# yerfor/Real3DPortrait

Hardware: AMD Instinct MI355X
Metric: rendered frames/sec @ 512x512, 48 depth samples (higher is better)
Workload: dtype f32 operands as fp16 hi + lo, fp32 accumulate (SR precision 'f16mx' = the library default, superresolution.DEFAULT_SR_PRECISION; the fp32-class f16x3 is `alt_f16x3`): in block0.conv1, block1.conv0 and block1.conv1 hi*hi runs on the f16 MFMA and the two cross products on the block-scaled 8-bit MFMA

## Files before the change

real3dportrait_amd/_lib.py:

```python
import contextlib
import ctypes
import os
import subprocess

_HERE = os.path.dirname(os.path.abspath(__file__))
LIB_PATH = os.environ.get("R3D_LIB") or os.path.join(_HERE, "lib", "libr3d_hip.so")
CSRC = os.path.join(_HERE, "csrc")

c_void_p, c_int, c_float, c_size_t, c_uint64 = (ctypes.c_void_p, ctypes.c_int, ctypes.c_float,
                                                ctypes.c_size_t, ctypes.c_uint64)
H = c_void_p


class DevPtr:
    DTYPES = {"float": ("float32",), "double": ("float64",), "int32_t": ("int32",), "int64_t": ("int64",), "uint8_t": ("uint8", "bool"),
              "uint16_t": ("bfloat16", "int16", "uint16"), "void": None}
    ctype = c_void_p

    def __init__(self, elem):
        self.elem = elem

    def __repr__(self):
        return "DevPtr(%r)" % self.elem


class Stream:
    ctype = c_void_p


F, F64, I32, I64, U8, U16, V = (DevPtr(e) for e in ("float", "double", "int32_t", "int64_t", "uint8_t", "uint16_t", "void"))
S = Stream()

SIGNATURES = {
    "r3d_version": (c_int, []),
    "r3d_last_error": (ctypes.c_char_p, []),
    "r3d_planes_to_nhwc": (c_int, [F, F, F, c_int, c_int, c_int, c_int, c_int, c_int, F, ctypes.POINTER(c_int), S]),
    "r3d_planes_absmax_partials": (c_size_t, [c_int, c_int, c_int, c_int, c_int]),
    "r3d_raygen": (c_int, [F, F, c_int, c_int, F, F, S]),
    "r3d_render_workspace_bytes": (c_size_t, [c_int, c_int, c_int, c_int]),
    "r3d_render_forward": (c_int, [F, c_int, c_int, c_int, c_int, F, F, F, F, F, F, c_int, c_int, c_int, c_float, c_int, F, F, c_uint64, F, c_int, F,
                                   F, U8, F, c_int, F, F, V, F, c_size_t, V, c_size_t, S]),
    "r3d_run_model": (c_int, [F, c_int, c_int, c_int, c_int, F, F, F, F, F, c_int, c_float, F, F, F, c_int, V, c_size_t, S]),
    "r3d_run_model_workspace_bytes": (c_size_t, []),
    "r3d_sr_block_prepacked_bytes": (c_size_t, [c_int, c_int]),
    "r3d_sr_block_styles_bytes": (c_size_t, [c_int, c_int, c_int]),
    "r3d_sr_block_workspace_bytes": (c_size_t, [c_int, c_int, c_int, c_int, c_int]),
    "r3d_sr_block_prepack": (c_int, [c_int, c_int, F, F, V, c_int, S]),
    "r3d_sr_block_styles": (c_int, [F, c_int, c_int, c_int, c_int, F, F, F, F, F, F, F, F, F, F, F, F, V, S]),
    "r3d_sr_block_forward": (c_int, [V, V, c_int, c_int, c_int, c_int, c_int, c_int, V, c_int, F, c_float, V, c_int, F, c_size_t, F, U8, F, c_int, V,
                                     c_size_t, S]),
    "r3d_chain_fold": (c_int, [H, c_int, c_int, H, c_int, H, c_int, S]),
    "r3d_sr_block_bound_offset": (c_size_t, [c_int, c_int]),
    "r3d_conv_scales_bound_offset": (c_size_t, [c_int, c_int]),
    "r3d_absmax": (c_int, [F, c_size_t, c_int, F, F, S]),
    "r3d_conv_prepacked_bytes": (c_size_t, [c_int, c_int, c_int]),
    "r3d_conv_workspace_bytes": (c_size_t, [c_int, c_int, c_int, c_int]),
    "r3d_conv_scales_bytes": (c_size_t, [c_int, c_int, c_int]),
    "r3d_conv_prepack": (c_int, [F, c_int, c_int, c_int, V, S]),
    "r3d_conv_forward": (c_int, [V, V, F, c_int, c_int, c_int, c_int, c_int, c_int, V, c_int, c_int, c_float, c_float, c_float, V, c_int, F,
                                 c_size_t, F, V, c_size_t, S]),
    "r3d_blend_cat_to_split": (c_int, [F, c_int, c_int, F, c_int, c_int, F, c_int, c_int, c_int, V, c_int, F, c_size_t, S]),
    "r3d_conv_forward_cat": (c_int, [V, V, F, c_int, c_int, c_int, c_int, c_int, c_int, V, c_int, c_int, c_float, c_float, c_float, V, c_int, c_int,
                                     c_int, F, c_int, F, c_size_t, V, c_size_t, S]),
    "r3d_conv_forward_blend": (c_int, [V, V, F, c_int, c_int, c_int, c_int, c_int, c_int, F, F, F, c_int, c_float, c_float, c_float, V, c_int, F,
                                       c_size_t, F, S]),
    "r3d_debug_conv_variant": (c_int, [c_int, c_int, c_int, c_int, c_int, c_int, c_int, c_int, ctypes.POINTER(c_int)]),
    "r3d_debug_sr_block_variants": (c_int, [c_int, c_int, c_int, c_int, c_int, c_int, c_int, c_int, c_float, ctypes.POINTER(c_int)]),
    "r3d_upsample2x_bilinear": (c_int, [F, c_int, c_int, c_int, c_int, V, c_int, F, c_size_t, S]),
    "r3d_resize_bilinear": (c_int, [F, c_int, c_int, c_int, F, c_int, c_int, c_int, S]),
    "r3d_blend": (c_int, [F, F, F, c_int, c_int, c_int, c_int, F, S]),
    "r3d_person_occlusion": (c_int, [F, F, c_float, c_size_t, F, S]),
    "r3d_frames_to_u8": (c_int, [F, c_int, c_int, c_int, U8, S]),
    "r3d_comm_unique_id": (c_int, [H]),
    "r3d_comm_init": (c_int, [H, c_int, c_int, ctypes.POINTER(c_void_p)]),
    "r3d_comm_destroy": (c_int, [H]),
    "r3d_gather_frames": (c_int, [H, U8, c_size_t, U8, c_int, S]),
    "r3d_event_create": (c_int, [ctypes.POINTER(c_void_p)]),
    "r3d_event_record": (c_int, [H, S]),
    "r3d_event_elapsed_ms": (c_int, [H, H, ctypes.POINTER(c_float)]),
    "r3d_event_destroy": (c_int, [H]),
    "r3d_profile_configure": (c_int, [ctypes.c_uint32]),
    "r3d_profile_reset": (c_int, []),
    "r3d_profile_read": (c_int, [c_int, ctypes.POINTER(ctypes.c_double), ctypes.POINTER(c_int)]),
    "r3d_profile_clock": (c_int, [c_int, ctypes.POINTER(ctypes.c_double), ctypes.POINTER(ctypes.c_ulonglong)]),
    "r3d_secc_embed1": (c_int, [F, c_int, c_int, c_int, c_int, F, F, F, F, F, F, F, S]),
    "r3d_secc_conv": (c_int, [F, c_int, c_int, c_int, c_int, F, F, c_int, c_int, c_int, c_int, F, F, c_float, F, S]),
    "r3d_secc_linear": (c_int, [F, c_int, c_int, F, F, c_float, F, F, c_int, c_int, F, F, S]),
    "r3d_secc_layernorm": (c_int, [F, c_int, c_int, F, F, c_float, F, S]),
    "r3d_secc_attention": (c_int, [F, F, c_int, c_int, c_int, c_int, c_int, c_float, F, S]),
    "r3d_secc_dwconv_gelu": (c_int, [F, c_int, c_int, c_int, c_int, F, F, F, S]),
    "r3d_secc_head": (c_int, [F, c_int, c_int, c_int, F, F, F, F, F, F, F, F, S]),
    "r3d_torso_volume_to_cl": (c_int, [F, c_int, c_int, c_int, c_int, c_int, F, S]),
    "r3d_torso_warp": (c_int, [F, c_int, c_int, c_int, c_int, c_int, F, c_int, c_int, c_int, F, c_int, S]),
    "r3d_torso_conv": (c_int, [F, c_int, c_int, c_int, c_int, c_int, c_int, F, F, c_float, F, F, c_int, c_int, c_int, c_float, F, F, F, S]),
    "r3d_torso_conv3d": (c_int, [F, c_int, c_int, c_int, c_int, c_int, c_int, F, F, c_int, c_int, c_int, c_int, c_float, c_int, F, c_int, c_int, F,
                                 S]),
    "r3d_torso_motion_input": (c_int, [F, c_int, c_int, c_int, c_int, c_int, F, F, F, F, F, c_int, F, c_int, F, c_int, S]),
    "r3d_torso_motion_deform": (c_int, [F, c_int, c_int, c_int, c_int, c_int, F, F, F, F, S]),
    "r3d_torso_motion_broadcast": (c_int, [F, c_int, c_int, c_int, c_int, c_int, F, c_int, c_int, S]),
    "r3d_torso_conv_prec": (c_int, [F, c_int, c_int, c_int, c_int, c_int, c_int, F, F, c_float, F, F, c_int, c_int, c_int, c_float, F, F, F, c_int,
                                    S]),
    "r3d_torso_conv3d_prec": (c_int, [F, c_int, c_int, c_int, c_int, c_int, c_int, F, F, c_int, c_int, c_int, c_int, c_float, c_int, F, c_int, c_int,
                                      F, c_int, S]),
    "r3d_torso_split_bf16x3": (c_int, [F, c_size_t, U16, U16, U16, S]),
    "r3d_torso_conv_pool": (c_int, [F, c_int, c_int, c_int, c_int, c_int, F, F, c_int, c_int, c_int, c_float, c_int, F, c_int, S]),
    "r3d_torso_conv_split": (c_int, [F, c_int, c_int, c_int, c_int, c_int, F, F, c_int, c_int, c_int, c_float, c_int, F, c_int, S]),
    "r3d_torso_conv3d_res": (c_int, [F, c_int, c_int, c_int, c_int, c_int, F, F, c_float, F, F, c_int, c_int, c_int, c_float, F, F, F, c_int, S]),
    "r3d_torso_seg_input": (c_int, [F, c_int, c_int, F, c_int, c_int, c_int, c_int, c_int, F, c_int, c_int, S]),
    "r3d_torso_mask_volume": (c_int, [F, c_int, c_int, c_int, c_int, c_int, F, c_int, c_int, c_int, c_int, c_int, c_int, c_int, F, F, S]),
    "r3d_raster_workspace_bytes": (c_size_t, [c_int, c_int, c_int]),
    "r3d_raster_forward": (c_int, [F, F, I32, c_int, c_int, c_int, c_int, c_int, c_int, c_float, c_float, c_int, c_int, c_float, c_float, I64, F, F,
                                   F, V, c_size_t, S]),
    "r3d_secc_blink_workspace_bytes": (c_size_t, [c_int, c_int, c_int]),
    "r3d_secc_blink": (c_int, [F, c_int, c_int, c_int, I32, F64, c_int, F, I32, V, c_size_t, S]),
    "r3d_face_vertex": (c_int, [F, F, F, c_int, c_int, c_int, F, F, F, F, c_int, c_float, c_int, F, S]),
    "r3d_face_landmarks": (c_int, [F, F, F, c_int, c_int, c_int, F, F, F, F, c_int, c_float, c_int, c_float, c_float, c_float, F, S]),
    "r3d_clip_camera": (c_int, [F, F, c_int, c_int, ctypes.c_double, F, S]),
    "r3d_camera_smooth": (c_int, [F, c_int, c_int, c_int, F, S]),
    "r3d_smooth_features": (c_int, [F, c_int, c_int, c_int, c_int, F, S]),
    "r3d_video_depth_range": (c_int, [F, c_size_t, c_int, I32, S]),
    "r3d_video_compose_debug": (c_int, [F, F, c_int, c_int, F, c_int, c_int, F, c_int, c_int, F, c_int, c_int, c_int, c_int, I32, U8, S]),
    "r3d_source_workspace_bytes": (c_size_t, [c_int, c_int, c_int]),
    "r3d_source_nearest": (c_int, [U8, c_int, c_int, c_int, I32, I32, I32, V, c_size_t, S]),
    "r3d_source_background": (c_int, [U8, U8, c_int, c_int, c_int, U8, I32, V, c_size_t, S]),
    "r3d_source_torso": (c_int, [U8, U8, c_int, c_int, ctypes.POINTER(ctypes.c_double), ctypes.POINTER(c_int), U8, U8, U8, U8, V, c_size_t, S]),
    "r3d_source_select": (c_int, [U8, U8, c_int, c_int, c_int, U8, U8, S]),
    "r3d_source_to_planes": (c_int, [U8, U8, c_int, c_int, c_int, F, S]),
}
AUDIO_SIGNATURES = {
    "r3d_a2m_conv1d": (c_int, [F, c_int, c_int, c_int, c_int, c_int, c_int, F, F, c_int, c_int, c_int, c_int, c_int, F, F, I64, c_int, c_int, F, F, F, F, F, F,
                               c_int, c_int, c_int, S]),
    "r3d_a2m_wn_layer": (c_int, [F, F, c_int, c_int, c_int, c_int, c_int, F, F, F, F, F, c_int, c_int, F, F, S]),
    "r3d_a2m_pitch_embed": (c_int, [F, c_int, c_int, F, c_int, c_int, I32, F, S]),
}
_FIT_COMMON = [F, F, F, c_int, c_int, c_int, F, F, c_int, c_int, c_float, c_float, c_float, ctypes.POINTER(c_float)]
FIT_SIGNATURES = {
    "r3d_fit_workspace_bytes": (c_size_t, [c_int, c_int, c_int, c_int]),
    "r3d_fit_state_bytes": (c_size_t, [c_int, c_int, c_int, c_int]),
    "r3d_fit_landmark_grad": (c_int, _FIT_COMMON + [F, F, F, F, F, F, F, F, F, V, c_size_t, S]),
    "r3d_fit_landmark_run": (c_int, _FIT_COMMON + [c_float, c_float, c_int, c_int, c_int, c_int, F, V, c_size_t, S]),
}
FIT_LOSS_WORDS, FIT_LAUNCHES = 8, 2
A2M_WN_ROWS = 16
VIDEO_STATE_WORDS, VIDEO_PANELS_ALL, VIDEO_PANEL_DEPTH = 8, 31, 8
SOURCE_MAX_SIDE, SOURCE_STATUS_WORDS, SOURCE_DARKEN, SOURCE_HEAD_CLASSES = 2048, 2, 53, 42

OPTIONAL_SIGNATURES = {
    "r3d_debug_merge_fallbacks": (c_int, [ctypes.POINTER(ctypes.c_ulonglong), c_int]),
    "r3d_debug_raster_forward": (c_int, [F, F, I32, c_int, c_int, c_int, c_int, c_int, c_int, c_float, c_float, c_int, c_int, c_float, c_float,
                                         I64, F, F, F, V, c_size_t, c_int, c_int, S]),
    "r3d_debug_secc_blink": (c_int, [F, c_int, c_int, c_int, I32, F64, c_int, F, I32, V, c_size_t, c_int, S]),
}


class ChainOp(ctypes.Structure):
    _fields_ = [("kind", c_int), ("Cin", c_int), ("Cout", c_int), ("ksize", c_int), ("act", c_int),
                ("gain", c_float), ("clamp", c_float), ("src_a", c_int), ("src_b", c_int),
                ("scales", c_void_p), ("prepacked", c_void_p), ("bias", c_void_p)]


CHAIN_SR_BLOCK, CHAIN_CONV, CHAIN_SR_BLOCK_TAIL, CHAIN_SRC_NONE, CHAIN_MAX_OPS, CHAIN_MAX_EXT, CHAIN_MAX_ZERO = 0, 1, 2, -1000, 12, 4, 4

ABI_VERSION = 80
_lib = None
_torch = None
_Tensor = ()
_plans = {}
_calls = None


def build(force=False):
    args = ["make", "-s", "-C", CSRC, "-j4"]
    if force:
        args.append("-B")
    subprocess.check_call(args)
    return LIB_PATH


def _bind(fn, name, res, params, torch):
    fn.restype, fn.argtypes = res, [getattr(p, "ctype", p) for p in params]
    dtypes = lambda names: names and tuple(getattr(torch, d) for d in names if hasattr(torch, d))
    dev = tuple((i, p.elem, dtypes(DevPtr.DTYPES[p.elem])) for i, p in enumerate(params) if isinstance(p, DevPtr))
    _plans[name] = (len(params), bool(params) and isinstance(params[-1], Stream), dev, res is c_int and name != "r3d_version")


def load():
    global _lib, _torch, _Tensor
    if _lib is not None:
        return _lib
    import torch
    if not os.path.exists(LIB_PATH):
        raise RuntimeError(
            "real3dportrait_amd: HIP extension %s not built -- run `make -C %s` (there is no CPU/eager fallback)"
            % (LIB_PATH, CSRC))
    try:
        lib = ctypes.CDLL(LIB_PATH)
    except OSError as e:
        raise RuntimeError("real3dportrait_amd: cannot load %s: %s" % (LIB_PATH, e))
    for name, (res, params) in list(SIGNATURES.items()) + list(AUDIO_SIGNATURES.items()) + list(FIT_SIGNATURES.items()):
        try:
            fn = getattr(lib, name)
        except AttributeError:
            raise RuntimeError("real3dportrait_amd: %s does not export %s, which this package binds -- rebuild it (`make -C %s`)"
                               % (LIB_PATH, name, CSRC))
        _bind(fn, name, res, params, torch)
    for name, (res, params) in OPTIONAL_SIGNATURES.items():
        fn = getattr(lib, name, None)
        if fn is not None:
            _bind(fn, name, res, params, torch)
    if lib.r3d_version() != ABI_VERSION:
        raise RuntimeError("real3dportrait_amd: %s reports ABI %d, this package binds ABI %d -- rebuild it (`make -C %s`)"
                           % (LIB_PATH, lib.r3d_version(), ABI_VERSION, CSRC))
    _torch, _Tensor = torch, torch.Tensor
    _lib = lib
    return lib


def call(name, *args):
    lib = load()
    n, stream, dev, status = _plans[name]
    args = list(args)
    add_stream = stream and len(args) == n - 1
    if len(args) != n and not add_stream:
        raise TypeError("libr3d_hip %s takes %d arguments%s, got %d" % (name, n, " (the stream may be left out)" if stream else "", len(args)))
    for i, elem, dtypes in dev:
        t = args[i]
        if isinstance(t, _Tensor):
            if dtypes is not None and t.dtype not in dtypes:
                raise TypeError("libr3d_hip %s: argument %d is a %s*, got a %s tensor" % (name, i, elem, t.dtype))
            if not t.is_contiguous():
                raise ValueError("libr3d_hip %s: argument %d (%s*) is not contiguous" % (name, i, elem))
            if not t.is_cuda:
                raise ValueError("libr3d_hip %s: argument %d (%s*) is not on a GPU: the library operates on device tensors only" % (name, i, elem))
            args[i] = t.data_ptr()
    if add_stream:
        args.append(_torch.cuda.current_stream().cuda_stream)
    if _calls is not None:
        _calls.append((name, tuple(args)))
    rc = getattr(lib, name)(*args)
    if not status:
        return rc
    if rc != 0:
        check(rc, name[4:])


@contextlib.contextmanager
def counting():
    global _calls
    outer, _calls = _calls, []
    try:
        yield _calls
    finally:
        _calls = outer


def check(rc, what=""):
    if rc != 0:
        msg = load().r3d_last_error()
        raise RuntimeError("libr3d_hip %s failed (%d): %s" % (what, rc, msg.decode() if msg else "?"))


def ptr(t):
    if t is None:
        return None
    if not t.is_cuda:
        raise ValueError("libr3d_hip operates on device tensors only")
    if not t.is_contiguous():
        raise ValueError("libr3d_hip takes contiguous tensors")
    return t.data_ptr()


def stream_ptr():
    load()
    return _torch.cuda.current_stream().cuda_stream
```

real3dportrait_amd/csrc/r3d_sr.hip:

```cpp
#include "r3d_sr_launch.h"

namespace r3d {


static constexpr int TILE_H = 8, TILE_W = 16;
static constexpr int PATCH_H = TILE_H + 2, PATCH_W = TILE_W + 2, PATCH_PIX = PATCH_H * PATCH_W;
static constexpr int CHUNKS_PER_STAGE = 4;

__global__ void nchw_to_cb8_kernel(const float* __restrict__ src, float* __restrict__ dst, int C, int HW)
{
    const int n = blockIdx.z, cb = blockIdx.y;
    const int p = blockIdx.x * blockDim.x + threadIdx.x;
    if (p >= HW) return;
    const float* s = src + ((size_t)n * C + cb * 8) * HW + p;
    float v[8];
#pragma unroll
    for (int c = 0; c < 8; ++c) v[c] = s[(size_t)c * HW];
    float4* d = reinterpret_cast<float4*>(dst + (((size_t)n * (C / 8) + cb) * HW + p) * 8);
    d[0] = make_float4(v[0], v[1], v[2], v[3]);
    d[1] = make_float4(v[4], v[5], v[6], v[7]);
}

__global__ void cb8_to_nchw_kernel(const float* __restrict__ src, float* __restrict__ dst, int C, int HW)
{
    const int n = blockIdx.z, cb = blockIdx.y;
    const int p = blockIdx.x * blockDim.x + threadIdx.x;
    if (p >= HW) return;
    const float4* s = reinterpret_cast<const float4*>(src + (((size_t)n * (C / 8) + cb) * HW + p) * 8);
    const float4 a = s[0], b = s[1];
    float* d = dst + ((size_t)n * C + cb * 8) * HW + p;
    d[0] = a.x; d[(size_t)HW] = a.y; d[(size_t)2 * HW] = a.z; d[(size_t)3 * HW] = a.w;
    d[(size_t)4 * HW] = b.x; d[(size_t)5 * HW] = b.y; d[(size_t)6 * HW] = b.z; d[(size_t)7 * HW] = b.w;
}

__global__ void sr_prepack_kernel(const float* __restrict__ w, int Ci, int Cout, float* __restrict__ out)
{
    const size_t e = (size_t)blockIdx.x * blockDim.x + threadIdx.x;
    const size_t total = (size_t)9 * (Ci / 8) * Cout * 2;
    if (e >= total) return;
    const int half = e & 1;
    const int co = (e >> 1) % Cout;
    const int chunk = ((e >> 1) / Cout) % (Ci / 8);
    const int tap = (int)((e >> 1) / Cout / (Ci / 8));
    const int ci = chunk * 8 + half * 4;
    const float* src = w + ((size_t)co * Ci + ci) * 9 + tap;
    reinterpret_cast<float4*>(out)[e] = make_float4(src[0], src[9], src[18], src[27]);
}

__global__ void sr_styles_kernel(const float* __restrict__ ws3, int WD, int Cin, int Cout,
                                 const float* __restrict__ aw0, const float* __restrict__ ab0,
                                 const float* __restrict__ aw1, const float* __restrict__ ab1,
                                 const float* __restrict__ aw2, const float* __restrict__ ab2,
                                 float* __restrict__ styles, size_t stride_n)
{
    const int layer = blockIdx.y, n = blockIdx.z;
    const SrStyleLayout L = sr_style_layout(Cin, Cout);
    const float* aw = layer == 0 ? aw0 : (layer == 1 ? aw1 : aw2);
    const float* ab = layer == 0 ? ab0 : (layer == 1 ? ab1 : ab2);
    const int C = layer == 0 ? Cin : Cout;
    const int lane = threadIdx.x & 63, c = blockIdx.x * (blockDim.x >> 6) + (threadIdx.x >> 6);
    if (c >= C) return;
    float* out = styles + n * stride_n + (layer == 0 ? L.s0 : (layer == 1 ? L.s1 : L.s2));
    const float* w = ws3 + ((size_t)n * 3 + layer) * WD;
    const float g = rsqrtf((float)WD);
    const float post = layer == 2 ? rsqrtf((float)Cout) : 1.0f;
    float acc = 0.f;
    for (int j = lane; j < WD; j += 64) acc += w[j] * (aw[(size_t)c * WD + j] * g);
#pragma unroll
    for (int d = 32; d >= 1; d >>= 1) acc += __shfl_xor(acc, d);
    if (lane == 0) out[c] = (acc + ab[c]) * post;
}

__global__ void sr_demod_kernel(int Cin, int Cout, const float* __restrict__ w0, const float* __restrict__ w1,
                                const float* __restrict__ wrgb, const float* __restrict__ b0, const float* __restrict__ b1,
                                const float* __restrict__ brgb, float* __restrict__ styles, size_t stride_n)
{
    const int co = blockIdx.x, n = blockIdx.y, layer = blockIdx.z;
    const SrStyleLayout L = sr_style_layout(Cin, Cout);
    float* base = styles + n * stride_n;
    if (co == Cout) {
        if (layer == 0)
            for (int i = threadIdx.x; i < 3 * Cout; i += blockDim.x) {
                base[L.wrgb + i] = wrgb[i] * base[L.s2 + (i % Cout)];
                if (i < Cout) { base[L.b0 + i] = b0[i]; base[L.b1 + i] = b1[i]; }
                if (i < 3) base[L.brgb + i] = brgb[i];
            }
        return;
    }
    const int Ci = layer == 0 ? Cin : Cout;
    const float* W = (layer == 0 ? w0 : w1) + (size_t)co * Ci * 9;
    const float* st = base + (layer == 0 ? L.s0 : L.s1);
    float ss = 0.f, l1 = 0.f, mx = 0.f;
    for (int i = threadIdx.x; i < Ci * 9; i += blockDim.x) {
        const float wv = W[i], v = wv * st[i / 9];
        ss += v * v; l1 += fabsf(v); mx = fmaxf(mx, fabsf(wv));
    }
#pragma unroll
    for (int d = 32; d >= 1; d >>= 1) { ss += __shfl_xor(ss, d); l1 += __shfl_xor(l1, d); mx = fmaxf(mx, __shfl_xor(mx, d)); }
    __shared__ float red[3][4];
    if ((threadIdx.x & 63) == 0) { red[0][threadIdx.x >> 6] = ss; red[1][threadIdx.x >> 6] = l1; red[2][threadIdx.x >> 6] = mx; }
    __syncthreads();
    if (threadIdx.x == 0) {
        const float d = rsqrtf(red[0][0] + red[0][1] + red[0][2] + red[0][3] + 1e-8f);
        base[(layer == 0 ? L.d0 : L.d1) + co] = d;
        base[(layer == 0 ? L.c0 : L.c1) + co] = d * (red[1][0] + red[1][1] + red[1][2] + red[1][3]);
        base[(layer == 0 ? L.wi0 : L.wi1) + co] = pow2f(-weight_row_exp(fmaxf(fmaxf(red[2][0], red[2][1]), fmaxf(red[2][2], red[2][3]))));
    }
}

struct ChainArgs {
    r3d_chain_op ops[R3D_CHAIN_MAX_OPS];
    const float* ext[R3D_CHAIN_MAX_EXT];
    float* zero[R3D_CHAIN_MAX_ZERO];
    int nops, N, nzero, next;
};

__device__ __forceinline__ float block_max(float v, float* red)
{
#pragma unroll
    for (int d = 32; d >= 1; d >>= 1) v = fmaxf(v, __shfl_xor(v, d));
    __syncthreads();
    if ((threadIdx.x & 63) == 0) red[threadIdx.x >> 6] = v;
    __syncthreads();
    return fmaxf(fmaxf(red[0], red[1]), fmaxf(red[2], red[3]));
}

__global__ __launch_bounds__(256) void chain_fold_kernel(ChainArgs a)
{
    __shared__ float red[4];
    __shared__ float bounds[R3D_CHAIN_MAX_OPS];
    __shared__ float extv[R3D_CHAIN_MAX_EXT];
    const int n = blockIdx.x, tid = threadIdx.x;
    if (tid < a.next) extv[tid] = fabsf(a.ext[tid][n]);
    {
        float touch = 0.f;
        for (int k = 0; k < a.nops; ++k) {
            const r3d_chain_op& op = a.ops[k];
            if (op.kind == R3D_CHAIN_SR_BLOCK || op.kind == R3D_CHAIN_SR_BLOCK_TAIL) {
                const SrStyleLayout L = sr_style_layout(op.Cin, op.Cout);
                const float* base = reinterpret_cast<const float*>(op.scales) + (size_t)n * L.total;
                for (int i = tid; i < op.Cin; i += 256) touch += base[L.s0 + i];
                for (int i = tid; i < op.Cout; i += 256)
                    touch += base[L.s1 + i] + base[L.d0 + i] + base[L.d1 + i] + base[L.wi0 + i] + base[L.wi1 + i] + base[L.b0 + i] + base[L.b1 + i] + base[L.c0 + i] + base[L.c1 + i];
            } else {
                const ConvPackLayout P = conv_pack_layout(op.Cin, op.Cout, op.ksize);
                const ConvTail T = conv_tail_layout(P.Co);
                const float* tail = reinterpret_cast<const float*>(op.prepacked) + P.tail;
                for (int i = tid; i < P.Co; i += 256) touch += tail[T.winv + i] + tail[T.l1 + i] + (op.bias && i < op.Cout ? op.bias[i] : 0.f);
            }
        }
        if (touch == 1.2345e-33f && a.nzero < 0) extv[0] = touch;
    }
    __syncthreads();
// ... 269 lines not shown
    float o[4] = {acc.x + b[0], acc.y + b[1], acc.z + b[2], acc.w + b[3]};
#pragma unroll
    for (int r = 0; r < 4; ++r) {
        float t = o[r];
        t = (t < 0.f ? t * 0.2f : t) * 1.4142135623730951f;
        if (clamp >= 0.f) t = fminf(fmaxf(t, -clamp), clamp);
        o[r] = t;
    }
    *reinterpret_cast<float4*>(y + (size_t)n * y_stride_n + (((size_t)cb * OH + oy) * OW + ox) * 8 + half * 4) =
        make_float4(o[0], o[1], o[2], o[3]);
}

__global__ void torgb_upsample_kernel(const float* __restrict__ x, size_t x_stride_n,
                                      const float* __restrict__ wrgb, const float* __restrict__ brgb, size_t pk_stride_n,
                                      const float* __restrict__ img_prev, float* __restrict__ img_out,
                                      int C, int H, int W, float clamp)
{
    extern __shared__ float sw[];
    const int n = blockIdx.y;
    for (int i = threadIdx.x; i < 3 * C; i += blockDim.x) sw[i] = wrgb[(size_t)n * pk_stride_n + i];
    __syncthreads();
    const int p = blockIdx.x * blockDim.x + threadIdx.x;
    if (p >= H * W) return;
    const int y = p / W, xx = p - y * W;
    const float* X = x + (size_t)n * x_stride_n;
    float a0 = 0.f, a1 = 0.f, a2 = 0.f;
    const int ncb = C >> 3;
    for (int cb = 0; cb < ncb; ++cb) {
        const float4* s = reinterpret_cast<const float4*>(X + ((size_t)cb * H * W + p) * 8);
        const float4 u = s[0], v = s[1];
        const float xv[8] = {u.x, u.y, u.z, u.w, v.x, v.y, v.z, v.w};
#pragma unroll
        for (int c = 0; c < 8; ++c) {
            a0 += xv[c] * sw[cb * 8 + c];
            a1 += xv[c] * sw[C + cb * 8 + c];
            a2 += xv[c] * sw[2 * C + cb * 8 + c];
        }
    }
    const float* br = brgb + (size_t)n * pk_stride_n;
    float o[3] = {a0 + br[0], a1 + br[1], a2 + br[2]};
    if (clamp >= 0.f) {
#pragma unroll
        for (int c = 0; c < 3; ++c) o[c] = fminf(fmaxf(o[c], -clamp), clamp);
    }
    const int Hh = H >> 1, Wh = W >> 1;
    const int ky = y >> 1, kx = xx >> 1;
    int r0, r1, c0, c1; float wy0, wy1, wx0, wx1;
    if (y & 1) { r0 = ky; r1 = ky + 1; wy0 = 0.75f; wy1 = 0.25f; } else { r0 = ky - 1; r1 = ky; wy0 = 0.25f; wy1 = 0.75f; }
    if (xx & 1) { c0 = kx; c1 = kx + 1; wx0 = 0.75f; wx1 = 0.25f; } else { c0 = kx - 1; c1 = kx; wx0 = 0.25f; wx1 = 0.75f; }
    const bool vr0 = r0 >= 0 && r0 < Hh, vr1 = r1 >= 0 && r1 < Hh, vc0 = c0 >= 0 && c0 < Wh, vc1 = c1 >= 0 && c1 < Wh;
#pragma unroll
    for (int c = 0; c < 3; ++c) {
        const float* I = img_prev + ((size_t)n * 3 + c) * Hh * Wh;
        float up = 0.f;
        if (vr0 && vc0) up += I[(size_t)r0 * Wh + c0] * (wy0 * wx0);
        if (vr0 && vc1) up += I[(size_t)r0 * Wh + c1] * (wy0 * wx1);
        if (vr1 && vc0) up += I[(size_t)r1 * Wh + c0] * (wy1 * wx0);
        if (vr1 && vc1) up += I[(size_t)r1 * Wh + c1] * (wy1 * wx1);
        img_out[((size_t)n * 3 + c) * H * W + p] = up + o[c];
    }
}


}

using namespace r3d;

extern "C" size_t r3d_sr_block_prepacked_bytes(int Cin, int Cout) { return sr_pack_layout(Cin, Cout).total * sizeof(float); }

extern "C" size_t r3d_sr_block_styles_bytes(int N, int Cin, int Cout)
{
    return (size_t)N * sr_style_layout(Cin, Cout).total * sizeof(float);
}

extern "C" size_t r3d_sr_block_workspace_bytes(int N, int Cin, int Cout, int Hin, int Win) { return sr_workspace_layout(N, Cin, Cout, Hin, Win).total; }

namespace r3d {
void sr_fill_tconv_phases(ConvPhase* ph, int Hin, int Win)
{
    for (int pa = 0; pa < 2; ++pa)
        for (int pb = 0; pb < 2; ++pb) {
            ConvPhase& p = ph[pa * 2 + pb];
            p.outH = Hin + (pa == 0); p.outW = Win + (pb == 0);
            p.oy_mul = 2; p.oy_add = pa; p.ox_mul = 2; p.ox_add = pb; p.out_off = 0;
            p.ntaps = 0;
            for (int ky = pa; ky < 3; ky += 2)
                for (int kx = pb; kx < 3; kx += 2) {
                    p.dy[p.ntaps] = -(ky >> 1); p.dx[p.ntaps] = -(kx >> 1); p.widx[p.ntaps] = ky * 3 + kx;
                    ++p.ntaps;
                }
        }
}
void sr_fill_conv3x3_phase(ConvPhase* ph, int H, int W)
{
    ConvPhase& p = ph[0];
    p.outH = H; p.outW = W; p.oy_mul = 1; p.oy_add = 0; p.ox_mul = 1; p.ox_add = 0; p.ntaps = 9; p.out_off = 0;
    for (int ky = 0; ky < 3; ++ky)
        for (int kx = 0; kx < 3; ++kx) { p.dy[ky * 3 + kx] = ky - 1; p.dx[ky * 3 + kx] = kx - 1; p.widx[ky * 3 + kx] = ky * 3 + kx; }
}
void sr_fill_conv1x1_phase(ConvPhase* ph, int H, int W)
{
    ConvPhase& p = ph[0];
    p.outH = H; p.outW = W; p.oy_mul = 1; p.oy_add = 0; p.ox_mul = 1; p.ox_add = 0; p.out_off = 0;
    p.ntaps = 1; p.dy[0] = 0; p.dx[0] = 0; p.widx[0] = 0;
}
}

static int sr_check_dims(const char* what, int Cin, int Cout)
{
    if (Cin <= 0 || Cout <= 0 || (Cin & 7) || (Cout % BLOCK_M)) {
        set_error("%s: Cin %d must be a multiple of 8 and Cout %d a multiple of %d", what, Cin, Cout, BLOCK_M);
        return R3D_ERR_INVALID_ARG;
    }
    return R3D_OK;
}

extern "C" int r3d_sr_block_prepack(int Cin, int Cout, const float* c0_w, const float* c1_w, void* prepacked,
                                    int precision, r3d_stream_t stream)
{
    if (precision < R3D_SR_F32 || precision > R3D_SR_F16MX) { set_error("sr_block_prepack: unknown precision %d", precision); return R3D_ERR_INVALID_ARG; }
    if (!c0_w || !c1_w || !prepacked) { set_error("sr_block_prepack: NULL pointer"); return R3D_ERR_INVALID_ARG; }
    if (int rc = sr_check_dims("sr_block_prepack", Cin, Cout)) return rc;
    hipStream_t st = (hipStream_t)stream;
    float* out = reinterpret_cast<float*>(prepacked);
    ProfScope ps(R3D_PROF_PACK, st);
    if (precision != R3D_SR_F32) return sr_prepack_f16x3(Cin, Cout, c0_w, c1_w, prepacked, st, precision == R3D_SR_F16MX);
    const size_t n0 = (size_t)9 * (Cin / 8) * Cout * 2, n1 = (size_t)9 * (Cout / 8) * Cout * 2;
    const SrPackLayout P = sr_pack_layout(Cin, Cout);
    hipLaunchKernelGGL(sr_prepack_kernel, dim3((unsigned)((n0 + 255) / 256)), dim3(256), 0, st, c0_w, Cin, Cout, out + P.c0);
    hipLaunchKernelGGL(sr_prepack_kernel, dim3((unsigned)((n1 + 255) / 256)), dim3(256), 0, st, c1_w, Cout, Cout, out + P.c1);
    return check_launch("sr_block_prepack");
}

extern "C" int r3d_sr_block_styles(const float* ws3, int N, int WD, int Cin, int Cout,
                                   const float* c0_w, const float* c0_b, const float* c0_aw, const float* c0_ab,
                                   const float* c1_w, const float* c1_b, const float* c1_aw, const float* c1_ab,
                                   const float* rgb_w, const float* rgb_b, const float* rgb_aw, const float* rgb_ab,
                                   void* styles, r3d_stream_t stream)
{
    if (!ws3 || !c0_w || !c0_b || !c0_aw || !c0_ab || !c1_w || !c1_b || !c1_aw || !c1_ab || !rgb_w || !rgb_b || !rgb_aw || !rgb_ab || !styles) {
        set_error("sr_block_styles: NULL pointer"); return R3D_ERR_INVALID_ARG;
    }
    if (N <= 0 || WD <= 0) { set_error("sr_block_styles: bad shape"); return R3D_ERR_INVALID_ARG; }
    if (int rc = sr_check_dims("sr_block_styles", Cin, Cout)) return rc;
    hipStream_t st = (hipStream_t)stream;
    float* sv = reinterpret_cast<float*>(styles);
    const size_t stride = sr_style_layout(Cin, Cout).total;
    ProfScope ps(R3D_PROF_PACK, st);
    hipLaunchKernelGGL(sr_styles_kernel, dim3(((Cin > Cout ? Cin : Cout) + 3) / 4, 3, N), dim3(256), 0, st, ws3, WD, Cin, Cout, c0_aw, c0_ab, c1_aw, c1_ab, rgb_aw, rgb_ab, sv, stride);
    hipLaunchKernelGGL(sr_demod_kernel, dim3(Cout + 1, N, 2), dim3(256), 0, st, Cin, Cout, c0_w, c1_w, rgb_w, c0_b, c1_b, rgb_b, sv, stride);
    return check_launch("sr_block_styles");
}

extern "C" int r3d_sr_block_forward(const void* prepacked, const void* styles, int N, int Cin, int Cout, int Hin, int Win, int up,
                                    const void* x, int x_format, const float* img, float clamp,
                                    void* x_out, int x_out_format, const float* next_scale, size_t next_scale_stride,
                                    float* img_out, uint8_t* img_u8, float* x_absmax, int precision,
                                    void* workspace, size_t workspace_bytes, r3d_stream_t stream)
{
    if (precision < R3D_SR_F32 || precision > R3D_SR_F16MX) { set_error("sr_block_forward: unknown precision %d", precision); return R3D_ERR_INVALID_ARG; }
    if ((img_u8 || x_absmax) && precision == R3D_SR_F32) { set_error("sr_block_forward: the fused uint8 output / x_absmax need R3D_SR_F16X3"); return R3D_ERR_INVALID_ARG; }
    if (!prepacked || !styles || !x || !img || (!img_out && !img_u8) || N <= 0 || Hin <= 0 || Win <= 0 || (Cin & 15) || (Cout % BLOCK_M) || (up != 0 && up != 1)) {
        set_error("sr_block_forward: bad argument"); return R3D_ERR_INVALID_ARG;
    }
    if (!up && precision == R3D_SR_F32) { set_error("sr_block_forward: up=0 (SynthesisBlockNoUp) needs R3D_SR_F16X3"); return R3D_ERR_INVALID_ARG; }
    if (int rc = r3d::check_index32("sr_block_forward", (size_t)(Cin > Cout ? Cin : Cout), (size_t)(up ? 2 : 1) * Hin, (size_t)(up ? 2 : 1) * Win)) return rc;
    if (!workspace || workspace_bytes < r3d_sr_block_workspace_bytes(N, Cin, Cout, Hin, Win)) {
        set_error("sr_block_forward: workspace too small"); return R3D_ERR_WORKSPACE;
    }
    if (!x_out) x_out_format = R3D_FMT_NONE;
    const bool f16 = precision != R3D_SR_F32;
    const bool mxp = precision == R3D_SR_F16MX;
    if (x_format < R3D_FMT_NCHW || x_format > R3D_FMT_SPLIT_MX || x_out_format < R3D_FMT_NONE || x_out_format > R3D_FMT_SPLIT_MX ||
        (!f16 && (x_format >= R3D_FMT_SPLIT || x_out_format >= R3D_FMT_SPLIT)) ||
        ((x_format == R3D_FMT_SPLIT_MX || x_out_format == R3D_FMT_SPLIT_MX) && !mxp) ||
        (x_out_format >= R3D_FMT_SPLIT && !next_scale)) {
        set_error("sr_block_forward: unsupported activation format (x %d, x_out %d, precision %d)", x_format, x_out_format, precision);
        return R3D_ERR_INVALID_ARG;
    }
    hipStream_t st = (hipStream_t)stream;
    if (f16)
        return sr_block_forward_f16x3(prepacked, styles, N, Cin, Cout, Hin, Win, up, x, x_format, img, clamp, x_out, x_out_format,
                                      next_scale, next_scale_stride, img_out, img_u8, x_absmax, workspace, st, precision == R3D_SR_F16MX);

    const SrStyleLayout L = sr_style_layout(Cin, Cout);
    const float* pk = reinterpret_cast<const float*>(styles);
    const float* wpk = reinterpret_cast<const float*>(prepacked);
    const SrPackLayout P = sr_pack_layout(Cin, Cout);
    const int OH = 2 * Hin, OW = 2 * Win, TH = OH + 1, TW = OW + 1;
    const SrWorkspaceLayout WS = sr_workspace_layout(N, Cin, Cout, Hin, Win);
    char* wsb = reinterpret_cast<char*>(workspace);
    float* xin = reinterpret_cast<float*>(wsb + WS.xin);
    float* T = reinterpret_cast<float*>(wsb + WS.T);
    float* y0 = reinterpret_cast<float*>(wsb + WS.y0);
    float* xo = reinterpret_cast<float*>(wsb + WS.xo);

    const float* xcb = reinterpret_cast<const float*>(x);
    if (x_format == R3D_FMT_NCHW) {
        ProfScope ps(R3D_PROF_LAYOUT, st);
        hipLaunchKernelGGL(nchw_to_cb8_kernel, dim3((Hin * Win + 255) / 256, Cin / 8, N), dim3(256), 0, st, xcb, xin, Cin, Hin * Win);
        xcb = xin;
    }
    {
        ConvArgs a;
        a.x = xcb; a.x_stride_n = (size_t)Cin * Hin * Win;
        a.wp = wpk + P.c0; a.in_scale = pk + L.s0; a.out_scale = pk + L.d0; a.vec_stride_n = L.total;
        a.bias = nullptr;
        a.y = T; a.y_stride_n = (size_t)Cout * TH * TW;
        a.Cin = Cin; a.Cout = Cout; a.H = Hin; a.W = Win; a.OH = TH; a.OW = TW;
        a.nphase = 4; a.act = 0; a.clamp = -1.f;
        sr_fill_tconv_phases(a.ph, Hin, Win);
        int maxtiles = 0;
        for (int p = 0; p < 4; ++p) {
            const int tiles = ((a.ph[p].outW + TILE_W - 1) / TILE_W) * ((a.ph[p].outH + TILE_H - 1) / TILE_H);
            if (tiles > maxtiles) maxtiles = tiles;
        }
        ProfScope ps(R3D_PROF_CONV, st);
        hipLaunchKernelGGL(conv_mfma_kernel, dim3(maxtiles, Cout / BLOCK_M, N * 4), dim3(256), 0, st, a);
    }
    {
    ProfScope ps(R3D_PROF_UPCONV, st);
    hipLaunchKernelGGL(fir_bias_act_kernel, dim3((OH * OW * 2 + 255) / 256, Cout / 8, N), dim3(256), 0, st,
                       T, (size_t)Cout * TH * TW, pk + L.b0, L.total, y0, (size_t)Cout * OH * OW, Cout, OH, OW, clamp);
    }
    float* xo_cb = (x_out_format == R3D_FMT_CB8) ? reinterpret_cast<float*>(x_out) : xo;
    {
        ConvArgs a;
        a.x = y0; a.x_stride_n = (size_t)Cout * OH * OW;
        a.wp = wpk + P.c1; a.in_scale = pk + L.s1; a.out_scale = pk + L.d1; a.vec_stride_n = L.total;
        a.bias = pk + L.b1;
        a.y = xo_cb; a.y_stride_n = (size_t)Cout * OH * OW;
        a.Cin = Cout; a.Cout = Cout; a.H = OH; a.W = OW; a.OH = OH; a.OW = OW;
        a.nphase = 1; a.act = 1; a.clamp = clamp;
        sr_fill_conv3x3_phase(a.ph, OH, OW);
        const int tiles = ((OW + TILE_W - 1) / TILE_W) * ((OH + TILE_H - 1) / TILE_H);
        ProfScope ps(R3D_PROF_CONV, st);
        hipLaunchKernelGGL(conv_mfma_kernel, dim3(tiles, Cout / BLOCK_M, N), dim3(256), 0, st, a);
    }
    {
    ProfScope ps(R3D_PROF_TORGB, st);
    hipLaunchKernelGGL(torgb_upsample_kernel, dim3((OH * OW + 255) / 256, N), dim3(256), 3 * Cout * sizeof(float), st,
                       xo_cb, (size_t)Cout * OH * OW, pk + L.wrgb, pk + L.brgb, L.total, img, img_out, Cout, OH, OW, clamp);
    }
    if (x_out_format == R3D_FMT_NCHW) {
        ProfScope ps(R3D_PROF_LAYOUT, st);
        hipLaunchKernelGGL(cb8_to_nchw_kernel, dim3((OH * OW + 255) / 256, Cout / 8, N), dim3(256), 0, st, xo_cb,
                           reinterpret_cast<float*>(x_out), Cout, OH * OW);
    }
    return check_launch("sr_block_forward");
}

extern "C" size_t r3d_conv_prepacked_bytes(int Cin, int Cout, int ksize) { return r3d::conv_prepacked_bytes_f16x3(Cin, Cout, ksize); }
extern "C" size_t r3d_conv_workspace_bytes(int N, int Cin, int H, int W) { return r3d::conv_workspace_bytes_f16x3(N, Cin, H, W); }
extern "C" size_t r3d_conv_scales_bytes(int N, int Cin, int Cout)
{
    const ConvPackLayout P = conv_pack_layout(Cin, Cout, 1);
    return (size_t)N * conv_scales_layout(P.Ci, P.Co).total * sizeof(float);
}
extern "C" size_t r3d_conv_scales_bound_offset(int Cin, int Cout)
{
    const ConvPackLayout P = conv_pack_layout(Cin, Cout, 1);
    return conv_scales_layout(P.Ci, P.Co).meta + 1;
}
extern "C" size_t r3d_sr_block_bound_offset(int Cin, int Cout) { return sr_style_layout(Cin, Cout).meta + SR_META_BOUND_OUT; }

extern "C" int r3d_conv_prepack(const float* weight, int Cin, int Cout, int ksize, void* prepacked, r3d_stream_t stream)
{
    using namespace r3d;
    if (!weight || !prepacked || Cin <= 0 || Cout <= 0 || (ksize != 1 && ksize != 3)) { set_error("conv_prepack: bad argument"); return R3D_ERR_INVALID_ARG; }
    return conv_prepack_f16x3(weight, Cin, Cout, ksize, prepacked, (hipStream_t)stream);
}

extern "C" int r3d_chain_fold(const r3d_chain_op* ops, int nops, int N, const float* const* ext_bounds, int n_ext,
                              float* const* zero_slots, int n_zero, r3d_stream_t stream)
{
    using namespace r3d;
    if (!ops || nops <= 0 || nops > R3D_CHAIN_MAX_OPS || N <= 0 || n_ext < 0 || n_ext > R3D_CHAIN_MAX_EXT || (n_ext && !ext_bounds) ||
        n_zero < 0 || n_zero > R3D_CHAIN_MAX_ZERO || (n_zero && !zero_slots)) {
        set_error("chain_fold: bad argument (1..%d ops, 0..%d external bounds, 0..%d zero slots)", R3D_CHAIN_MAX_OPS, R3D_CHAIN_MAX_EXT, R3D_CHAIN_MAX_ZERO);
        return R3D_ERR_INVALID_ARG;
    }
    ChainArgs a = {};
    a.nops = nops; a.N = N; a.nzero = n_zero; a.next = n_ext;
    for (int j = 0; j < n_zero; ++j) {
        if (!zero_slots[j]) { set_error("chain_fold: zero slot %d is NULL", j); return R3D_ERR_INVALID_ARG; }
        a.zero[j] = zero_slots[j];
    }
    for (int j = 0; j < n_ext; ++j) {
        if (!ext_bounds[j]) { set_error("chain_fold: external bound %d is NULL", j); return R3D_ERR_INVALID_ARG; }
        a.ext[j] = ext_bounds[j];
    }
    for (int k = 0; k < nops; ++k) {
        const r3d_chain_op& op = ops[k];
        const int srcs[2] = {op.src_a, op.src_b};
        for (int j = 0; j < 2; ++j) {
            const int sidx = srcs[j];
            const bool ok = sidx == R3D_CHAIN_SRC_NONE || (sidx >= 0 && sidx < k) || (sidx < 0 && sidx >= -n_ext);
            if (!ok) { set_error("chain_fold: op %d reads bound source %d (must be an earlier op or an external bound)", k, sidx); return R3D_ERR_INVALID_ARG; }
        }
        if (op.src_a == R3D_CHAIN_SRC_NONE && op.src_b == R3D_CHAIN_SRC_NONE) { set_error("chain_fold: op %d has no input bound", k); return R3D_ERR_INVALID_ARG; }
        if ((op.kind != R3D_CHAIN_SR_BLOCK && op.kind != R3D_CHAIN_CONV && op.kind != R3D_CHAIN_SR_BLOCK_TAIL) || !op.scales || op.Cin <= 0 || op.Cout <= 0 ||
            (op.kind == R3D_CHAIN_CONV && (!op.prepacked || (op.ksize != 1 && op.ksize != 3)))) {
            set_error("chain_fold: op %d is malformed", k); return R3D_ERR_INVALID_ARG;
        }
        a.ops[k] = op;
        if (a.ops[k].src_a == R3D_CHAIN_SRC_NONE) a.ops[k].src_a = -R3D_CHAIN_MAX_EXT - 1;
        if (a.ops[k].src_b == R3D_CHAIN_SRC_NONE) a.ops[k].src_b = -R3D_CHAIN_MAX_EXT - 1;
    }
    ProfScope ps(R3D_PROF_PACK, (hipStream_t)stream);
    hipLaunchKernelGGL(chain_fold_kernel, dim3(N), dim3(256), 0, (hipStream_t)stream, a);
    return check_launch("chain_fold");
}

extern "C" int r3d_absmax(const float* x, size_t count_per_sample, int N, float* out, float* zero_next, r3d_stream_t stream)
{
    using namespace r3d;
    if (!x || !out || N <= 0 || count_per_sample == 0) { set_error("absmax: bad argument"); return R3D_ERR_INVALID_ARG; }
    size_t blocks = (count_per_sample / 4 + 255) / 256;
    if (blocks > 512) blocks = 512;
    if (blocks < 1) blocks = 1;
    ProfScope ps(R3D_PROF_LAYOUT, (hipStream_t)stream);
    hipLaunchKernelGGL(absmax_kernel, dim3((unsigned)blocks, N), dim3(256), 0, (hipStream_t)stream, x, count_per_sample,
                       reinterpret_cast<unsigned*>(out), reinterpret_cast<unsigned*>(zero_next));
    return check_launch("absmax");
}

extern "C" int r3d_conv_forward(const void* prepacked, const void* scales, const float* bias,
                                int N, int Cin, int Cout, int H, int W, int ksize,
                                const void* x, int x_format, int act, float act_slope, float act_gain, float clamp,
                                void* y, int y_format, const float* next_scale, size_t next_scale_stride, float* y_absmax,
                                void* workspace, size_t workspace_bytes, r3d_stream_t stream)
{
    using namespace r3d;
    SrConvCall c = sr_conv_call("conv_forward", N, Cin, Cout, H, W, ksize, act, act_slope, act_gain, clamp, y, y_format, next_scale, next_scale_stride,
                                y_absmax, (hipStream_t)stream);
    c.prepacked = prepacked; c.scales = scales; c.bias = bias; c.x = x; c.x_format = x_format; c.workspace = workspace; c.workspace_bytes = workspace_bytes;
    if (int rc = check(c)) return rc;
    return conv_forward_f16x3(c);
}

extern "C" int r3d_conv_forward_cat(const void* prepacked, const void* scales, const float* bias,
                                    int N, int Cin, int Cout, int H, int W, int ksize,
                                    const void* x, int x_format, int act, float act_slope, float act_gain, float clamp,
                                    void* y_cat, int y_format, int C_total, int chan_off, const float* mask, int mask_invert,
                                    const float* next_scale, size_t next_scale_stride,
                                    void* workspace, size_t workspace_bytes, r3d_stream_t stream)
{
    using namespace r3d;
    const ConvCat cat = {mask, mask_invert ? 1 : 0, C_total, chan_off};
    SrConvCall c = sr_conv_call("conv_forward_cat", N, Cin, Cout, H, W, ksize, act, act_slope, act_gain, clamp, y_cat, y_format, next_scale, next_scale_stride,
                                nullptr, (hipStream_t)stream);
    c.prepacked = prepacked; c.scales = scales; c.bias = bias; c.x = x; c.x_format = x_format; c.workspace = workspace; c.workspace_bytes = workspace_bytes;
    c.cat = &cat;
    if (int rc = check(c)) return rc;
    return conv_forward_f16x3(c);
}

extern "C" int r3d_conv_forward_blend(const void* prepacked, const void* scales, const float* bias,
                                      int N, int Ca, int Cb, int Cout, int H, int W,
                                      const float* a, const float* b, const float* mask,
                                      int act, float act_slope, float act_gain, float clamp,
                                      void* y, int y_format, const float* next_scale, size_t next_scale_stride, float* y_absmax, r3d_stream_t stream)
{
    using namespace r3d;
    SrConvCall c = sr_conv_call("conv_forward_blend", N, Ca + Cb, Cout, H, W, 1, act, act_slope, act_gain, clamp, y, y_format,
                                next_scale, next_scale_stride, y_absmax, (hipStream_t)stream);
    c.prepacked = prepacked; c.scales = scales; c.bias = bias;
    c.blend = true; c.bl_a = a; c.bl_b = b; c.bl_mask = mask; c.Ca = Ca; c.Cb = Cb;
    if (int rc = check(c)) return rc;
    return conv_forward_blend_f16x3(c);
}

static void put_variant(const r3d::SrVariantChoice& v, int* out)
{
    out[0] = v.variant; out[1] = v.bits; out[2] = v.order; out[3] = (int)v.gx; out[4] = (int)v.gy; out[5] = (int)v.gz;
}

extern "C" int r3d_debug_conv_variant(int N, int Cin, int Cout, int H, int W, int ksize, int x_format, int blend, int* out)
{
    using namespace r3d;
    if (!out || N <= 0 || Cin <= 0 || Cout <= 0 || H <= 0 || W <= 0 || (ksize != 1 && ksize != 3) || (blend && ksize != 1) ||
        x_format < R3D_FMT_NCHW || x_format > R3D_FMT_SPLIT_MX || (x_format != R3D_FMT_NCHW && (Cin & 15)) || (x_format == R3D_FMT_SPLIT_MX && ksize != 3)) {
        set_error("debug_conv_variant: bad argument"); return R3D_ERR_INVALID_ARG;
    }
    const ConvPackLayout P = conv_pack_layout(Cin, Cout, ksize);
    put_variant(blend ? sr_blend_variant(P.Co, H, W, N) : sr_conv_variant(ksize, P.Ci, P.Co, H, W, N, x_format == R3D_FMT_SPLIT_MX, false, sr_wino_mode()), out);
    return R3D_OK;
}

extern "C" int r3d_debug_sr_block_variants(int N, int Cin, int Cout, int Hin, int Win, int up, int x_format, int precision, float clamp, int* out)
{
    using namespace r3d;
    if (!out || N <= 0 || Hin <= 0 || Win <= 0 || (Cin & 15) || Cin <= 0 || Cout <= 0 || (Cout % BLOCK_M) || (up != 0 && up != 1) ||
        (precision != R3D_SR_F16X3 && precision != R3D_SR_F16MX) || x_format < R3D_FMT_NCHW || x_format > R3D_FMT_SPLIT_MX ||
        (x_format == R3D_FMT_SPLIT_MX && precision != R3D_SR_F16MX)) {
        set_error("debug_sr_block_variants: bad argument"); return R3D_ERR_INVALID_ARG;
    }
    SrVariantChoice v[2];
    sr_block_variants(N, Cin, Cout, Hin, Win, up, x_format, precision == R3D_SR_F16MX, clamp, sr_wino_mode(), v);
    put_variant(v[0], out); put_variant(v[1], out + 6);
    return R3D_OK;
}

extern "C" int r3d_upsample2x_bilinear(const float* x_cb8, int N, int C, int H, int W, void* y, int y_format,
                                       const float* next_scale, size_t next_scale_stride, r3d_stream_t stream)
{
    using namespace r3d;
    if (!x_cb8 || !y || N <= 0 || C <= 0 || (C & 7) || H <= 0 || W <= 0) { set_error("upsample2x_bilinear: bad argument (C %d must be a multiple of 8)", C); return R3D_ERR_INVALID_ARG; }
    if (y_format != R3D_FMT_CB8 && y_format != R3D_FMT_SPLIT && y_format != R3D_FMT_SPLIT_MX) { set_error("upsample2x_bilinear: y_format %d must be CB8, SPLIT or SPLIT_MX", y_format); return R3D_ERR_INVALID_ARG; }
    if (y_format == R3D_FMT_SPLIT_MX && (C & 15)) { set_error("upsample2x_bilinear: SPLIT_MX needs C %% 16 == 0 (C %d)", C); return R3D_ERR_INVALID_ARG; }
    return upsample2x_bilinear_f16x3(x_cb8, N, C, H, W, y, y_format, next_scale, next_scale_stride, (hipStream_t)stream);
}

extern "C" int r3d_blend_cat_to_split(const float* a, int a_format, int Ca, const float* b, int b_format, int Cb, const float* mask,
                                      int N, int H, int W, void* y_split, int y_format, const float* next_scale, size_t next_scale_stride,
                                      r3d_stream_t stream)
{
    if (y_format != R3D_FMT_SPLIT && y_format != R3D_FMT_SPLIT_MX) { set_error("blend_cat_to_split: y_format %d must be SPLIT or SPLIT_MX", y_format); return R3D_ERR_INVALID_ARG; }
    using namespace r3d;
    if (!a || !mask || !y_split || N <= 0 || H <= 0 || W <= 0 || Ca <= 0 || Cb <= 0 || (Ca & 7) || (Cb & 7) || ((Ca + Cb) & 15) || (!b && (Ca & 15))) {
        set_error("blend_cat_to_split: bad argument (Ca %d, Cb %d: multiples of 8, sum a multiple of 16; b = NULL needs Ca %% 16 == 0)", Ca, Cb); return R3D_ERR_INVALID_ARG;
    }
    if ((a_format != R3D_FMT_NCHW && a_format != R3D_FMT_CB8) || (b && b_format != R3D_FMT_NCHW && b_format != R3D_FMT_CB8)) {
        set_error("blend_cat_to_split: inputs must be NCHW or CB8 (a %d, b %d)", a_format, b_format); return R3D_ERR_INVALID_ARG;
    }
    return blend_cat_to_split_f16x3(a, a_format, Ca, b, b_format, Cb, mask, N, H, W, y_split, y_format, next_scale, next_scale_stride, (hipStream_t)stream);
}
```

real3dportrait_amd/csrc/r3d_sr_common.h:

```cpp
#pragma once
#include "r3d_common.h"

namespace r3d {

typedef float f32x16 __attribute__((ext_vector_type(16)));
static constexpr int BLOCK_M = 128;
static __host__ __device__ inline size_t align256(size_t b) { return (b + 255) & ~(size_t)255; }

static constexpr int kWeightTargetExp = 10;
static constexpr int kActTargetExp = 15;

__host__ __device__ inline int pow2_ceil_exp(float m)
{
    if (!(m > 0.f) || !(m < 3.0e38f)) return 0;
    int e;
    (void)frexpf(m, &e);
    return e;
}
__host__ __device__ inline float pow2f(int e) { return ldexpf(1.0f, e < -120 ? -120 : (e > 120 ? 120 : e)); }
__host__ __device__ inline int weight_row_exp(float rowmax) { return rowmax > 0.f ? kWeightTargetExp + 1 - pow2_ceil_exp(rowmax) : 0; }
__host__ __device__ inline int act_exp(float B, float smax)
{
    const int eb = B > 0.f ? pow2_ceil_exp(B) : 0;
    int es = smax > 0.f ? pow2_ceil_exp(smax) : 0;
    if (smax > 0.f && smax < 3.0e38f && ldexpf(1.0f, es - 1) == smax) --es;
    return kActTargetExp - eb - es;
}

struct SrStyleLayout { size_t s0f, s1f, d0f, d1f, s0, s1, s2, d0, d1, wrgb, b0, b1, brgb, c0, c1, wi0, wi1, meta, total; };
static __host__ __device__ inline SrStyleLayout sr_style_layout(int Cin, int Cout)
{
    SrStyleLayout L;
    size_t o = 0;
    L.s0f = o; o += Cin;
    L.s1f = o; o += Cout;
    L.d0f = o; o += Cout;
    L.d1f = o; o += Cout;
    L.s0 = o; o += Cin;
    L.s1 = o; o += Cout;
    L.s2 = o; o += Cout;
    L.d0 = o; o += Cout;
    L.d1 = o; o += Cout;
    L.wrgb = o; o += (size_t)3 * Cout;
    L.b0 = o; o += Cout;
    L.b1 = o; o += Cout;
    L.brgb = o; o += 4;
    L.c0 = o; o += Cout;
    L.c1 = o; o += Cout;
    L.wi0 = o; o += Cout;
    L.wi1 = o; o += Cout;
    L.meta = o; o += 8;
    L.total = (o + 3) & ~(size_t)3;
    return L;
}
enum { SR_META_BOUND_IN = 0, SR_META_BOUND_MID = 1, SR_META_BOUND_OUT = 2, SR_META_E0 = 3, SR_META_E1 = 4, SR_META_SMAX0 = 5, SR_META_SMAX1 = 6 };

struct ConvTail { size_t winv, l1, total; };
static __host__ __device__ inline ConvTail conv_tail_layout(int CoutPadded)
{
    ConvTail T; T.winv = 0; T.l1 = CoutPadded; T.total = 2 * (size_t)CoutPadded; return T;
}
struct ConvScales { size_t in_vec, out_vec, meta, total; };
static __host__ __device__ inline ConvScales conv_scales_layout(int CinPadded, int CoutPadded)
{
    ConvScales S; S.in_vec = 0; S.out_vec = CinPadded; S.meta = (size_t)CinPadded + CoutPadded; S.total = (S.meta + 4 + 3) & ~(size_t)3; return S;
}

struct SrPackLayout { size_t c0, c1, c0_up, tail0, tail1, c0_up_mx, c0_mx, c1_wino, total; };
static __host__ __device__ inline SrPackLayout sr_pack_layout(int Cin, int Cout)
{
    SrPackLayout P;
    const size_t w0 = (size_t)9 * Cin * Cout, w1 = (size_t)9 * Cout * Cout;
    size_t o = 0;
    P.c0 = o; o += w0;
    P.c1 = o; o += w1;
    P.c0_up = o; o += w0;
    P.tail0 = o; o += conv_tail_layout(Cout).total;
    P.tail1 = o; o += conv_tail_layout(Cout).total;
    P.c0_up_mx = o; o += w0;
    P.c0_mx = o; o += w0;
    P.c1_wino = o; o += (size_t)12 * Cout * Cout;
    P.total = o;
    return P;
}
struct ConvPackLayout { int Ci, Co; size_t w, tail, w_mx, w_wino, total; };
static __host__ __device__ inline ConvPackLayout conv_pack_layout(int Cin, int Cout, int ksize)
{
    ConvPackLayout P;
    P.Ci = (Cin + 15) / 16 * 16; P.Co = (Cout + BLOCK_M - 1) / BLOCK_M * BLOCK_M;
    const size_t cc = (size_t)P.Ci * P.Co, w = (size_t)(ksize * ksize) * cc;
    size_t o = 0;
    P.w = o; o += w;
    P.tail = o; o += conv_tail_layout(P.Co).total;
    P.w_mx = o; o += ksize == 3 ? w : 0;
    P.w_wino = o; o += ksize == 3 ? 12 * cc : 0;
    P.total = o;
    return P;
}
struct SrWorkspaceLayout { size_t xin, T, y0, xo, rgbp, total; };
static __host__ __device__ inline SrWorkspaceLayout sr_workspace_layout(int N, int Cin, int Cout, int Hin, int Win)
{
    SrWorkspaceLayout L;
    const size_t y = align256((size_t)N * Cout * 4 * Hin * Win * 4);
    size_t o = 0;
    L.xin = o; o += align256((size_t)N * Cin * Hin * Win * 4);
    L.T = o; o += align256((size_t)N * Cout * 4 * (Hin + 1) * (Win + 1) * 4);
    L.y0 = o; o += y;
    L.xo = o; o += y;
    L.rgbp = o; o += align256((size_t)N * (Cout / 64) * 3 * 4 * Hin * Win * 4);
    L.total = o;
    return L;
}

struct ConvPhase {
    int outH, outW;
    int oy_mul, oy_add, ox_mul, ox_add;
    int ntaps;
    int dy[9], dx[9], widx[9];
    size_t out_off;
};

void sr_fill_tconv_phases(ConvPhase* ph, int Hin, int Win);
void sr_fill_conv3x3_phase(ConvPhase* ph, int H, int W);
void sr_fill_conv1x1_phase(ConvPhase* ph, int H, int W);

int sr_prepack_f16x3(int Cin, int Cout, const float* c0_w, const float* c1_w, void* prepacked, hipStream_t st, bool mx);
int sr_block_forward_f16x3(const void* prepacked, const void* styles, int N, int Cin, int Cout, int Hin, int Win, int up,
                           const void* x, int x_format, const float* img, float clamp,
                           void* x_out, int x_out_format, const float* next_scale, size_t next_scale_stride,
                           float* img_out, uint8_t* img_u8, float* x_absmax, void* workspace, hipStream_t st, bool mx);

size_t conv_prepacked_bytes_f16x3(int Cin, int Cout, int ksize);
int conv_prepack_f16x3(const float* w, int Cin, int Cout, int ksize, void* prepacked, hipStream_t st);
size_t conv_workspace_bytes_f16x3(int N, int Cin, int H, int W);
struct ConvCat { const float* mask; int mask_invert; int C_total; int chan_off; };

int upsample2x_bilinear_f16x3(const float* x_cb8, int N, int C, int H, int W, void* y, int y_format,
                              const float* next_scale, size_t next_scale_stride, hipStream_t st);

int blend_cat_to_split_f16x3(const float* a, int a_format, int Ca, const float* b, int b_format, int Cb, const float* mask,
                             int N, int H, int W, void* y_split, int y_format, const float* next_scale, size_t next_scale_stride, hipStream_t st);

}
```

real3dportrait_amd/csrc/r3d_sr_f16x3.hip:

```cpp
#include <stdlib.h>

#include "r3d_sr_launch.h"
#include "r3d_stamps.h"

namespace r3d {

typedef _Float16 h8 __attribute__((ext_vector_type(8)));
typedef _Float16 h4 __attribute__((ext_vector_type(4)));
static constexpr int F_TILE_H = 16, F_TILE_W = 16;
static constexpr int F_PATCH_H = F_TILE_H + 2, F_PATCH_W = F_TILE_W + 2, F_PATCH_PIX = F_PATCH_H * F_PATCH_W;

__device__ __forceinline__ void split1(float v, _Float16& hi, _Float16& lo)
{
    v = as_rounded(v);
    const float c = fminf(fmaxf(v, -65504.f), 65504.f);
    hi = (_Float16)c;
    lo = (_Float16)(v - (float)hi);
}

__device__ __forceinline__ void split1_folded(float v, _Float16& hi, _Float16& lo)
{
    v = as_rounded(v);
    hi = (_Float16)v;
    lo = (_Float16)(v - (float)hi);
// ... 20 lines not shown
    return (unsigned)v;
}

__global__ void weight_row_stats_kernel(const float* __restrict__ w, int row_len, int CoutReal, int Cout, float* __restrict__ tail)
{
    const int co = blockIdx.x;
    const ConvTail T = conv_tail_layout(Cout);
    float mx = 0.f, l1 = 0.f;
    if (co < CoutReal)
        for (int i = threadIdx.x; i < row_len; i += blockDim.x) { const float v = fabsf(w[(size_t)co * row_len + i]); mx = fmaxf(mx, v); l1 += v; }
#pragma unroll
    for (int d = 32; d >= 1; d >>= 1) { mx = fmaxf(mx, __shfl_xor(mx, d)); l1 += __shfl_xor(l1, d); }
    __shared__ float rm[4], rl[4];
    if ((threadIdx.x & 63) == 0) { rm[threadIdx.x >> 6] = mx; rl[threadIdx.x >> 6] = l1; }
    __syncthreads();
    if (threadIdx.x == 0) {
        mx = fmaxf(fmaxf(rm[0], rm[1]), fmaxf(rm[2], rm[3]));
        tail[T.winv + co] = pow2f(-weight_row_exp(mx));
        tail[T.l1 + co] = rl[0] + rl[1] + rl[2] + rl[3];
    }
}

__global__ void sr_prepack_mx_kernel(const float* __restrict__ w, int CiReal, int CoutReal, int ntaps, int Ci, int Cout,
                                     const float* __restrict__ winv, uint4* __restrict__ out)
{
    const size_t e = (size_t)blockIdx.x * blockDim.x + threadIdx.x;
    const size_t total = (size_t)ntaps * (Ci / 16) * Cout;
    if (e >= total) return;
    const int co = e % Cout;
    const int grp = (e / Cout) % (Ci / 16);
    const int tap = (int)(e / Cout / (Ci / 16));
    const float ws = 1.0f / winv[co];
    float hi[16], lo[16];
    h8 h0, h1;
#pragma unroll
    for (int j = 0; j < 16; ++j) {
        const int ci = grp * 16 + j;
        const float v = (co < CoutReal && ci < CiReal) ? w[((size_t)co * CiReal + ci) * ntaps + tap] * ws : 0.f;
        _Float16 a, b; split1(v, a, b);
        hi[j] = (float)a; lo[j] = v - (float)a;
        if (j < 8) h0[j] = a; else h1[j - 8] = a;
    }
    uint4 wl8, wh8;
    unsigned* pl = reinterpret_cast<unsigned*>(&wl8); unsigned* ph = reinterpret_cast<unsigned*>(&wh8);
#pragma unroll
    for (int q = 0; q < 4; ++q) {
        const int c = mx_rec_chan(q);
        pl[q] = pack4_fp8(lo[c] * kMxWl, lo[c + 1] * kMxWl, lo[c + 2] * kMxWl, lo[c + 3] * kMxWl);
        ph[q] = pack4_fp8(hi[c] * kMxWh, hi[c + 1] * kMxWh, hi[c + 2] * kMxWh, hi[c + 3] * kMxWh);
    }
    const size_t base = ((size_t)tap * (Ci / 8) + 2 * grp) * 2 * Cout + co;
    out[base] = *reinterpret_cast<uint4*>(&h0);
    out[base + Cout] = wl8;
    out[base + 2 * Cout] = *reinterpret_cast<uint4*>(&h1);
    out[base + 3 * Cout] = wh8;
}

__global__ void sr_prepack_f16_kernel(const float* __restrict__ w, int CiReal, int CoutReal, int ntaps, int Ci, int Cout,
                                      const float* __restrict__ winv, uint4* __restrict__ out)
{
    const size_t e = (size_t)blockIdx.x * blockDim.x + threadIdx.x;
    const size_t total = (size_t)ntaps * (Ci / 8) * Cout;
    if (e >= total) return;
    const int co = e % Cout;
    const int chunk = (e / Cout) % (Ci / 8);
    const int tap = (int)(e / Cout / (Ci / 8));
    const float ws = 1.0f / winv[co];
    h8 hi, lo;
#pragma unroll
    for (int j = 0; j < 8; ++j) {
        const int ci = chunk * 8 + j;
        const float v = (co < CoutReal && ci < CiReal) ? w[((size_t)co * CiReal + ci) * ntaps + tap] * ws : 0.f;
        _Float16 a, b; split1(v, a, b); hi[j] = a; lo[j] = b;
    }
    const size_t base = ((size_t)tap * (Ci / 8) + chunk) * 2 * Cout + co;
    out[base] = *reinterpret_cast<uint4*>(&hi);
    out[base + Cout] = *reinterpret_cast<uint4*>(&lo);
}

__global__ void to_split_kernel(const float* __restrict__ src, int cb8, const float* __restrict__ scale, size_t scale_stride_n,
                                uint4* __restrict__ dst, int C, int Creal, int HW)
{
    const int n = blockIdx.z, cb = blockIdx.y;
    const int p = blockIdx.x * blockDim.x + threadIdx.x;
    if (p >= HW) return;
    float v[8];
    if (cb8) {
        const float4* s4 = reinterpret_cast<const float4*>(src + (((size_t)n * (C / 8) + cb) * HW + p) * 8);
        const float4 a = s4[0], b = s4[1];
        v[0] = a.x; v[1] = a.y; v[2] = a.z; v[3] = a.w; v[4] = b.x; v[5] = b.y; v[6] = b.z; v[7] = b.w;
    } else {
        const float* s = src + ((size_t)n * Creal + cb * 8) * HW + p;
#pragma unroll
        for (int c = 0; c < 8; ++c) v[c] = (cb * 8 + c < Creal) ? s[(size_t)c * HW] : 0.f;
    }
    h8 hi, lo;
#pragma unroll
    for (int c = 0; c < 8; ++c) {
        const float sc = (scale && cb * 8 + c < Creal) ? scale[n * scale_stride_n + cb * 8 + c] : 1.f;
        _Float16 a, b; split_scaled(v[c], sc, a, b); hi[c] = a; lo[c] = b;
    }
    const size_t plane = (size_t)(C / 8) * HW;
    uint4* d = dst + (size_t)n * 2 * plane + (size_t)cb * HW + p;
    d[0] = *reinterpret_cast<uint4*>(&hi);
    d[plane] = *reinterpret_cast<uint4*>(&lo);
}

__device__ uint4 g_zero16[1];

__device__ __forceinline__ void dma64(const uint4* gsrc, uint4* lds_dst_uniform)
{
    const unsigned d = __builtin_amdgcn_readfirstlane((unsigned)(size_t)(__attribute__((address_space(3))) uint4*)lds_dst_uniform);
    unsigned keep;
    asm volatile("s_mov_b32 %0, m0\n\ts_mov_b32 m0, %2\n\ts_nop 0\n\tglobal_load_lds_dwordx4 %1, off\n\ts_mov_b32 m0, %0"
                 : "=&s"(keep) : "v"(gsrc), "s"(d) : "memory");
}

__device__ __forceinline__ void dma64s(const void* base_uniform, unsigned voff_bytes, uint4* lds_dst_uniform)
{
    const unsigned d = __builtin_amdgcn_readfirstlane((unsigned)(size_t)(__attribute__((address_space(3))) uint4*)lds_dst_uniform);
    unsigned keep;
    asm volatile("s_mov_b32 %0, m0\n\ts_mov_b32 m0, %3\n\ts_nop 0\n\tglobal_load_lds_dwordx4 %1, %2\n\ts_mov_b32 m0, %0"
                 : "=&s"(keep) : "v"(voff_bytes), "s"(base_uniform), "s"(d) : "memory");
}
__device__ __forceinline__ void dma64s_masked(const void* base_uniform, unsigned voff_bytes, unsigned long long mask, uint4* lds_dst_uniform)
{
    const unsigned d = __builtin_amdgcn_readfirstlane((unsigned)(size_t)(__attribute__((address_space(3))) uint4*)lds_dst_uniform);
    unsigned keep; unsigned long long save;
    asm volatile("s_mov_b32 %0, m0\n\ts_mov_b32 m0, %4\n\ts_and_saveexec_b64 %1, %5\n\tglobal_load_lds_dwordx4 %2, %3\n\ts_mov_b64 exec, %1\n\ts_mov_b32 m0, %0"
                 : "=&s"(keep), "=&s"(save) : "v"(voff_bytes), "s"(base_uniform), "s"(d), "s"(mask) : "memory", "scc");
}

struct Conv2Args {
    const uint4* x; size_t x_stride_n;
    const uint4* wp;
    const float* out_scale; size_t out_scale_stride_n;
    const float* bias; size_t bias_stride_n;
    float* y_f32; size_t y_f32_stride_n; int OH, OW;
    float* y_nchw; size_t y_nchw_stride_n;
    uint4* y_split; size_t y_split_stride_n;
    int y_split_mx;
    const float* y_mask; int y_mask_invert; int y_cat_chunks, y_cat_off;
    const float* next_scale; size_t next_scale_stride_n;
    unsigned* y_absmax;
    const float* wrgb; size_t wrgb_stride_n; float* rgb_partial; size_t rgbp_stride_n;
    int Cin, Cout, CoutReal, H, W, nphase;
    int act; float act_slope, act_gain, clamp;
    unsigned long long* clk;
    int order;
    const float* bl_a; const float* bl_b; const float* bl_mask; const float* bl_scale; size_t bl_scale_stride_n; int bl_Ca;
    ConvPhase ph[4];
};

static constexpr int EV_STRIDE = BLOCK_M;
template <int WN, int NT, bool WINO = false, bool CAT = false>
__device__ __forceinline__ void conv_epilogue(const Conv2Args& a, const ConvPhase& ph, int n, f32x16 (&acc)[2][NT],
                                              int i0, int j0, int m0, float* ev)
{
#pragma clang fp contract(off)
    const int lane = threadIdx.x & 63, wave = threadIdx.x >> 6;
    const int wm = wave / WN, wn = wave - wm * WN;
    const int li = lane & 31, h = lane >> 5;
    const int prow = li >> 4, pcol = ((li & 15) - 2 * prow) & 15;
    const int row0 = wn * 2 * NT;
    const bool do_rgb = a.rgb_partial != nullptr;
    {
        constexpr int NTHR = 128 * WN;
        for (int e = threadIdx.x; e < 6 * BLOCK_M; e += NTHR) {
            const int v = e / BLOCK_M, c = e - v * BLOCK_M, co = m0 + c;
            float val = (v == 0 || v == 2) ? 1.f : 0.f;
            if (co < a.CoutReal) {
                if (v == 0) { if (a.out_scale) val = a.out_scale[(size_t)n * a.out_scale_stride_n + co]; }
                else if (v == 1) { if (a.bias) val = a.bias[(size_t)n * a.bias_stride_n + co]; }
                else if (v == 2) { if (a.y_split && a.next_scale) val = a.next_scale[(size_t)n * a.next_scale_stride_n + co]; }
                else if (do_rgb) val = a.wrgb[(size_t)n * a.wrgb_stride_n + (size_t)(v - 3) * a.CoutReal + co];
            }
            if (WINO && v == 0) val *= 4.0f;
            ev[e] = val;
        }
        __syncthreads();
    }
    float vmax = 0.f;
    unsigned rec_h[NT], rec_l[NT];
#pragma unroll
    for (int nt = 0; nt < NT; ++nt) { rec_h[nt] = 0u; rec_l[nt] = 0u; }
    float rgbp[NT][3];
#pragma unroll
    for (int nt = 0; nt < NT; ++nt) { rgbp[nt][0] = 0.f; rgbp[nt][1] = 0.f; rgbp[nt][2] = 0.f; }
    const size_t oplane = (size_t)(CAT && a.y_cat_chunks ? a.y_cat_chunks : a.CoutReal >> 3) * a.OH * a.OW;
    const unsigned cs = (unsigned)a.OH * (unsigned)a.OW;
    const int wm_u = __builtin_amdgcn_readfirstlane(wm);
    unsigned p0[NT];
    bool inside_nt[NT];
#pragma unroll
    for (int nt = 0; nt < NT; ++nt) {
        const int i = i0 + row0 + nt * 2 + prow, j = j0 + pcol;
        inside_nt[nt] = i < ph.outH && j < ph.outW;
        p0[nt] = (unsigned)(i * ph.oy_mul + ph.oy_add) * (unsigned)a.OW + (unsigned)(j * ph.ox_mul + ph.ox_add);
    }
    float* Yf = a.y_f32 ? a.y_f32 + (size_t)n * a.y_f32_stride_n + ph.out_off : nullptr;
    float* Yn = a.y_nchw ? a.y_nchw + (size_t)n * a.y_nchw_stride_n : nullptr;
    uint4* Ys = a.y_split ? a.y_split + (size_t)n * a.y_split_stride_n + (CAT ? (size_t)a.y_cat_off * a.OH * a.OW : 0) : nullptr;
    float ym[NT];
#pragma unroll
    for (int nt = 0; nt < NT; ++nt) ym[nt] = 1.f;
    const bool masked = CAT && a.y_mask != nullptr;
    if (masked) {
#pragma unroll
        for (int nt = 0; nt < NT; ++nt) {
            const float mk = inside_nt[nt] ? a.y_mask[(size_t)n * cs + p0[nt]] : 0.f;
            ym[nt] = a.y_mask_invert ? 1.0f - mk : mk;
        }
    }
    const bool want_max = a.y_absmax != nullptr;
#pragma unroll
    for (int mt = 0; mt < 2; ++mt)
#pragma unroll
        for (int g = 0; g < 4; ++g) {
            const int cu = 64 * wm_u + 32 * mt + 8 * g;
            const int cl = cu + 4 * h, co = m0 + cl;
            if (co >= a.CoutReal) continue;
            const unsigned pbase = (unsigned)((m0 + cu) >> 3) * cs;
            const float4 d4 = *reinterpret_cast<const float4*>(ev + cl);
            const float4 b4 = *reinterpret_cast<const float4*>(ev + EV_STRIDE + cl);
            const float4 s4 = *reinterpret_cast<const float4*>(ev + 2 * EV_STRIDE + cl);
            const float4 w0 = *reinterpret_cast<const float4*>(ev + 3 * EV_STRIDE + cl);
            const float4 w1 = *reinterpret_cast<const float4*>(ev + 4 * EV_STRIDE + cl);
            const float4 w2 = *reinterpret_cast<const float4*>(ev + 5 * EV_STRIDE + cl);
            const float dv[4] = {d4.x, d4.y, d4.z, d4.w}, bv[4] = {b4.x, b4.y, b4.z, b4.w}, sv[4] = {s4.x, s4.y, s4.z, s4.w};
            constexpr bool WIDE = NT % 2 == 0;
            uint2 hiw[NT], low[NT];
            unsigned xh8w[NT], xl8w[NT];
#pragma unroll
            for (int nt = 0; nt < NT; ++nt) {
                const bool inside = inside_nt[nt];
                float v[4];
#pragma unroll
                for (int r = 0; r < 4; ++r) {
                    float t = __builtin_fmaf(acc[mt][nt][4 * g + r], dv[r], bv[r]);
                    if (a.act) t = (t < 0.f ? t * a.act_slope : t) * a.act_gain;
                    if (a.clamp >= 0.f) t = fminf(fmaxf(t, -a.clamp), a.clamp);
                    v[r] = t;
                }
                if (do_rgb) {
                    rgbp[nt][0] = __builtin_fmaf(v[3], w0.w, __builtin_fmaf(v[2], w0.z, __builtin_fmaf(v[1], w0.y, __builtin_fmaf(v[0], w0.x, rgbp[nt][0]))));
                    rgbp[nt][1] = __builtin_fmaf(v[3], w1.w, __builtin_fmaf(v[2], w1.z, __builtin_fmaf(v[1], w1.y, __builtin_fmaf(v[0], w1.x, rgbp[nt][1]))));
                    rgbp[nt][2] = __builtin_fmaf(v[3], w2.w, __builtin_fmaf(v[2], w2.z, __builtin_fmaf(v[1], w2.y, __builtin_fmaf(v[0], w2.x, rgbp[nt][2]))));
                }
                if (inside) {
                if (want_max) vmax = fmaxf(vmax, fmaxf(fmaxf(fabsf(v[0]), fabsf(v[1])), fmaxf(fabsf(v[2]), fabsf(v[3]))));
                const unsigned pix = pbase + p0[nt];
                if (Yf) *reinterpret_cast<float4*>(Yf + (size_t)pix * 8 + 4 * h) = make_float4(v[0], v[1], v[2], v[3]);
                if (Yn) {
                    float* yn = Yn + (size_t)(unsigned)(m0 + cu) * cs + (size_t)((unsigned)(4 * h) * cs + p0[nt]);
#pragma unroll
                    for (int r = 0; r < 4; ++r) yn[(size_t)r * cs] = v[r];
                }
                }
                if (Ys) {
                    h4 hi, lo;
                    float lf[4];
#pragma unroll
                    for (int r = 0; r < 4; ++r) {
                        const float sv_ = as_rounded(masked ? v[r] * ym[nt] * sv[r] : v[r] * sv[r]);
                        const _Float16 x0 = (_Float16)sv_;
                        lf[r] = sv_ - (float)x0;
                        hi[r] = x0; lo[r] = (_Float16)lf[r];
                    }
                    if constexpr (WIDE) {
                    hiw[nt] = *reinterpret_cast<uint2*>(&hi);
                    if (a.y_split_mx) {
                        xh8w[nt] = pack4_x8((float)hi[0] * kMxXh, (float)hi[1] * kMxXh, (float)hi[2] * kMxXh, (float)hi[3] * kMxXh);
                        xl8w[nt] = pack4_x8(lf[0] * kMxXl, lf[1] * kMxXl, lf[2] * kMxXl, lf[3] * kMxXl);
                    } else low[nt] = *reinterpret_cast<uint2*>(&lo);
                    } else {
                    if (!inside) continue;
                    const unsigned pix = pbase + p0[nt];
                    uint2* dst = reinterpret_cast<uint2*>(Ys + pix) + h;
                    dst[0] = *reinterpret_cast<uint2*>(&hi);
                    if (a.y_split_mx) {
                        const unsigned xh8 = pack4_x8((float)hi[0] * kMxXh, (float)hi[1] * kMxXh, (float)hi[2] * kMxXh, (float)hi[3] * kMxXh);
                        const unsigned xl8 = pack4_x8(lf[0] * kMxXl, lf[1] * kMxXl, lf[2] * kMxXl, lf[3] * kMxXl);
                        const unsigned c8 = (unsigned)(m0 + cu) >> 3;
                        if (!(c8 & 1u)) { rec_h[nt] = xh8; rec_l[nt] = xl8; }
                        else {
                            uint2* rec = reinterpret_cast<uint2*>(Ys + oplane + (size_t)((c8 & ~1u) * cs + p0[nt])) + h;
                            rec[0] = make_uint2(rec_h[nt], xh8);
                            rec[2 * (size_t)cs] = make_uint2(rec_l[nt], xl8);
                        }
                    } else {
                        dst[2 * oplane] = *reinterpret_cast<uint2*>(&lo);
                    }
                    }
                }
            }
            if constexpr (WIDE) if (Ys) {
                const unsigned c8 = (unsigned)(m0 + cu) >> 3;
#pragma unroll
                for (int nt = 0; nt < NT; nt += 2) {
                    const bool ins = h ? inside_nt[nt + 1] : inside_nt[nt];
                    const unsigned pp = h ? p0[nt + 1] : p0[nt];
                    auto swp = [](unsigned x, unsigned y, unsigned& ox, unsigned& oy) { const auto r = __builtin_amdgcn_permlane32_swap(x, y, false, false); ox = r[0]; oy = r[1]; };
                    uint4 w;
                    swp(hiw[nt].x, hiw[nt + 1].x, w.x, w.z); swp(hiw[nt].y, hiw[nt + 1].y, w.y, w.w);
                    if (ins) Ys[pbase + pp] = w;
                    if (a.y_split_mx) {
                        if (!(c8 & 1u)) { rec_h[nt] = xh8w[nt]; rec_l[nt] = xl8w[nt]; rec_h[nt + 1] = xh8w[nt + 1]; rec_l[nt + 1] = xl8w[nt + 1]; }
                        else {
                            uint4 rh, rl;
                            swp(rec_h[nt], rec_h[nt + 1], rh.x, rh.z); swp(xh8w[nt], xh8w[nt + 1], rh.y, rh.w);
                            swp(rec_l[nt], rec_l[nt + 1], rl.x, rl.z); swp(xl8w[nt], xl8w[nt + 1], rl.y, rl.w);
                            uint4* rec = Ys + oplane + (size_t)((c8 & ~1u) * cs + pp);
                            if (ins) { rec[0] = rh; rec[cs] = rl; }
                        }
                    } else {
                        swp(low[nt].x, low[nt + 1].x, w.x, w.z); swp(low[nt].y, low[nt + 1].y, w.y, w.w);
                        if (ins) Ys[oplane + pbase + pp] = w;
                    }
                }
            }
        }
    if (want_max) {
#pragma unroll
        for (int d = 32; d >= 1; d >>= 1) vmax = fmaxf(vmax, __shfl_xor(vmax, d));
        __syncthreads();
        if (lane == 0) ev[wave] = vmax;
        __syncthreads();
        if (threadIdx.x == 0) {
            float m = ev[0];
            for (int w = 1; w < 2 * WN; ++w) m = fmaxf(m, ev[w]);
            if (m > 0.f) atomicMax(a.y_absmax + n, __float_as_uint(m));
        }
    }
    if (do_rgb) {
#pragma unroll
        for (int nt = 0; nt < NT; ++nt)
#pragma unroll
            for (int o = 0; o < 3; ++o) rgbp[nt][o] += __shfl_xor(rgbp[nt][o], 32);
        if (h == 0) {
            float* P = a.rgb_partial + (size_t)n * a.rgbp_stride_n + (size_t)(m0 / 64 + wm) * 3 * a.OH * a.OW;
#pragma unroll
            for (int nt = 0; nt < NT; ++nt) {
                const int i = i0 + row0 + nt * 2 + prow, j = j0 + pcol;
                if (i < ph.outH && j < ph.outW) {
                    const int oy = i * ph.oy_mul + ph.oy_add, ox = j * ph.ox_mul + ph.ox_add;
#pragma unroll
                    for (int o = 0; o < 3; ++o) P[(size_t)o * a.OH * a.OW + (size_t)oy * a.OW + ox] = rgbp[nt][o];
                }
            }
        }
    }
}

template <int WN, int NT>
__device__ __forceinline__ void conv2_block(const Conv2Args& a, const ConvPhase& ph, int n, uint4* lds)
{
    static_assert(WN * NT == 8, "16 pixel rows per block");
    constexpr int NTHR = 128 * WN;
    constexpr int B_ELEMS = 2 * 2 * F_PATCH_PIX;
    constexpr int NPF = (B_ELEMS + NTHR - 1) / NTHR;
    constexpr int A_ELEMS = 2 * 256;
    constexpr int A_BUF = 3 * 2 * 256;
    constexpr int NAR = A_ELEMS / NTHR;
    uint4* patchB = lds;
    uint4* bufA = lds + B_ELEMS;
    const int tiles_x = (ph.outW + F_TILE_W - 1) / F_TILE_W;
    const int tile = blockIdx.x;
    const int ty = tile / tiles_x, tx = tile - ty * tiles_x;
    const int i0 = ty * F_TILE_H, j0 = tx * F_TILE_W;
    const int m0 = blockIdx.y * BLOCK_M;
    const int lane = threadIdx.x & 63, wave = threadIdx.x >> 6;
    const int wm = wave / WN, wn = wave - wm * WN;
    const int li = lane & 31, h = lane >> 5;
    const int nchunks = a.Cin >> 3;
    const size_t plane = (size_t)nchunks * a.H * a.W;
    const uint4* X = a.x + (size_t)n * a.x_stride_n;
    const uint4* WP = a.wp;

    f32x16 acc[2][NT];
#pragma unroll
    for (int mt = 0; mt < 2; ++mt)
#pragma unroll
        for (int nt = 0; nt < NT; ++nt)
#pragma unroll
            for (int r = 0; r < 16; ++r) acc[mt][nt][r] = 0.f;

    const int prow = li >> 4, pcol = ((li & 15) - 2 * prow) & 15;
    const int row0 = wn * 2 * NT;
    int boff[NT];
#pragma unroll
    for (int nt = 0; nt < NT; ++nt) boff[nt] = (row0 + nt * 2 + prow + 1) * F_PATCH_W + (pcol + 1) + h * F_PATCH_PIX;
    const int aoff = h * 256 + 64 * wm + li;

    const int chunk_stride = a.H * a.W;
    uint4 pf[NPF];
    unsigned pf_off[NPF];
    unsigned pf_valid = 0;
#pragma unroll
    for (int k = 0; k < NPF; ++k) {
        const int e = threadIdx.x + NTHR * k;
        unsigned off = 0;
        if (e < B_ELEMS) {
            const int pl = e / (2 * F_PATCH_PIX);
            const int rem = e - pl * (2 * F_PATCH_PIX);
            const int c = rem / F_PATCH_PIX, pp = rem - c * F_PATCH_PIX;
            const int py = pp / F_PATCH_W, px = pp - py * F_PATCH_W;
            const int iy = i0 + py - 1, ix = j0 + px - 1;
            if (iy >= 0 && iy < a.H && ix >= 0 && ix < a.W) {
                off = (unsigned)(pl * plane) + (unsigned)(c * chunk_stride + iy * a.W + ix);
                pf_valid |= 1u << k;
            }
        }
        pf_off[k] = off;
    }
    auto load_patch = [&](int c0) {
        const uint4* Xs = X + (size_t)c0 * chunk_stride;
#pragma unroll
        for (int k = 0; k < NPF; ++k) {
            uint4 v = Xs[pf_off[k]];
            if (!(pf_valid & (1u << k))) v = make_uint4(0, 0, 0, 0);
            pf[k] = v;
        }
    };
    const int tid_seg = __builtin_amdgcn_readfirstlane(threadIdx.x >> 7);
    const int wave_u = __builtin_amdgcn_readfirstlane(wave);
    const unsigned tid_lo = threadIdx.x & 127;
    auto dma_weights = [&](int c0, uint4* dstA) {
#pragma unroll
        for (int k = 0; k < NAR; ++k) {
            const int seg = (NTHR >> 7) * k + tid_seg, t = seg >> 2, hc = (seg >> 1) & 1, hl = seg & 1;
            if (t >= 1) continue;
            const uint4* src = WP + (((size_t)ph.widx[t] * nchunks + (c0 + hc)) * 2 + hl) * a.Cout + m0;
            const unsigned lds_dst = __builtin_amdgcn_readfirstlane(
                (unsigned)(size_t)(__attribute__((address_space(3))) uint4*)(dstA + NTHR * k + 64 * wave_u));
            const uint4* gsrc = src + tid_lo;
            unsigned keep;
            asm volatile("s_mov_b32 %0, m0\n\ts_mov_b32 m0, %2\n\ts_nop 0\n\tglobal_load_lds_dwordx4 %1, off\n\ts_mov_b32 m0, %0"
                         : "=&s"(keep) : "v"(gsrc), "s"(lds_dst) : "memory");
        }
    };

    dma_weights(0, bufA);
    load_patch(0);
    int g = 0;
    for (int c0 = 0; c0 < nchunks; c0 += 2, ++g) {
        __syncthreads();
#pragma unroll
        for (int k = 0; k < NPF; ++k) {
            const int e = threadIdx.x + NTHR * k;
            if (e < B_ELEMS) patchB[e] = pf[k];
        }
        asm volatile("s_waitcnt vmcnt(0)" ::: "memory");
        asm volatile("s_waitcnt lgkmcnt(0)" ::: "memory");
        __builtin_amdgcn_s_barrier();
        asm volatile("" ::: "memory");
        const uint4* curA = bufA + (g & 1) * A_BUF;
        uint4* nxtA = bufA + ((g + 1) & 1) * A_BUF;
        if (c0 + 2 < nchunks) {
            dma_weights(c0 + 2, nxtA);
            load_patch(c0 + 2);
        }
        h8 ah[2], al[2];
#pragma unroll
        for (int mt = 0; mt < 2; ++mt) {
            uint4 q0 = curA[aoff + mt * 32], q1 = curA[aoff + mt * 32 + 128];
            ah[mt] = *reinterpret_cast<h8*>(&q0); al[mt] = *reinterpret_cast<h8*>(&q1);
        }
        const int toff = ph.dy[0] * F_PATCH_W + ph.dx[0];
#pragma unroll
        for (int nt = 0; nt < NT; ++nt) {
            uint4 r0 = patchB[boff[nt] + toff];
            uint4 r1 = patchB[boff[nt] + toff + 2 * F_PATCH_PIX];
            const h8 bh = *reinterpret_cast<h8*>(&r0), bl = *reinterpret_cast<h8*>(&r1);
#pragma unroll
            for (int mt = 0; mt < 2; ++mt) {
                acc[mt][nt] = __builtin_amdgcn_mfma_f32_32x32x16_f16(al[mt], bh, acc[mt][nt], 0, 0, 0);
                acc[mt][nt] = __builtin_amdgcn_mfma_f32_32x32x16_f16(ah[mt], bl, acc[mt][nt], 0, 0, 0);
                acc[mt][nt] = __builtin_amdgcn_mfma_f32_32x32x16_f16(ah[mt], bh, acc[mt][nt], 0, 0, 0);
            }
        }
    }
    __syncthreads();
    conv_epilogue<WN, NT, false, true>(a, ph, n, acc, i0, j0, m0, reinterpret_cast<float*>(lds));
}

static constexpr int P_SEGS = 21, P_BUF = P_SEGS * 64;
static constexpr int W2_BUF = 2 * 2 * 2 * 128;
static constexpr int F3_LDS_UINT4 = 2 * P_BUF + 2 * W2_BUF;

typedef int i8v __attribute__((ext_vector_type(8)));

template <bool MX = false, int TH = F_TILE_H>
__device__ __forceinline__ void conv3x3_dma_block(const Conv2Args& a, const ConvPhase& ph, int n, uint4* lds)
{
    static_assert(TH == 16 || TH == 8, "tile rows");
    constexpr int WN = 4, NT = TH / 8;
    constexpr int PATCH_PIX = (TH + 2) * F_PATCH_W;
    constexpr int PSEGS = (4 * PATCH_PIX + 63) / 64;
    constexpr int PBUF = PSEGS * 64;
    constexpr int KMAX = (PSEGS + 7) / 8;
    static_assert(PBUF == (TH == 16 ? P_BUF : 768), "patch buffer");
    uint4* pbuf = lds;
    uint4* wbuf = lds + 2 * PBUF;
    const int tiles_x = (ph.outW + F_TILE_W - 1) / F_TILE_W;
    int tile = blockIdx.x, cgi = blockIdx.y;
    if (a.order) {
        const int G = gridDim.y, b = blockIdx.x + gridDim.x * blockIdx.y;
        const int xcd = b & 7, slot = b >> 3;
        cgi = slot % G;
        const int t = slot / G;
        tile = a.order == 1 ? t * 8 + xcd : xcd * (gridDim.x >> 3) + t;
    }
    const int ty = tile / tiles_x, tx = tile - ty * tiles_x;
    const int i0 = ty * TH, j0 = tx * F_TILE_W;
    const int m0 = cgi * BLOCK_M;
    const int lane = threadIdx.x & 63, wave = threadIdx.x >> 6;
    const int wave_u = __builtin_amdgcn_readfirstlane(wave);
    const int wm = wave / WN, wn = wave - wm * WN;
    const int li = lane & 31, h = lane >> 5;
    const int nchunks = a.Cin >> 3, nst = a.Cin >> 4;
    const int chunk_stride = a.H * a.W;
    const size_t plane = (size_t)nchunks * chunk_stride;
    const uint4* X = a.x + (size_t)n * a.x_stride_n;
    const uint4* WP = a.wp + m0 + (wave_u & 1) * 64 + lane;

    f32x16 acc[2][NT];
#pragma unroll
    for (int mt = 0; mt < 2; ++mt)
#pragma unroll
        for (int nt = 0; nt < NT; ++nt)
#pragma unroll
            for (int r = 0; r < 16; ++r) acc[mt][nt][r] = 0.f;

    const int prow = li >> 4, pcol = ((li & 15) - 2 * prow) & 15;
    const int row0 = wn * 2 * NT;
    int boff[NT];
#pragma unroll
    for (int nt = 0; nt < NT; ++nt) boff[nt] = (row0 + nt * 2 + prow + 1) * F_PATCH_W + (pcol + 1) + h * PATCH_PIX;
    const int aoff = h * 256 + 64 * wm + li;

    unsigned pf_off[3];
    unsigned pf_valid = 0;
#pragma unroll
    for (int k = 0; k < KMAX; ++k) {
        const int e = (8 * k + wave_u) * 64 + lane;
        unsigned off = 0;
        if (e < 4 * PATCH_PIX) {
            const int pl = e / (2 * PATCH_PIX), rem = e - pl * (2 * PATCH_PIX);
            const int c = rem / PATCH_PIX, pp = rem - c * PATCH_PIX;
            const int py = pp / F_PATCH_W, px = pp - py * F_PATCH_W;
            const int iy = i0 + py - 1, ix = j0 + px - 1;
            if (iy >= 0 && iy < a.H && ix >= 0 && ix < a.W) {
                off = (unsigned)(pl * plane) + (unsigned)(c * chunk_stride + iy * a.W + ix);
                pf_valid |= 1u << k;
            }
        }
        pf_off[k] = off;
    }
    const bool three = wave_u < PSEGS - 8 * (KMAX - 1);
    unsigned long long pmask[3] = {0, 0, 0};
    unsigned pf_boff[3] = {0, 0, 0};
    const unsigned lane16 = (unsigned)lane * 16u;
    if constexpr (MX) {
#pragma unroll
        for (int k = 0; k < KMAX; ++k) {
            pmask[k] = __ballot((pf_valid >> k) & 1u);
            pf_boff[k] = pf_off[k] * 16u;
            if (k < KMAX - 1 || three) {
                const bool outside = !((pf_valid >> k) & 1u);
                if (outside) pbuf[64 * (8 * k + wave_u) + lane] = make_uint4(0, 0, 0, 0);
                if (outside || nst == 1) pbuf[PBUF + 64 * (8 * k + wave_u) + lane] = make_uint4(0, 0, 0, 0);
            }
        }
        __syncthreads();
    }
    auto dma_patch = [&](int st, uint4* dst) {
        const uint4* Xs = X + (size_t)(2 * st) * chunk_stride;
#pragma unroll
        for (int k = 0; k < KMAX; ++k)
            if (k < KMAX - 1 || three) {
                if constexpr (MX) {
                    if (pmask[k]) dma64s_masked(Xs, pf_boff[k], pmask[k], dst + 64 * (8 * k + wave_u));
                    else dma64(g_zero16, dst + 64 * (8 * k + wave_u));
                } else {
                    dma64((pf_valid & (1u << k)) ? Xs + pf_off[k] : g_zero16, dst + 64 * (8 * k + wave_u));
                }
            }
    };
    auto dma_weights2 = [&](int T0, uint4* dst) {
#pragma unroll
        for (int ts = 0; ts < 2; ++ts) {
            const int T = T0 + ts;
            if (T < 9 * nst) {
                const int st = T / 9, t = T - 9 * st;
                const int hc = (wave_u >> 2) & 1, hl = (wave_u >> 1) & 1;
                if constexpr (MX)
                    dma64s(a.wp + m0 + (wave_u & 1) * 64 + (((size_t)t * nchunks + (2 * st + hc)) * 2 + hl) * a.Cout, lane16,
                           dst + ts * 512 + wave_u * 64);
                else
                    dma64(WP + (((size_t)t * nchunks + (2 * st + hc)) * 2 + hl) * a.Cout, dst + ts * 512 + wave_u * 64);
            } else if (MX && ts == 1 && T0 < 9 * nst) {
                dma64(g_zero16, dst + ts * 512 + wave_u * 64);
            }
        }
    };

    R3D_STAMP_DECL;
    if (blockIdx.x == (gridDim.x >> 1) && blockIdx.y == 0 && blockIdx.z == 0 && threadIdx.x == 0) clk_begin(kernarg_clk<Conv2Args>());
    dma_weights2(0, wbuf);
    dma_patch(0, pbuf);
    R3D_STAMP(4);
    for (int sp = 0; sp < nst; sp += 2) {
#pragma unroll
        for (int uu = 0; uu < 9; ++uu) {
            const int T0 = 9 * sp + 2 * uu;
            if (T0 >= 9 * nst) break;
            const bool patch_behind = ((uu == 1 && sp + 1 < nst) || (uu == 6 && sp + 2 < nst));
            if (patch_behind) {
                if constexpr (KMAX == 3) { if (three) asm volatile("s_waitcnt vmcnt(3)" ::: "memory"); else asm volatile("s_waitcnt vmcnt(2)" ::: "memory"); }
                else { if (three) asm volatile("s_waitcnt vmcnt(2)" ::: "memory"); else asm volatile("s_waitcnt vmcnt(1)" ::: "memory"); }
            } else asm volatile("s_waitcnt vmcnt(0)" ::: "memory");
            asm volatile("s_waitcnt lgkmcnt(0)" ::: "memory");
            __builtin_amdgcn_s_barrier();
            asm volatile("" ::: "memory");
            const int par = (uu + (sp >> 1)) & 1;
            const uint4* curW = wbuf + par * W2_BUF;
            dma_weights2(T0 + 2, wbuf + (par ^ 1) * W2_BUF);
            if (uu == 0 && sp + 1 < nst) dma_patch(sp + 1, pbuf + PBUF);
            if (uu == 5 && sp + 2 < nst) dma_patch(sp + 2, pbuf);
#pragma unroll
            for (int ts = 0; ts < 2; ++ts) {
                const int Tl = 2 * uu + ts;
                const int sl = Tl / 9, t = Tl - 9 * sl;
                if (sp + sl < nst) {
                    const uint4* curP = pbuf + sl * PBUF;
                    h8 ah[2], al[2];
#pragma unroll
                    for (int mt = 0; mt < 2; ++mt) {
                        uint4 q0 = curW[ts * 512 + aoff + mt * 32];
                        ah[mt] = *reinterpret_cast<h8*>(&q0);
                        if (!MX) { uint4 q1 = curW[ts * 512 + aoff + mt * 32 + 128]; al[mt] = *reinterpret_cast<h8*>(&q1); }
                    }
                    const int toff = (t / 3 - 1) * F_PATCH_W + (t % 3 - 1);
#pragma unroll
                    for (int nt = 0; nt < NT; ++nt) {
                        uint4 r0 = curP[boff[nt] + toff];
                        const h8 bh = *reinterpret_cast<h8*>(&r0);
                        h8 bl;
                        if (!MX) { uint4 r1 = curP[boff[nt] + toff + 2 * PATCH_PIX]; bl = *reinterpret_cast<h8*>(&r1); }
#pragma unroll
                        for (int mt = 0; mt < 2; ++mt) {
                            if (!MX) {
                                acc[mt][nt] = __builtin_amdgcn_mfma_f32_32x32x16_f16(al[mt], bh, acc[mt][nt], 0, 0, 0);
                                acc[mt][nt] = __builtin_amdgcn_mfma_f32_32x32x16_f16(ah[mt], bl, acc[mt][nt], 0, 0, 0);
                            }
                            acc[mt][nt] = __builtin_amdgcn_mfma_f32_32x32x16_f16(ah[mt], bh, acc[mt][nt], 0, 0, 0);
                        }
                    }
                }
            }
            if constexpr (MX) {
                const int Tl0 = 2 * uu, Tl1 = 2 * uu + 1;
                const int sl0 = Tl0 / 9, t0 = Tl0 - 9 * sl0, sl1 = Tl1 / 9, t1 = Tl1 - 9 * sl1;
                const int toffa = (t0 / 3 - 1) * F_PATCH_W + (t0 % 3 - 1), toffb = (t1 / 3 - 1) * F_PATCH_W + (t1 % 3 - 1);
                __builtin_amdgcn_sched_barrier(0);
                int hh = h;
                asm volatile("" : "+v"(hh));
                const int p8 = 2 * PATCH_PIX + sl0 * PBUF + toffa + hh * ((sl1 - sl0) * PBUF + toffb - toffa - PATCH_PIX);
                const uint4* P8 = pbuf + p8;
                const uint4* W8 = curW + 128 + aoff + hh * 256;
                i8v a8[2];
#pragma unroll
                for (int mt = 0; mt < 2; ++mt) {
                    const uint4 q0 = W8[mt * 32], q1 = W8[mt * 32 + 256];
                    a8[mt] = (i8v){(int)q0.x, (int)q0.y, (int)q0.z, (int)q0.w, (int)q1.x, (int)q1.y, (int)q1.z, (int)q1.w};
                }
#pragma unroll
                for (int nt = 0; nt < NT; ++nt) {
                    const uint4 r0 = P8[boff[nt]], r1 = P8[boff[nt] + PATCH_PIX];
                    const i8v b8 = (i8v){(int)r0.x, (int)r0.y, (int)r0.z, (int)r0.w, (int)r1.x, (int)r1.y, (int)r1.z, (int)r1.w};
#pragma unroll
                    for (int mt = 0; mt < 2; ++mt) {
                        acc[mt][nt] = __builtin_amdgcn_mfma_scale_f32_32x32x64_f8f6f4(a8[mt], b8, acc[mt][nt], 0, kMxFmtB, 0, kMxScaleA, 0, kMxScaleB);
                    }
                }
                __builtin_amdgcn_sched_barrier(0);
            }
        }
    }
    __syncthreads();
    R3D_STAMP(5);
    conv_epilogue<WN, NT>(a, ph, n, acc, i0, j0, m0, reinterpret_cast<float*>(lds));
    if (blockIdx.x == (gridDim.x >> 1) && blockIdx.y == 0 && blockIdx.z == 0 && threadIdx.x == 0) clk_end(kernarg_clk<Conv2Args>());
    R3D_STAMP(6);
#ifdef R3D_STAMPS
    asm volatile("s_waitcnt vmcnt(0)" ::: "memory");
    R3D_STAMP(7);
    if ((threadIdx.x & 63) == 0) { for (int i_ = 4; i_ < 8; ++i_) atomicAdd(&r3d::g_stamps[8 + i_], st_acc_[i_]); atomicAdd(&r3d::g_stamps[30], 1ull); }
    R3D_STAMP_CLOCKS(26);
#endif
}

#include "r3d_sr_wino.h"

static constexpr int F_LDS_UINT4 = 2 * 2 * F_PATCH_PIX + 2 * 3 * 2 * 256;

template <int WN, int NT, int OCC, bool MX = false>
__global__ __launch_bounds__(128 * WN, OCC) void conv_mfma_f16x3_kernel(Conv2Args a)
{
    static_assert(WN == 4 && NT == 2, "conv3x3_dma_block: 8 waves x (64 couts x 64 px)");
    __shared__ uint4 lds[F3_LDS_UINT4];
    conv3x3_dma_block<MX>(a, a.ph[0], blockIdx.z, lds);
}

static constexpr int F3S_LDS_UINT4 = 2 * 768 + 2 * W2_BUF;
template <bool MX = false>
__global__ __launch_bounds__(512, 4) void conv_mfma_f16x3_rows8_kernel(Conv2Args a)
{
    __shared__ uint4 lds[F3S_LDS_UINT4];
    conv3x3_dma_block<MX, 8>(a, a.ph[0], blockIdx.z, lds);
}

template <int WN, int NT, int OCC>
__global__ __launch_bounds__(128 * WN, OCC) void conv1x1_mfma_f16x3_kernel(Conv2Args a)
{
    __shared__ uint4 lds[F_LDS_UINT4];
    conv2_block<WN, NT>(a, a.ph[0], blockIdx.z, lds);
}

static constexpr int BL_PATCH = 2 * 2 * 256;
static constexpr int BL_DEPTH = 4;
__global__ __launch_bounds__(512, 2) void conv1x1_blend_f16x3_kernel(Conv2Args a)
{
    __shared__ uint4 lds[2 * BL_PATCH + 2 * 512];
    constexpr int WN = 4, NT = 2;
    const ConvPhase& ph = a.ph[0];
    const int n = blockIdx.z;
    const int tiles_x = (ph.outW + F_TILE_W - 1) / F_TILE_W;
    const int tile = blockIdx.x;
    const int ty = tile / tiles_x, tx = tile - ty * tiles_x;
    const int i0 = ty * F_TILE_H, j0 = tx * F_TILE_W;
    const int m0 = blockIdx.y * BLOCK_M;
    const int lane = threadIdx.x & 63, wave = threadIdx.x >> 6;
    const int wm = wave / WN, wn = wave - wm * WN;
    const int li = lane & 31, h = lane >> 5;
    const int nst = a.Cin >> 4, hw = a.H * a.W;
    const int ca8 = a.bl_Ca >> 3, cb8 = (a.Cin - a.bl_Ca) >> 3;

    f32x16 acc[2][NT];
#pragma unroll
    for (int mt = 0; mt < 2; ++mt)
#pragma unroll
        for (int nt = 0; nt < NT; ++nt)
#pragma unroll
            for (int r = 0; r < 16; ++r) acc[mt][nt][r] = 0.f;

    const int tc = threadIdx.x >> 8, py = (threadIdx.x >> 4) & 15, px = threadIdx.x & 15;
    const bool inside = i0 + py < a.H && j0 + px < a.W;
    const size_t pix = inside ? (size_t)(i0 + py) * a.W + (j0 + px) : 0;
    const float m = inside ? a.bl_mask[(size_t)n * hw + pix] : 0.f;
    const float sc = a.bl_scale[(size_t)n * a.bl_scale_stride_n];
    const float ma = inside ? m : 0.f, mb = inside ? 1.0f - m : 0.f;
    const int wslot = tc * 256 + py * 16 + ((px + 2 * (py & 1)) & 15);
    auto src_of = [&](int st) -> const float4* {
        const int cc = 2 * st + tc;
        const float* base = cc < ca8 ? a.bl_a + ((size_t)n * ca8 + cc) * hw * 8 : a.bl_b + ((size_t)n * cb8 + (cc - ca8)) * hw * 8;
        return reinterpret_cast<const float4*>(base + pix * 8);
    };
    float4 raw[BL_DEPTH][2];
    auto issue = [&](int st, float4 (&r)[2]) {
        const float4* s4 = src_of(st < nst ? st : nst - 1); r[0] = s4[0]; r[1] = s4[1];
    };
    auto stage_patch = [&](int st, const float4 (&r)[2], uint4* P) {
        const float f = (2 * st + tc) < ca8 ? ma : mb;
        const float x[8] = {r[0].x, r[0].y, r[0].z, r[0].w, r[1].x, r[1].y, r[1].z, r[1].w};
        h8 hi, lo;
#pragma unroll
        for (int j = 0; j < 8; ++j) {
            const float t = as_rounded(x[j] * f * sc);
            const float cl = fminf(fmaxf(t, -65504.f), 65504.f);
            hi[j] = (_Float16)cl; lo[j] = (_Float16)(t - (float)hi[j]);
        }
        P[wslot] = *reinterpret_cast<uint4*>(&hi);
        P[512 + wslot] = *reinterpret_cast<uint4*>(&lo);
    };
    const uint4* WP = a.wp + (size_t)(threadIdx.x >> 7) * a.Cout + m0 + (threadIdx.x & 127);
    typedef unsigned u32x4 __attribute__((ext_vector_type(4)));
    u32x4 wraw[BL_DEPTH];
    auto issue_w = [&](int st, u32x4& r) { r = *reinterpret_cast<const u32x4*>(WP + (size_t)(st < nst ? st : nst - 1) * 4 * a.Cout); };
    uint4* const Abuf = lds + 2 * BL_PATCH;
    const int aoff = h * 256 + 64 * wm + li;
    const int prow = li >> 4, row0 = wn * 2 * NT;
    int boff[NT];
#pragma unroll
    for (int nt = 0; nt < NT; ++nt) boff[nt] = h * 256 + (row0 + nt * 2 + prow) * 16 + (li & 15);

#pragma unroll
    for (int d = 0; d < BL_DEPTH; ++d) { issue(d, raw[d]); issue_w(d, wraw[d]); }
    stage_patch(0, raw[0], lds);
    *reinterpret_cast<u32x4*>(Abuf + threadIdx.x) = wraw[0];
    issue(BL_DEPTH, raw[0]); issue_w(BL_DEPTH, wraw[0]);
    asm volatile("s_waitcnt lgkmcnt(0)" ::: "memory");
    __builtin_amdgcn_s_barrier();
    asm volatile("" ::: "memory");
    for (int s0 = 0; s0 < nst; s0 += BL_DEPTH) {
#pragma unroll
        for (int d = 0; d < BL_DEPTH; ++d) {
            const int s = s0 + d;
            {
                const uint4* P = lds + (d & 1) * BL_PATCH;
                const uint4* A = Abuf + (d & 1) * 512 + aoff;
                h8 ah[2], al[2];
#pragma unroll
                for (int mt = 0; mt < 2; ++mt) { const uint4 q0 = A[32 * mt], q1 = A[128 + 32 * mt]; ah[mt] = *reinterpret_cast<const h8*>(&q0); al[mt] = *reinterpret_cast<const h8*>(&q1); }
                h8 bh[NT], bl[NT];
#pragma unroll
                for (int nt = 0; nt < NT; ++nt) { const uint4 r0 = P[boff[nt]], r1 = P[512 + boff[nt]]; bh[nt] = *reinterpret_cast<const h8*>(&r0); bl[nt] = *reinterpret_cast<const h8*>(&r1); }
#pragma unroll
                for (int nt = 0; nt < NT; ++nt)
#pragma unroll
                    for (int mt = 0; mt < 2; ++mt) {
                        acc[mt][nt] = __builtin_amdgcn_mfma_f32_32x32x16_f16(al[mt], bh[nt], acc[mt][nt], 0, 0, 0);
                        acc[mt][nt] = __builtin_amdgcn_mfma_f32_32x32x16_f16(ah[mt], bl[nt], acc[mt][nt], 0, 0, 0);
                        acc[mt][nt] = __builtin_amdgcn_mfma_f32_32x32x16_f16(ah[mt], bh[nt], acc[mt][nt], 0, 0, 0);
                    }
                stage_patch(s + 1, raw[(d + 1) % BL_DEPTH], lds + ((d + 1) & 1) * BL_PATCH);
                *reinterpret_cast<u32x4*>(Abuf + ((d + 1) & 1) * 512 + threadIdx.x) = wraw[(d + 1) % BL_DEPTH];
                issue(s + 1 + BL_DEPTH, raw[(d + 1) % BL_DEPTH]); issue_w(s + 1 + BL_DEPTH, wraw[(d + 1) % BL_DEPTH]);
                asm volatile("s_waitcnt lgkmcnt(0)" ::: "memory");
                __builtin_amdgcn_s_barrier();
                asm volatile("" ::: "memory");
            }
        }
    }
    conv_epilogue<WN, NT>(a, ph, n, acc, i0, j0, m0, reinterpret_cast<float*>(lds));
}

static constexpr int U_TILE = 14;
static constexpr int U_WSTAGE = 9 * 2 * 2 * 32;
static constexpr int U_PW = 17, U_PPLANE = 320;
static constexpr int U_PATCH = 4 * U_PPLANE;
static constexpr int U_STAGE = U_PATCH + U_WSTAGE;
static constexpr int U_LDS_UINT4 = 2 * U_STAGE + 2;
static constexpr int U_ZERO = 2 * U_STAGE;


struct UpArgs {
    const uint4* x; size_t x_stride_n;
    const uint4* wp;
    const float* out_scale; const float* bias; const float* next_scale; size_t vec_stride_n;
    uint4* y; size_t y_stride_n;
    int Cin, Cout, H, W, tiles_x, ntiles, tiles_per_xcd;
    float clamp;
    unsigned long long* clk;
};

__global__ void sr_prepack_up_kernel(const float* __restrict__ w, int Cin, int Cout, const float* __restrict__ winv, uint4* __restrict__ out)
{
    const size_t e = (size_t)blockIdx.x * blockDim.x + threadIdx.x;
    const size_t total = (size_t)9 * (Cin / 8) * Cout * 2;
    if (e >= total) return;
    const int co = e & 31, hl = (e >> 5) & 1, hc = (e >> 6) & 1;
    const int t = (int)((e >> 7) % 9);
    const size_t r = (e >> 7) / 9;
    const int nst = Cin / 16;
    const int st = (int)(r % nst), cg = (int)(r / nst);
    const int cout = cg * 32 + co;
    h8 v8;
#pragma unroll
    for (int j = 0; j < 8; ++j) {
        const int ci = st * 16 + hc * 8 + j;
        _Float16 a, b; split1(w[((size_t)cout * Cin + ci) * 9 + t] * (1.0f / winv[cout]), a, b);
        v8[j] = hl ? b : a;
// ... 218 lines not shown
                    const int t = ky * 3 + kx, p = (ky & 1) * 2 + (kx & 1);
                    uint4 q0 = cur[t * 128 + aoff], q1 = cur[t * 128 + aoff + 32];
                    const h8 ah = *reinterpret_cast<h8*>(&q0), al = *reinterpret_cast<h8*>(&q1);
#pragma unroll
                    for (int nt = 0; nt < NTL; ++nt) {
                        acc[p][nt] = __builtin_amdgcn_mfma_f32_32x32x16_f16(al, bh[nt], acc[p][nt], 0, 0, 0);
                        acc[p][nt] = __builtin_amdgcn_mfma_f32_32x32x16_f16(ah, bl[nt], acc[p][nt], 0, 0, 0);
                        acc[p][nt] = __builtin_amdgcn_mfma_f32_32x32x16_f16(ah, bh[nt], acc[p][nt], 0, 0, 0);
                    }
                }
        }
    }
    if constexpr (MXIN) {
#pragma unroll
        for (int nt = 0; nt < NTL; ++nt) {
            acc[0][nt] = __builtin_amdgcn_mfma_scale_f32_32x32x64_f8f6f4(pa68, pb68[nt], acc[0][nt], 0, kMxFmtB, 0, kMxScaleA, 0, kMxScaleB);
            acc[1][nt] = __builtin_amdgcn_mfma_scale_f32_32x32x64_f8f6f4(pa17, pb17[nt], acc[1][nt], 0, kMxFmtB, 0, kMxScaleA, 0, kMxScaleB);
        }
    }

    R3D_STAMP(1);
    typedef float f2 __attribute__((ext_vector_type(2)));
    typedef _Float16 hh2 __attribute__((ext_vector_type(2)));
    float4* hls0 = reinterpret_cast<float4*>(lds);
    const int co0 = cg * 32;
    const float* D = a.out_scale + (size_t)n * a.vec_stride_n + co0;
    const float* Bv = a.bias + (size_t)n * a.vec_stride_n + co0;
    const float* NS = a.next_scale + (size_t)n * a.vec_stride_n + co0;
    const int OH = 2 * a.H, OW = 2 * a.W;
    const size_t oplane = (size_t)(a.Cout >> 3) * OH * OW;
    float4 dv4[4], bv4[4], nv4[4];
#pragma unroll
    for (int g = 0; g < 4; ++g) {
        dv4[g] = *reinterpret_cast<const float4*>(D + 8 * g + 4 * (tid & 1));
        bv4[g] = *reinterpret_cast<const float4*>(Bv + 8 * g + 4 * (tid & 1));
        nv4[g] = *reinterpret_cast<const float4*>(NS + 8 * g + 4 * (tid & 1));
    }
#pragma unroll
    for (int g = 0; g < 4; ++g)
        asm volatile("" :: "v"(dv4[g].x), "v"(dv4[g].w), "v"(bv4[g].x), "v"(bv4[g].w), "v"(nv4[g].x), "v"(nv4[g].w));
    __syncthreads();
    unsigned mxk_h[1024 / NTHR][2], mxk_l[1024 / NTHR][2];
#pragma unroll
    for (int k = 0; k < 1024 / NTHR; ++k) { mxk_h[k][0] = mxk_h[k][1] = 0u; mxk_l[k][0] = mxk_l[k][1] = 0u; }
#pragma unroll
    for (int g = 0; g < 4; ++g) {
        float4* hls = hls0 + (g & 1) * 2048;
#pragma unroll
        for (int pa = 0; pa < 2; ++pa)
#pragma unroll
            for (int nt = 0; nt < NTL; ++nt) {
                float hx[2][4];
#pragma unroll
                for (int r = 0; r < 4; ++r) {
                    const float t0 = acc[2 * pa][nt][4 * g + r], t1 = acc[2 * pa + 1][nt][4 * g + r];
                    const float ts = t0 + t1;
                    const float tsp1 = __builtin_bit_cast(float, __builtin_amdgcn_mov_dpp(__builtin_bit_cast(int, ts), 0x12F, 0xF, 0xF, true));
                    const float t0p1 = __builtin_bit_cast(float, __builtin_amdgcn_mov_dpp(__builtin_bit_cast(int, t0), 0x12F, 0xF, 0xF, true));
                    const float t1p1 = __builtin_bit_cast(float, __builtin_amdgcn_mov_dpp(__builtin_bit_cast(int, t1), 0x12F, 0xF, 0xF, true));
                    const float t0p2 = __builtin_bit_cast(float, __builtin_amdgcn_mov_dpp(__builtin_bit_cast(int, t0), 0x12E, 0xF, 0xF, true));
                    const float t1p2 = __builtin_bit_cast(float, __builtin_amdgcn_mov_dpp(__builtin_bit_cast(int, t1), 0x12E, 0xF, 0xF, true));
                    hx[0][r] = __builtin_fmaf(tsp1, 3.0f, t1 + t0p2);
                    hx[1][r] = __builtin_fmaf(t1p1 + t0p2, 3.0f, t0p1 + t1p2);
                }
                const int gy = row0 + nt * 2 + prow;
#pragma unroll
                for (int dx = 0; dx < 2; ++dx)
                    hls[((pa * 2 + h) * 16 + gy) * 32 + ((2 * pcol + dx + 8 * h) & 31)] = make_float4(hx[dx][0], hx[dx][1], hx[dx][2], hx[dx][3]);
            }
        __syncthreads();
        {
            const float4 b4 = bv4[g], n4 = nv4[g], d4 = dv4[g];
            const f2 ba = f2{b4.x, b4.y}, bb = f2{b4.z, b4.w};
            const f2 da = f2{d4.x, d4.y} * 0.0625f, db = f2{d4.z, d4.w} * 0.0625f;
            const float m = 1.4142135623730951f;
            const f2 ma = f2{n4.x, n4.y} * m, mb = f2{n4.z, n4.w} * m;
            uint4* d = a.y + (size_t)n * a.y_stride_n + (size_t)((co0 >> 3) + g) * OH * OW;
#pragma unroll
            for (int k = 0; k < 1024 / NTHR; ++k) {
                const int q = tid + NTHR * k;
                const int half = q & 1, oc = (q >> 1) & 31, rp = q >> 6;
                const bool live = rp < U_TILE && oc < 2 * U_TILE;
                f2 ha[5], hb[5];
#pragma unroll
                for (int rr = 0; rr < 5; ++rr) {
                    const int gyy = min(rp, U_TILE - 1) + ((rr + 1) >> 1);
                    const float4 t4 = hls[((((rr + 1) & 1) * 2 + half) * 16 + gyy) * 32 + ((oc + 8 * half) & 31)];
                    ha[rr] = f2{t4.x, t4.y}; hb[rr] = f2{t4.z, t4.w};
                }
#pragma unroll
                for (int dy = 0; dy < 2; ++dy) {
                    f2 va = ((ha[dy] + ha[dy + 3]) + (ha[dy + 1] + ha[dy + 2]) * 3.0f) * da + ba;
                    f2 vb = ((hb[dy] + hb[dy + 3]) + (hb[dy + 1] + hb[dy + 2]) * 3.0f) * db + bb;
                    va = __builtin_elementwise_max(va, va * 0.2f);
                    vb = __builtin_elementwise_max(vb, vb * 0.2f);
                    if constexpr (CLAMP) {
                        const f2 lim = f2{a.clamp, a.clamp} * 0.7071067811865476f;
                        va = __builtin_elementwise_min(__builtin_elementwise_max(va, -lim), lim);
                        vb = __builtin_elementwise_min(__builtin_elementwise_max(vb, -lim), lim);
                    }
                    va = va * ma;
                    vb = vb * mb;
                    asm("" : "+v"(va), "+v"(vb));
                    const hh2 hia = __builtin_convertvector(va, hh2), hib = __builtin_convertvector(vb, hh2);
                    const hh2 loa = __builtin_convertvector(va - __builtin_convertvector(hia, f2), hh2);
                    const hh2 lob = __builtin_convertvector(vb - __builtin_convertvector(hib, f2), hh2);
                    const uint2 hw = make_uint2(*reinterpret_cast<const unsigned*>(&hia), *reinterpret_cast<const unsigned*>(&hib));
                    const int oy = 2 * (i0 + rp) + dy, ox = 2 * j0 + oc;
                    if constexpr (MX) {
                        const f2 fha = __builtin_convertvector(hia, f2), fhb = __builtin_convertvector(hib, f2);
                        const f2 fla = va - fha, flb = vb - fhb;
                        const unsigned xh8 = pack4_x8(fha.x * kMxXh, fha.y * kMxXh, fhb.x * kMxXh, fhb.y * kMxXh);
                        const unsigned xl8 = pack4_x8(fla.x * kMxXl, fla.y * kMxXl, flb.x * kMxXl, flb.y * kMxXl);
                        if (!(g & 1)) { mxk_h[k][dy] = xh8; mxk_l[k][dy] = xl8; }
                        if (live && oy < OH && ox < OW) {
                            const size_t pix = (size_t)oy * OW + ox;
                            reinterpret_cast<uint2*>(d + pix)[half] = hw;
                            if (g & 1) {
                                uint4* rec = a.y + (size_t)n * a.y_stride_n + oplane + (size_t)((co0 >> 3) + (g & ~1)) * OH * OW + pix;
                                reinterpret_cast<uint2*>(rec)[half] = make_uint2(mxk_h[k][dy], xh8);
                                reinterpret_cast<uint2*>(rec + (size_t)OH * OW)[half] = make_uint2(mxk_l[k][dy], xl8);
                            }
                        }
                    } else {
                        const uint2 lw = make_uint2(*reinterpret_cast<const unsigned*>(&loa), *reinterpret_cast<const unsigned*>(&lob));
                        if (live && oy < OH && ox < OW) {
                            uint2* d2 = reinterpret_cast<uint2*>(d + (size_t)oy * OW + ox) + half;
                            d2[0] = hw;
                            d2[2 * oplane] = lw;
                        }
                    }
                }
            }
        }
    }
    R3D_STAMP(2);
    if (blockIdx.x == (gridDim.x >> 1) && blockIdx.y == 0 && threadIdx.x == 0) clk_end(kernarg_clk<UpArgs>());
#ifdef R3D_STAMPS
    asm volatile("s_waitcnt vmcnt(0)" ::: "memory");
    R3D_STAMP(3);
    R3D_STAMP_FLUSH(6, 1);
#endif
}
R3D_STAMP_READER(r3d_debug_stamps_sr)

__global__ void rgb_finalize_kernel(const float* __restrict__ img_prev, const float* __restrict__ partial, size_t part_stride_n,
                                    int nparts, const float* __restrict__ brgb, size_t vec_stride_n,
                                    float* __restrict__ img_out, uint8_t* __restrict__ img_u8, int H, int W, float clamp, int up)
{
    const int n = blockIdx.y;
    const int p = blockIdx.x * blockDim.x + threadIdx.x;
    if (p >= H * W) return;
    const int y = p / W, xx = p - y * W;
    const int Hh = H >> 1, Wh = W >> 1;
    const int ky = y >> 1, kx = xx >> 1;
    int r0, r1, c0, c1; float wy0, wy1, wx0, wx1;
    if (y & 1) { r0 = ky; r1 = ky + 1; wy0 = 0.75f; wy1 = 0.25f; } else { r0 = ky - 1; r1 = ky; wy0 = 0.25f; wy1 = 0.75f; }
    if (xx & 1) { c0 = kx; c1 = kx + 1; wx0 = 0.75f; wx1 = 0.25f; } else { c0 = kx - 1; c1 = kx; wx0 = 0.25f; wx1 = 0.75f; }
    const bool vr0 = r0 >= 0 && r0 < Hh, vr1 = r1 >= 0 && r1 < Hh, vc0 = c0 >= 0 && c0 < Wh, vc1 = c1 >= 0 && c1 < Wh;
    float rgb[3];
#pragma unroll
    for (int c = 0; c < 3; ++c) {
        float t = brgb[(size_t)n * vec_stride_n + c];
        for (int m = 0; m < nparts; ++m) t += partial[(size_t)n * part_stride_n + ((size_t)m * 3 + c) * H * W + p];
        if (clamp >= 0.f) t = fminf(fmaxf(t, -clamp), clamp);
        float upv;
        if (up) {
            const float* I = img_prev + ((size_t)n * 3 + c) * Hh * Wh;
            upv = 0.f;
            if (vr0 && vc0) upv += I[(size_t)r0 * Wh + c0] * (wy0 * wx0);
            if (vr0 && vc1) upv += I[(size_t)r0 * Wh + c1] * (wy0 * wx1);
            if (vr1 && vc0) upv += I[(size_t)r1 * Wh + c0] * (wy1 * wx0);
            if (vr1 && vc1) upv += I[(size_t)r1 * Wh + c1] * (wy1 * wx1);
        } else {
            upv = img_prev[((size_t)n * 3 + c) * H * W + p];
        }
        rgb[c] = upv + t;
        if (img_out) img_out[((size_t)n * 3 + c) * H * W + p] = rgb[c];
    }
    if (img_u8) {
        uint8_t* d = img_u8 + ((size_t)n * H * W + p) * 3;
#pragma unroll
        for (int c = 0; c < 3; ++c) d[c] = frame_u8(rgb[c]);
    }
}

__global__ void cb8_to_nchw2_kernel(const float* __restrict__ src, float* __restrict__ dst, int C, int HW)
{
    const int n = blockIdx.z, cb = blockIdx.y;
    const int p = blockIdx.x * blockDim.x + threadIdx.x;
    if (p >= HW) return;
    const float4* s = reinterpret_cast<const float4*>(src + (((size_t)n * (C / 8) + cb) * HW + p) * 8);
    const float4 a = s[0], b = s[1];
    float* d = dst + ((size_t)n * C + cb * 8) * HW + p;
    d[0] = a.x; d[(size_t)HW] = a.y; d[(size_t)2 * HW] = a.z; d[(size_t)3 * HW] = a.w;
    d[(size_t)4 * HW] = b.x; d[(size_t)5 * HW] = b.y; d[(size_t)6 * HW] = b.z; d[(size_t)7 * HW] = b.w;
}

__global__ void blend_cat_to_split_kernel(const float* __restrict__ a, int a_cb8, int Ca, const float* __restrict__ b, int b_cb8, int Cb,
                                          const float* __restrict__ mask, uint4* __restrict__ dst, int HW,
                                          const float* __restrict__ next_scale, size_t next_scale_stride_n, int mx)
{
    const int n = blockIdx.z, cb = blockIdx.y;
    const int p = blockIdx.x * blockDim.x + threadIdx.x;
    if (p >= HW) return;
    const bool first = cb < Ca / 8;
    const float* src = first ? a : b;
    const int C = first ? Ca : Cb, c8 = first ? cb : cb - Ca / 8, cb8 = first ? a_cb8 : b_cb8;
    const float m = mask[(size_t)n * HW + p];
    const float sc = first ? m : 1.0f - m;
    float v[8];
    if (cb8) {
        const float4* s4 = reinterpret_cast<const float4*>(src + (((size_t)n * (C / 8) + c8) * HW + p) * 8);
        const float4 x0 = s4[0], x1 = s4[1];
        v[0] = x0.x; v[1] = x0.y; v[2] = x0.z; v[3] = x0.w; v[4] = x1.x; v[5] = x1.y; v[6] = x1.z; v[7] = x1.w;
    } else {
        const float* s1 = src + ((size_t)n * C + c8 * 8) * HW + p;
#pragma unroll
        for (int c = 0; c < 8; ++c) v[c] = s1[(size_t)c * HW];
    }
    h8 hi, lo;
    float hf[8], lf[8];
#pragma unroll
    for (int c = 0; c < 8; ++c) {
        const float ns = next_scale ? next_scale[n * next_scale_stride_n + cb * 8 + c] : 1.f;
        const float t = as_rounded(v[c] * sc * ns);
        const float cl = fminf(fmaxf(t, -65504.f), 65504.f);
        hi[c] = (_Float16)cl; hf[c] = (float)hi[c]; lf[c] = t - hf[c]; lo[c] = (_Float16)lf[c];
    }
    const size_t plane = (size_t)((Ca + Cb) / 8) * HW;
    uint4* d = dst + (size_t)n * 2 * plane + (size_t)cb * HW + p;
    d[0] = *reinterpret_cast<uint4*>(&hi);
    if (mx) {
        unsigned* rec = reinterpret_cast<unsigned*>(dst + (size_t)n * 2 * plane + plane + (size_t)(cb & ~1) * HW + p) + (cb & 1);
        rec[0] = pack4_x8(hf[0] * kMxXh, hf[1] * kMxXh, hf[2] * kMxXh, hf[3] * kMxXh);
        rec[2] = pack4_x8(hf[4] * kMxXh, hf[5] * kMxXh, hf[6] * kMxXh, hf[7] * kMxXh);
        rec[4 * (size_t)HW] = pack4_x8(lf[0] * kMxXl, lf[1] * kMxXl, lf[2] * kMxXl, lf[3] * kMxXl);
        rec[4 * (size_t)HW + 2] = pack4_x8(lf[4] * kMxXl, lf[5] * kMxXl, lf[6] * kMxXl, lf[7] * kMxXl);
    } else {
        d[plane] = *reinterpret_cast<uint4*>(&lo);
    }
}

int blend_cat_to_split_f16x3(const float* a, int a_format, int Ca, const float* b, int b_format, int Cb, const float* mask,
                             int N, int H, int W, void* y_split, int y_format, const float* next_scale, size_t next_scale_stride, hipStream_t st)
{
    ProfScope ps(R3D_PROF_LAYOUT, st);
    hipLaunchKernelGGL(blend_cat_to_split_kernel, dim3((H * W + 255) / 256, (b ? Ca + Cb : Ca) / 8, N), dim3(256), 0, st,
                       a, a_format == R3D_FMT_CB8 ? 1 : 0, Ca, b, b_format == R3D_FMT_CB8 ? 1 : 0, Cb, mask,
                       reinterpret_cast<uint4*>(y_split), H * W, next_scale, next_scale_stride, y_format == R3D_FMT_SPLIT_MX ? 1 : 0);
    return check_launch("blend_cat_to_split");
}

__global__ void upsample2x_bilinear_kernel(const float* __restrict__ x, uint4* __restrict__ y_split, float* __restrict__ y_cb8,
                                           const float* __restrict__ next_scale, size_t next_scale_stride_n, int C, int H, int W, int mx)
{
    const int n = blockIdx.z, cb = blockIdx.y;
    const int OH = 2 * H, OW = 2 * W;
    const int p = blockIdx.x * blockDim.x + threadIdx.x;
    if (p >= OH * OW) return;
    const int oy = p / OW, ox = p - oy * OW;
    const float sh = OH > 1 ? (float)(H - 1) / (float)(OH - 1) : 0.f, sw = OW > 1 ? (float)(W - 1) / (float)(OW - 1) : 0.f;
    const float fy = sh * oy, fx = sw * ox;
    const int y0 = (int)fy, x0 = (int)fx;
    const int y1 = y0 + (y0 < H - 1 ? 1 : 0), x1 = x0 + (x0 < W - 1 ? 1 : 0);
    const float ly = fy - y0, lx = fx - x0, hy = 1.f - ly, hx = 1.f - lx;
    const float* X = x + ((size_t)n * (C / 8) + cb) * H * W * 8;
    float v[8];
#pragma unroll
    for (int half = 0; half < 2; ++half) {
        const float4 a = *reinterpret_cast<const float4*>(X + ((size_t)y0 * W + x0) * 8 + 4 * half);
        const float4 b = *reinterpret_cast<const float4*>(X + ((size_t)y0 * W + x1) * 8 + 4 * half);
        const float4 c = *reinterpret_cast<const float4*>(X + ((size_t)y1 * W + x0) * 8 + 4 * half);
        const float4 d = *reinterpret_cast<const float4*>(X + ((size_t)y1 * W + x1) * 8 + 4 * half);
        v[4 * half + 0] = hy * (hx * a.x + lx * b.x) + ly * (hx * c.x + lx * d.x);
        v[4 * half + 1] = hy * (hx * a.y + lx * b.y) + ly * (hx * c.y + lx * d.y);
        v[4 * half + 2] = hy * (hx * a.z + lx * b.z) + ly * (hx * c.z + lx * d.z);
        v[4 * half + 3] = hy * (hx * a.w + lx * b.w) + ly * (hx * c.w + lx * d.w);
    }
    if (y_cb8) {
        float4* d = reinterpret_cast<float4*>(y_cb8 + (((size_t)n * (C / 8) + cb) * OH * OW + p) * 8);
        d[0] = make_float4(v[0], v[1], v[2], v[3]); d[1] = make_float4(v[4], v[5], v[6], v[7]);
    }
    if (y_split) {
        h8 hi, lo;
        float hf[8], lf[8];
#pragma unroll
        for (int c = 0; c < 8; ++c) {
            const float sc = next_scale ? next_scale[n * next_scale_stride_n + cb * 8 + c] : 1.f;
            const float t = as_rounded(v[c] * sc);
            const float cl = fminf(fmaxf(t, -65504.f), 65504.f);
            hi[c] = (_Float16)cl; hf[c] = (float)hi[c]; lf[c] = t - hf[c]; lo[c] = (_Float16)lf[c];
        }
        const size_t plane = (size_t)(C / 8) * OH * OW, HW = (size_t)OH * OW;
        uint4* d = y_split + (size_t)n * 2 * plane + (size_t)cb * HW + p;
        d[0] = *reinterpret_cast<uint4*>(&hi);
        if (mx) {
            unsigned* rec = reinterpret_cast<unsigned*>(y_split + (size_t)n * 2 * plane + plane + (size_t)(cb & ~1) * HW + p) + (cb & 1);
            rec[0] = pack4_x8(hf[0] * kMxXh, hf[1] * kMxXh, hf[2] * kMxXh, hf[3] * kMxXh);
            rec[2] = pack4_x8(hf[4] * kMxXh, hf[5] * kMxXh, hf[6] * kMxXh, hf[7] * kMxXh);
            rec[4 * HW] = pack4_x8(lf[0] * kMxXl, lf[1] * kMxXl, lf[2] * kMxXl, lf[3] * kMxXl);
            rec[4 * HW + 2] = pack4_x8(lf[4] * kMxXl, lf[5] * kMxXl, lf[6] * kMxXl, lf[7] * kMxXl);
        } else {
            d[plane] = *reinterpret_cast<uint4*>(&lo);
        }
    }
}

int upsample2x_bilinear_f16x3(const float* x_cb8, int N, int C, int H, int W, void* y, int y_format,
                              const float* next_scale, size_t next_scale_stride, hipStream_t st)
{
    ProfScope ps(R3D_PROF_LAYOUT, st);
    hipLaunchKernelGGL(upsample2x_bilinear_kernel, dim3((4 * H * W + 255) / 256, C / 8, N), dim3(256), 0, st, x_cb8,
                       (y_format == R3D_FMT_SPLIT || y_format == R3D_FMT_SPLIT_MX) ? reinterpret_cast<uint4*>(y) : nullptr,
                       y_format == R3D_FMT_CB8 ? reinterpret_cast<float*>(y) : nullptr, next_scale, next_scale_stride, C, H, W,
                       y_format == R3D_FMT_SPLIT_MX ? 1 : 0);
    return check_launch("upsample2x_bilinear");
}

static constexpr float kSqrt2 = 1.4142135623730951f;

int sr_prepack_f16x3(int Cin, int Cout, const float* c0_w, const float* c1_w, void* prepacked, hipStream_t st, bool mx)
{
    float* out = reinterpret_cast<float*>(prepacked);
    const size_t m0 = (size_t)9 * (Cin / 8) * Cout, m1 = (size_t)9 * (Cout / 8) * Cout;
    const SrPackLayout P = sr_pack_layout(Cin, Cout);
    const ConvTail T = conv_tail_layout(Cout);
    float* tail0 = out + P.tail0;
    float* tail1 = out + P.tail1;
    hipLaunchKernelGGL(weight_row_stats_kernel, dim3(Cout), dim3(256), 0, st, c0_w, Cin * 9, Cout, Cout, tail0);
    hipLaunchKernelGGL(weight_row_stats_kernel, dim3(Cout), dim3(256), 0, st, c1_w, Cout * 9, Cout, Cout, tail1);
    hipLaunchKernelGGL(sr_prepack_f16_kernel, dim3((unsigned)((m0 + 255) / 256)), dim3(256), 0, st, c0_w, Cin, Cout, 9, Cin, Cout,
                       tail0 + T.winv, reinterpret_cast<uint4*>(out + P.c0));
    if (mx)
        hipLaunchKernelGGL(sr_prepack_mx_kernel, dim3((unsigned)((m1 / 2 + 255) / 256)), dim3(256), 0, st, c1_w, Cout, Cout, 9, Cout, Cout,
                           tail1 + T.winv, reinterpret_cast<uint4*>(out + P.c1));
    else
        hipLaunchKernelGGL(sr_prepack_f16_kernel, dim3((unsigned)((m1 + 255) / 256)), dim3(256), 0, st, c1_w, Cout, Cout, 9, Cout, Cout,
                           tail1 + T.winv, reinterpret_cast<uint4*>(out + P.c1));
    const size_t mu = (size_t)9 * (Cin / 8) * Cout * 2;
    hipLaunchKernelGGL(sr_prepack_up_kernel, dim3((unsigned)((mu + 255) / 256)), dim3(256), 0, st, c0_w, Cin, Cout, tail0 + T.winv,
                       reinterpret_cast<uint4*>(out + P.c0_up));
    if (mx) {
        hipLaunchKernelGGL(sr_prepack_up_mx_kernel, dim3((unsigned)((mu + 255) / 256)), dim3(256), 0, st, c0_w, Cin, Cout, tail0 + T.winv,
                           reinterpret_cast<uint4*>(out + P.c0_up_mx));
        if ((Cin & 15) == 0)
            hipLaunchKernelGGL(sr_prepack_mx_kernel, dim3((unsigned)((m0 / 2 + 255) / 256)), dim3(256), 0, st, c0_w, Cin, Cout, 9, Cin, Cout,
                               tail0 + T.winv, reinterpret_cast<uint4*>(out + P.c0_mx));
    }
    {
        const size_t mw = (size_t)(Cout >> 7) * (Cout >> 4) * 8 * 3 * 2 * 32;
        hipLaunchKernelGGL(sr_prepack_wino_kernel, dim3((unsigned)((mw + 255) / 256)), dim3(256), 0, st, c1_w, Cout, Cout, Cout, Cout, tail1 + T.winv,
                           reinterpret_cast<uint4*>(out + P.c1_wino), mx ? 1 : 0);
    }
    return check_launch("sr_block_prepack");
}

static_assert(SR_TILE == F_TILE_H && SR_TILE == F_TILE_W && SR_UP_TILE == U_TILE, "sr_conv_variant / sr_block_variants (r3d_sr_launch.h) size the grids by these tiles");

static void launch_conv2(Conv2Args& a, const SrVariantChoice& v, hipStream_t st)
{
    a.clk = prof_clock_slot(R3D_PROF_CONV);
    a.order = v.order;
    const dim3 grid(v.gx, v.gy, v.gz);
    switch (v.variant) {
    case SR_VAR_WINO: hipLaunchKernelGGL(conv_wino_f16x3_kernel<false>, grid, dim3(512), 0, st, a); break;
    case SR_VAR_WINO_MX: hipLaunchKernelGGL(conv_wino_f16x3_kernel<true>, grid, dim3(512), 0, st, a); break;
    case SR_VAR_ROWS8: hipLaunchKernelGGL(conv_mfma_f16x3_rows8_kernel<false>, grid, dim3(512), 0, st, a); break;
    case SR_VAR_ROWS8_MX: hipLaunchKernelGGL(conv_mfma_f16x3_rows8_kernel<true>, grid, dim3(512), 0, st, a); break;
    case SR_VAR_CONV1X1: hipLaunchKernelGGL((conv1x1_mfma_f16x3_kernel<4, 2, 4>), grid, dim3(512), 0, st, a); break;
    case SR_VAR_DIRECT16_MX: hipLaunchKernelGGL((conv_mfma_f16x3_kernel<4, 2, 4, true>), grid, dim3(512), 0, st, a); break;
    default: hipLaunchKernelGGL((conv_mfma_f16x3_kernel<4, 2, 4>), grid, dim3(512), 0, st, a); break;
    }
}

static const uint4* split_input(const void* x, int x_format, const float* in_scale, size_t in_scale_stride, void* xin, int Ci, int Cin, int N, int H, int W, hipStream_t st)
{
    if (x_format == R3D_FMT_SPLIT || x_format == R3D_FMT_SPLIT_MX) return reinterpret_cast<const uint4*>(x);
    ProfScope ps(R3D_PROF_LAYOUT, st);
    hipLaunchKernelGGL(to_split_kernel, dim3((H * W + 255) / 256, Ci / 8, N), dim3(256), 0, st,
                       reinterpret_cast<const float*>(x), x_format == R3D_FMT_CB8 ? 1 : 0, in_scale, in_scale_stride, reinterpret_cast<uint4*>(xin), Ci, Cin, H * W);
    return reinterpret_cast<const uint4*>(xin);
}

static void (*const kUpconv[2][2][2])(UpArgs) = {
    {{upconv_fir_f16x3_kernel<false, false, false>, upconv_fir_f16x3_kernel<false, false, true>}, {upconv_fir_f16x3_kernel<false, true, false>, upconv_fir_f16x3_kernel<false, true, true>}},
    {{upconv_fir_f16x3_kernel<true, false, false>, upconv_fir_f16x3_kernel<true, false, true>}, {upconv_fir_f16x3_kernel<true, true, false>, upconv_fir_f16x3_kernel<true, true, true>}}};

int sr_block_forward_f16x3(const void* prepacked, const void* styles, int N, int Cin, int Cout, int Hin, int Win, int up,
                           const void* x, int x_format, const float* img, float clamp,
                           void* x_out, int x_out_format, const float* next_scale, size_t next_scale_stride,
                           float* img_out, uint8_t* img_u8, float* x_absmax, void* workspace, hipStream_t st, bool mx)
{
    const SrStyleLayout L = sr_style_layout(Cin, Cout);
    const float* pk = reinterpret_cast<const float*>(styles);
    const float* wpk = reinterpret_cast<const float*>(prepacked);
    const SrPackLayout P = sr_pack_layout(Cin, Cout);
    const int OH = up ? 2 * Hin : Hin, OW = up ? 2 * Win : Win;
    const SrWorkspaceLayout WS = sr_workspace_layout(N, Cin, Cout, Hin, Win);
    char* wsb = reinterpret_cast<char*>(workspace);
    uint4* y0 = reinterpret_cast<uint4*>(wsb + WS.y0);
    float* rgbp = reinterpret_cast<float*>(wsb + WS.rgbp);

    const bool mx_in = x_format == R3D_FMT_SPLIT_MX;
    const uint4* xs = split_input(x, x_format, pk + L.s0f, L.total, wsb + WS.xin, Cin, Cin, N, Hin, Win, st);
    SrVariantChoice v[2];
    sr_block_variants(N, Cin, Cout, Hin, Win, up, x_format, mx, clamp, sr_wino_mode(), v);
    const bool wino1 = v[1].wino();
    const bool mx0 = mx && !wino1;
    if (up) {
        UpArgs u = {};
        u.x = xs; u.x_stride_n = (size_t)Cin / 8 * Hin * Win * 2;
        u.wp = reinterpret_cast<const uint4*>(wpk + (mx_in ? P.c0_up_mx : P.c0_up));
        u.out_scale = pk + L.d0f; u.bias = pk + L.b0; u.next_scale = pk + L.s1f; u.vec_stride_n = L.total;
        u.y = y0; u.y_stride_n = (size_t)Cout / 8 * OH * OW * 2;
        u.Cin = Cin; u.Cout = Cout; u.H = Hin; u.W = Win;
        u.tiles_x = (Win + U_TILE - 1) / U_TILE;
        u.ntiles = v[0].tiles;
        u.tiles_per_xcd = (u.ntiles + 7) / 8;
        u.clamp = clamp;
        u.clk = prof_clock_slot(R3D_PROF_UPCONV);
        ProfScope ps(R3D_PROF_UPCONV, st);
        const dim3 ugrid(v[0].gx, v[0].gy);
        hipLaunchKernelGGL(kUpconv[(v[0].bits & SR_UP_CLAMP) != 0][(v[0].bits & SR_UP_MX) != 0][(v[0].bits & SR_UP_MXIN) != 0], ugrid, dim3(256), 0, st, u);
    } else {
        SrConvCall c0 = sr_conv_call("sr_block_forward", N, Cin, Cout, OH, OW, 3, 1, 0.2f, kSqrt2, clamp, y0, mx0 ? R3D_FMT_SPLIT_MX : R3D_FMT_SPLIT,
                                     pk + L.s1f, L.total, nullptr, st);
        c0.bias = pk + L.b0;
        Conv2Args a = {};
        c0.fill(a, Cin, Cout, pk + L.d0f, L.total, L.total);
        a.x = xs; a.x_stride_n = (size_t)Cin / 8 * Hin * Win * 2;
        a.wp = reinterpret_cast<const uint4*>(wpk + (mx_in ? P.c0_mx : P.c0));
        ProfScope ps(R3D_PROF_CONV, st);
        launch_conv2(a, v[0], st);
    }
    {
        SrConvCall c1 = sr_conv_call("sr_block_forward", N, Cout, Cout, OH, OW, 3, 1, 0.2f, kSqrt2, clamp, x_out, x_out ? x_out_format : R3D_FMT_NONE,
                                     next_scale, next_scale_stride, x_absmax, st);
        c1.bias = pk + L.b1;
        Conv2Args a = {};
        c1.fill(a, Cout, Cout, pk + L.d1f, L.total, L.total);
        a.x = y0; a.x_stride_n = (size_t)Cout / 8 * OH * OW * 2;
        a.wp = reinterpret_cast<const uint4*>(wpk + (wino1 ? P.c1_wino : P.c1));
        a.wrgb = pk + L.wrgb; a.wrgb_stride_n = L.total; a.rgb_partial = rgbp; a.rgbp_stride_n = (size_t)(Cout / 64) * 3 * OH * OW;
        ProfScope ps(R3D_PROF_CONV, st);
        launch_conv2(a, v[1], st);
    }
    {
        ProfScope ps(R3D_PROF_TORGB, st);
        hipLaunchKernelGGL(rgb_finalize_kernel, dim3((OH * OW + 255) / 256, N), dim3(256), 0, st, img, rgbp,
                           (size_t)(Cout / 64) * 3 * OH * OW, Cout / 64, pk + L.brgb, L.total, img_out, img_u8, OH, OW, clamp, up);
    }
    return check_launch("sr_block_forward(f16x3)");
}

size_t conv_prepacked_bytes_f16x3(int Cin, int Cout, int ksize) { return conv_pack_layout(Cin, Cout, ksize).total * sizeof(float); }

int conv_prepack_f16x3(const float* w, int Cin, int Cout, int ksize, void* prepacked, hipStream_t st)
{
    const ConvPackLayout P = conv_pack_layout(Cin, Cout, ksize);
    const int Ci = P.Ci, Co = P.Co, nt = ksize * ksize;
    const size_t m = (size_t)nt * (Ci / 8) * Co;
    float* out = reinterpret_cast<float*>(prepacked);
    float* tail = out + P.tail;
    ProfScope ps(R3D_PROF_PACK, st);
    hipLaunchKernelGGL(weight_row_stats_kernel, dim3(Co), dim3(256), 0, st, w, Cin * nt, Cout, Co, tail);
    hipLaunchKernelGGL(sr_prepack_f16_kernel, dim3((unsigned)((m + 255) / 256)), dim3(256), 0, st, w, Cin, Cout, nt, Ci, Co,
                       tail + conv_tail_layout(Co).winv, reinterpret_cast<uint4*>(out + P.w));
    if (ksize == 3) {
        hipLaunchKernelGGL(sr_prepack_mx_kernel, dim3((unsigned)((m / 2 + 255) / 256)), dim3(256), 0, st, w, Cin, Cout, nt, Ci, Co,
                           tail + conv_tail_layout(Co).winv, reinterpret_cast<uint4*>(out + P.w_mx));
        const size_t mw = (size_t)(Co >> 7) * (Ci >> 4) * 8 * 3 * 2 * 32;
        hipLaunchKernelGGL(sr_prepack_wino_kernel, dim3((unsigned)((mw + 255) / 256)), dim3(256), 0, st, w, Cin, Cout, Ci, Co, tail + conv_tail_layout(Co).winv,
                           reinterpret_cast<uint4*>(out + P.w_wino), 0);
    }
    return check_launch("conv_prepack");
}

size_t conv_workspace_bytes_f16x3(int N, int Cin, int H, int W) { return align256((size_t)N * conv_pack_layout(Cin, 1, 1).Ci * H * W * 4) + 256; }

int conv_forward_f16x3(const SrConvCall& c)
{
    const ConvPackLayout P = conv_pack_layout(c.Cin, c.Cout, c.ksize);
    const ConvScales S = conv_scales_layout(P.Ci, P.Co);
    const float* scales = reinterpret_cast<const float*>(c.scales);
    const bool mx_in = c.x_format == R3D_FMT_SPLIT_MX;
    Conv2Args a = {};
    c.fill(a, P.Ci, P.Co, scales + S.out_vec, S.total, 0);
    a.x = split_input(c.x, c.x_format, scales + S.in_vec, S.total, c.workspace, P.Ci, c.Cin, c.N, c.H, c.W, c.stream);
    a.x_stride_n = (size_t)P.Ci / 8 * c.H * c.W * 2;
    if (const ConvCat* cat = c.cat) {
        a.y_split_stride_n = (size_t)cat->C_total / 8 * c.H * c.W * 2; a.y_cat_chunks = cat->C_total / 8; a.y_cat_off = cat->chan_off / 8;
        a.y_mask = cat->mask; a.y_mask_invert = cat->mask_invert;
        if (c.next_scale) a.next_scale = c.next_scale + cat->chan_off;
    }
    const SrVariantChoice v = sr_conv_variant(c.ksize, P.Ci, P.Co, c.H, c.W, c.N, mx_in, false, sr_wino_mode());
    a.wp = reinterpret_cast<const uint4*>(reinterpret_cast<const float*>(c.prepacked) + (mx_in ? P.w_mx : v.wino() ? P.w_wino : P.w));
    ProfScope ps(R3D_PROF_CONV, c.stream);
    launch_conv2(a, v, c.stream);
    return check_launch("conv_forward");
}

int conv_forward_blend_f16x3(const SrConvCall& c)
{
    const ConvPackLayout P = conv_pack_layout(c.Cin, c.Cout, 1);
    const ConvScales S = conv_scales_layout(P.Ci, P.Co);
    const float* scales = reinterpret_cast<const float*>(c.scales);
    Conv2Args a = {};
    c.fill(a, P.Ci, P.Co, scales + S.out_vec, S.total, 0);
    a.wp = reinterpret_cast<const uint4*>(reinterpret_cast<const float*>(c.prepacked) + P.w);
    a.bl_a = c.bl_a; a.bl_b = c.bl_b; a.bl_mask = c.bl_mask; a.bl_scale = scales + S.in_vec; a.bl_scale_stride_n = S.total; a.bl_Ca = c.Ca;
    ProfScope ps(R3D_PROF_CONV, c.stream);
    const SrVariantChoice v = sr_blend_variant(P.Co, c.H, c.W, c.N);
    hipLaunchKernelGGL(conv1x1_blend_f16x3_kernel, dim3(v.gx, v.gy, v.gz), dim3(512), 0, c.stream, a);
    return check_launch("conv_forward_blend");
}

}
```

real3dportrait_amd/csrc/r3d_sr_launch.h:

```cpp
#pragma once
#include "r3d_sr_common.h"

namespace r3d {

inline int check_index32(const char* what, size_t channels, size_t H, size_t W)
{
    if (channels * H * W < ((size_t)1 << 32)) return R3D_OK;
    set_error("%s: activation of %zu elements per sample exceeds the 32-bit index range", what, channels * H * W);
    return R3D_ERR_INVALID_ARG;
}

struct SrConvCall {
    const char* what = "";
    int N = 0, Cin = 0, Cout = 0, H = 0, W = 0, ksize = 0;
    const void* prepacked = nullptr; const void* scales = nullptr; const float* bias = nullptr;
    const void* x = nullptr; int x_format = R3D_FMT_SPLIT;
    bool blend = false;
    const float* bl_a = nullptr; const float* bl_b = nullptr; const float* bl_mask = nullptr; int Ca = 0, Cb = 0;
    void* y = nullptr; int y_format = R3D_FMT_NONE;
    const float* next_scale = nullptr; size_t next_scale_stride = 0;
    const ConvCat* cat = nullptr;
    float* y_absmax = nullptr;
    int act = 0; float act_slope = 0.f, act_gain = 1.f, clamp = -1.f;
    void* workspace = nullptr; size_t workspace_bytes = 0;
    hipStream_t stream = nullptr;

    bool x_is_split() const { return x_format == R3D_FMT_SPLIT || x_format == R3D_FMT_SPLIT_MX; }

    template <class Args>
    void fill(Args& a, int Ci, int Co, const float* out_scale, size_t out_scale_stride, size_t bias_stride) const
    {
        a.out_scale = out_scale; a.out_scale_stride_n = out_scale_stride; a.bias = bias; a.bias_stride_n = bias_stride;
        a.OH = H; a.OW = W;
        if (y_format == R3D_FMT_CB8) { a.y_f32 = reinterpret_cast<float*>(y); a.y_f32_stride_n = (size_t)Cout * H * W; }
        else if (y_format == R3D_FMT_NCHW) { a.y_nchw = reinterpret_cast<float*>(y); a.y_nchw_stride_n = (size_t)Cout * H * W; }
        else if (y_format == R3D_FMT_SPLIT || y_format == R3D_FMT_SPLIT_MX) {
            a.y_split = reinterpret_cast<uint4*>(y); a.y_split_stride_n = (size_t)Cout / 8 * H * W * 2;
            a.next_scale = next_scale; a.next_scale_stride_n = next_scale_stride;
            a.y_split_mx = y_format == R3D_FMT_SPLIT_MX ? 1 : 0;
        }
        a.y_absmax = reinterpret_cast<unsigned*>(y_absmax);
        a.Cin = Ci; a.Cout = Co; a.CoutReal = Cout; a.H = H; a.W = W; a.nphase = 1;
        a.act = act; a.act_slope = act_slope; a.act_gain = act_gain; a.clamp = clamp;
        if (ksize == 3) sr_fill_conv3x3_phase(a.ph, H, W);
        else sr_fill_conv1x1_phase(a.ph, H, W);
    }
};

inline SrConvCall sr_conv_call(const char* what, int N, int Cin, int Cout, int H, int W, int ksize, int act, float act_slope, float act_gain,
                               float clamp, void* y, int y_format, const float* next_scale, size_t next_scale_stride, float* y_absmax, hipStream_t st)
{
    SrConvCall c;
    c.what = what; c.N = N; c.Cin = Cin; c.Cout = Cout; c.H = H; c.W = W; c.ksize = ksize;
    c.act = act; c.act_slope = act_slope; c.act_gain = act_gain; c.clamp = clamp;
    c.y = y; c.y_format = y_format; c.next_scale = next_scale; c.next_scale_stride = next_scale_stride; c.y_absmax = y_absmax; c.stream = st;
    return c;
}

inline int check(const SrConvCall& c)
{
    const bool no_input = c.blend ? (!c.bl_a || !c.bl_b || !c.bl_mask || c.Ca <= 0 || c.Cb <= 0) : !c.x;
    if (!c.prepacked || !c.scales || !c.y || no_input || (c.cat && !c.cat->mask) || c.N <= 0 || c.Cin <= 0 || c.Cout <= 0 || c.H <= 0 || c.W <= 0)
        { set_error("%s: bad argument", c.what); return R3D_ERR_INVALID_ARG; }
    if (c.cat && c.ksize != 1)
        { set_error("%s: ksize %d: only the 1x1 conv kernel carries the concatenation epilogue", c.what, c.ksize); return R3D_ERR_INVALID_ARG; }
    if (c.ksize != 1 && c.ksize != 3) { set_error("%s: bad argument (ksize %d is not 1 or 3)", c.what, c.ksize); return R3D_ERR_INVALID_ARG; }
    if (c.cat && c.y_format != R3D_FMT_SPLIT && c.y_format != R3D_FMT_SPLIT_MX)
        { set_error("%s: y_format %d must be SPLIT or SPLIT_MX", c.what, c.y_format); return R3D_ERR_INVALID_ARG; }
    if (c.cat && ((c.Cout & 15) || (c.cat->chan_off & 15) || (c.cat->C_total & 15) || c.cat->chan_off < 0 || c.cat->chan_off + c.Cout > c.cat->C_total)) {
        set_error("%s: Cout %d, chan_off %d, C_total %d must be multiples of 16 with chan_off + Cout <= C_total", c.what, c.Cout, c.cat->chan_off, c.cat->C_total);
        return R3D_ERR_INVALID_ARG;
    }
    if (c.blend && ((c.Ca & 7) || (c.Cb & 7) || ((c.Ca + c.Cb) & 63)))
        { set_error("%s: Ca %d and Cb %d must be multiples of 8 and their sum a multiple of 64", c.what, c.Ca, c.Cb); return R3D_ERR_INVALID_ARG; }
    if (c.x_format < R3D_FMT_NCHW || c.x_format > R3D_FMT_SPLIT_MX || (c.x_format != R3D_FMT_NCHW && (c.Cin & 15)) || (c.x_format == R3D_FMT_SPLIT_MX && c.ksize != 3)) {
        set_error("%s: unsupported input (format %d, Cin %d, ksize %d): blocked formats need Cin %% 16 == 0, SPLIT_MX a 3x3 conv", c.what, c.x_format, c.Cin, c.ksize);
        return R3D_ERR_INVALID_ARG;
    }
    if (c.y_format < R3D_FMT_NCHW || c.y_format > R3D_FMT_SPLIT_MX || (c.Cout & 3) || (c.y_format != R3D_FMT_NCHW && (c.Cout & 7)) || (c.y_format == R3D_FMT_SPLIT_MX && (c.Cout & 15))) {
        set_error("%s: unsupported output (format %d, Cout %d): Cout must be a multiple of 4, blocked formats need Cout %% 8 == 0, SPLIT_MX Cout %% 16 == 0", c.what, c.y_format, c.Cout);
        return R3D_ERR_INVALID_ARG;
    }
    const int cout = c.cat ? c.cat->C_total : c.Cout;
    if (int rc = check_index32(c.what, (size_t)((c.Cin > cout ? c.Cin : cout) + BLOCK_M), c.H, c.W)) return rc;
    if (!c.blend && !c.x_is_split() && (!c.workspace || c.workspace_bytes < conv_workspace_bytes_f16x3(c.N, c.Cin, c.H, c.W)))
        { set_error("%s: workspace too small", c.what); return R3D_ERR_WORKSPACE; }
    return R3D_OK;
}

enum SrVariant {
    SR_VAR_DIRECT16 = 0,
    SR_VAR_DIRECT16_MX = 1,
    SR_VAR_ROWS8 = 2,
    SR_VAR_ROWS8_MX = 3,
    SR_VAR_WINO = 4,
    SR_VAR_WINO_MX = 5,
    SR_VAR_CONV1X1 = 6,
    SR_VAR_BLEND1X1 = 7,
    SR_VAR_UPCONV = 8,
};
enum { SR_UP_CLAMP = 4, SR_UP_MX = 2, SR_UP_MXIN = 1 };

static constexpr int SR_TILE = 16, SR_TILE_ROWS8 = 8, SR_UP_TILE = 14, SR_UP_COUTS = 32;
static constexpr size_t SR_ROWS8_MAX_BLOCKS = 256;

struct SrVariantChoice {
    int variant = -1, bits = 0;
    int order = 0;
    unsigned gx = 0, gy = 0, gz = 1;
    int tiles = 0;
    bool wino() const { return variant == SR_VAR_WINO || variant == SR_VAR_WINO_MX; }
};

inline int sr_wino_mode() { static const int v = getenv("R3D_CONV_WINO") ? atoi(getenv("R3D_CONV_WINO")) : 3; return v; }

inline bool sr_use_wino(int wino_mode, int Ci, int Co, int H, int W, bool mx)
{
    const int m = wino_mode;
    return (m == 1 || (m == 2 && mx) || (m == 3 && !mx)) && (H & 15) == 0 && (W & 15) == 0 && (Ci & 15) == 0 && (Co % BLOCK_M) == 0 &&
           (size_t)Ci * H * W * 4 < ((size_t)1 << 31) && (size_t)48 * Ci * Co < ((size_t)1 << 31);
}

inline int sr_tiles_of(int H, int W, int rows = SR_TILE) { return ((W + SR_TILE - 1) / SR_TILE) * ((H + rows - 1) / rows); }

inline SrVariantChoice sr_conv_variant(int ksize, int Ci, int Co, int H, int W, int N, bool operand_mx, bool layer_mx, int wino_mode)
{
    SrVariantChoice c;
    c.tiles = sr_tiles_of(H, W);
    c.gy = (unsigned)(Co / BLOCK_M); c.gz = (unsigned)N;
    if (ksize == 3 && !operand_mx && sr_use_wino(wino_mode, Ci, Co, H, W, layer_mx)) c.variant = layer_mx ? SR_VAR_WINO_MX : SR_VAR_WINO;
    else if (ksize == 3 && (size_t)c.tiles * c.gy * c.gz <= SR_ROWS8_MAX_BLOCKS) {
        c.variant = operand_mx ? SR_VAR_ROWS8_MX : SR_VAR_ROWS8;
        c.tiles = sr_tiles_of(H, W, SR_TILE_ROWS8);
    }
    else c.variant = ksize == 1 ? SR_VAR_CONV1X1 : operand_mx ? SR_VAR_DIRECT16_MX : SR_VAR_DIRECT16;
    c.gx = (unsigned)c.tiles;
    c.order = (c.tiles & 7) == 0 ? 2 : 0;
    return c;
}

inline SrVariantChoice sr_blend_variant(int Co, int H, int W, int N)
{
    SrVariantChoice c;
    c.variant = SR_VAR_BLEND1X1; c.tiles = sr_tiles_of(H, W);
    c.gx = (unsigned)c.tiles; c.gy = (unsigned)(Co / BLOCK_M); c.gz = (unsigned)N;
    return c;
}

inline void sr_block_variants(int N, int Cin, int Cout, int Hin, int Win, int up, int x_format, bool mx, float clamp, int wino_mode, SrVariantChoice v[2])
{
    const int OH = up ? 2 * Hin : Hin, OW = up ? 2 * Win : Win;
    const bool mx_in = x_format == R3D_FMT_SPLIT_MX;
    v[1] = sr_conv_variant(3, Cout, Cout, OH, OW, N, mx && !sr_use_wino(wino_mode, Cout, Cout, OH, OW, mx), mx, wino_mode);
    const bool mx0 = mx && !v[1].wino();
    if (!up) { v[0] = sr_conv_variant(3, Cin, Cout, OH, OW, N, mx_in, mx, 0); return; }
    SrVariantChoice c;
    c.variant = SR_VAR_UPCONV;
    c.bits = (clamp >= 0.f ? SR_UP_CLAMP : 0) | (mx0 ? SR_UP_MX : 0) | (mx_in ? SR_UP_MXIN : 0);
    c.tiles = ((Win + SR_UP_TILE - 1) / SR_UP_TILE) * ((Hin + SR_UP_TILE - 1) / SR_UP_TILE);
    c.gx = (unsigned)(8 * ((c.tiles + 7) / 8) * (Cout / SR_UP_COUTS)); c.gy = (unsigned)N;
    v[0] = c;
}

int conv_forward_f16x3(const SrConvCall& c);
int conv_forward_blend_f16x3(const SrConvCall& c);

}
```

real3dportrait_amd/superresolution.py:

```python
import ctypes
import os

import numpy as np
import torch
import torch.nn as nn

from . import _lib
from ._state import Derived, _DeviceBuffers
from .sr_activation import (FMT, MAX_DEPTH, SPLIT_FORMATS, _keep_tags, _tag, as_input, bound_of, empty, fmt_of, logical_shape, out_target,
                            tag_bound, tag_split)
from .volumetric_rendering import _FC, _f32c

_SQRT2 = float(np.sqrt(2.0))


def _setup_filter():
    f = torch.tensor([1.0, 3.0, 3.0, 1.0])
    f = torch.outer(f, f)
    return f / f.sum()


class _BoundMeter:

    def __init__(self):
# ... 51 lines not shown
        assert t.is_cuda and t.dtype == torch.float32 and t.numel() >= N and t.is_contiguous()
    ptrs = (ctypes.c_void_p * max(1, len(ext)))(*[t.data_ptr() for t in ext])
    zptrs = (ctypes.c_void_p * max(1, len(zero)))(*[t.data_ptr() for t in zero])
    _lib.call("r3d_chain_fold", ctypes.cast(arr, ctypes.c_void_p), len(ops), N, ctypes.cast(ptrs, ctypes.c_void_p), len(ext),
              ctypes.cast(zptrs, ctypes.c_void_p), len(zero))


class SynthesisLayer(nn.Module):

    def __init__(self, in_channels, out_channels, w_dim, resolution, kernel_size=3, up=1, use_noise=True,
                 activation="lrelu", resample_filter=(1, 3, 3, 1), conv_clamp=None, channels_last=False, **_):
        super().__init__()
        assert kernel_size == 3 and activation == "lrelu" and tuple(resample_filter) == (1, 3, 3, 1)
        self.in_channels, self.out_channels, self.w_dim = in_channels, out_channels, w_dim
        self.resolution, self.up, self.use_noise, self.conv_clamp = resolution, up, use_noise, conv_clamp
        self.register_buffer("resample_filter", _setup_filter())
        self.affine = _FC(w_dim, in_channels, bias_init=1.0)
        self.weight = nn.Parameter(torch.randn(out_channels, in_channels, kernel_size, kernel_size))
        if use_noise:
            self.register_buffer("noise_const", torch.randn(resolution, resolution))
            self.noise_strength = nn.Parameter(torch.zeros([]))
        self.bias = nn.Parameter(torch.zeros(out_channels))


class ToRGBLayer(nn.Module):

    def __init__(self, in_channels, out_channels, w_dim, kernel_size=1, conv_clamp=None, channels_last=False):
        super().__init__()
        assert kernel_size == 1 and out_channels == 3
        self.in_channels, self.out_channels, self.w_dim, self.conv_clamp = in_channels, out_channels, w_dim, conv_clamp
        self.affine = _FC(w_dim, in_channels, bias_init=1.0)
        self.weight = nn.Parameter(torch.randn(out_channels, in_channels, kernel_size, kernel_size))
        self.bias = nn.Parameter(torch.zeros(out_channels))
        self.weight_gain = 1 / np.sqrt(in_channels * (kernel_size ** 2))


class SynthesisBlock(_DeviceBuffers, nn.Module):

    _UP = 1

    def __init__(self, in_channels, out_channels, w_dim, resolution, img_channels, is_last, architecture="skip",
                 resample_filter=(1, 3, 3, 1), conv_clamp=256, use_fp16=False, fp16_channels_last=False,
                 fused_modconv_default=True, **layer_kwargs):
        super().__init__()
        if in_channels == 0 or architecture != "skip" or img_channels != 3:
            raise NotImplementedError("HIP SynthesisBlock covers the SR configuration only "
                                      "(in_channels != 0, architecture 'skip', 3 image channels)")
        if use_fp16:
            raise NotImplementedError("use_fp16 SR blocks: the Real3D shells run SR in fp32 "
                                      "(img2plane_baseline.py:102); fp16 is not built")
        self.in_channels, self.out_channels, self.w_dim = in_channels, out_channels, w_dim
        self.resolution, self.img_channels, self.is_last, self.architecture = resolution, img_channels, is_last, architecture
        self.use_fp16 = False
        self.fused_modconv_default = fused_modconv_default
        self.register_buffer("resample_filter", _setup_filter())
        self.num_conv, self.num_torgb = 2, 1
        self.conv0 = SynthesisLayer(in_channels, out_channels, w_dim=w_dim, resolution=resolution, up=2 if self._UP else 1,
                                    conv_clamp=conv_clamp, **layer_kwargs)
        self.conv1 = SynthesisLayer(out_channels, out_channels, w_dim=w_dim, resolution=resolution,
                                    conv_clamp=conv_clamp, **layer_kwargs)
        self.torgb = ToRGBLayer(out_channels, img_channels, w_dim=w_dim, conv_clamp=conv_clamp)
        self.conv_clamp = conv_clamp
        self.out_format = "nchw"
        self.return_x = True
        self.precision = os.environ.get("R3D_SR_PRECISION", DEFAULT_SR_PRECISION)
        self._prepacked = None
        self._prepack_state = Derived()
        self._styles = None
        self._styles_state = Derived()
        self._workspace = None
        self._meter = _BoundMeter()
        self._depth_in = 0
        self._fold_epoch = 0

    _FMT = FMT
    _PREC = {"f32": 0, "f16x3": 1, "f16mx": 2}

    def _prec(self):
        return self._PREC[self.precision]

    def wants_mx(self):
        return self._prec() == 2 and self.in_channels % 16 == 0 and (_MX_UPCONV or not self._UP)

    def _clamp(self):
        return -1.0 if self.conv_clamp is None else float(self.conv_clamp)

    def prepare(self, ws, dev=None, ws_key=None):
        Cin, Cout = self.in_channels, self.out_channels
        c0, c1, tr = self.conv0, self.conv1, self.torgb
        params = (c0.weight, c0.bias, c0.affine.weight, c0.affine.bias, c1.weight, c1.bias, c1.affine.weight, c1.affine.bias,
                  tr.weight, tr.bias, tr.affine.weight, tr.affine.bias)
        keep = [_f32c(t) for t in params]
        dev = keep[0].device if dev is None else dev
        prec = self._prec()
        N = ws.shape[0]

        def prepack():
            pre = self._buf("_prepacked", _lib.call("r3d_sr_block_prepacked_bytes", Cin, Cout), dev)
            _lib.call("r3d_sr_block_prepack", Cin, Cout, keep[0], keep[4], pre, prec)

        def styles():
            w = _f32c(ws)
            assert w.shape[1] == self.num_conv + self.num_torgb and w.shape[2] == self.w_dim, w.shape
            buf = self._buf("_styles", _lib.call("r3d_sr_block_styles_bytes", N, Cin, Cout), dev)
            _lib.call("r3d_sr_block_styles", w, N, self.w_dim, Cin, Cout, *keep, buf)

        self._prepack_state.get([c0.weight, c1.weight], prepack, (dev, prec))
        self._styles_state.get([ws if ws_key is None else ws_key, *params], styles, (N, dev))
        return self._prepacked, self._styles

    def styles_stride(self):
        return _lib.call("r3d_sr_block_styles_bytes", 1, self.in_channels, self.out_channels) // 4

    def in_scale(self):
        return self._styles.view(torch.float32), self.styles_stride()

    def chain_op(self, src_a=-1, src_b=_lib.CHAIN_SRC_NONE, tail=False):
        self._fold_epoch += 1
        return _lib.ChainOp(kind=_lib.CHAIN_SR_BLOCK_TAIL if tail else _lib.CHAIN_SR_BLOCK, Cin=self.in_channels, Cout=self.out_channels, ksize=3, act=1, gain=_SQRT2,
                            clamp=self._clamp(), src_a=src_a, src_b=src_b, scales=self._styles.data_ptr(), prepacked=None, bias=None)

    def bound_out(self, N):
        off = _lib.call("r3d_sr_block_bound_offset", self.in_channels, self.out_channels)
        return self._styles.view(torch.float32).as_strided((N,), (self.styles_stride(),), off).contiguous()

    def forward(self, x, img, ws, force_fp32=False, fused_modconv=None, update_emas=False, noise_mode="random",
                _prepared=None, _next=None, _folded=False, _u8_out=None, _need_img=True, _x_absmax=None, _out_format=None, _return_x=None,
                **layer_kwargs):
        if noise_mode == "random" or (noise_mode == "const" and
                                      (float(self.conv0.noise_strength) != 0 or float(self.conv1.noise_strength) != 0)):
            raise NotImplementedError("noise_mode=%r: the inference path uses 'none' "
                                      "(img2plane_baseline.py:113)" % noise_mode)
        if img is None:
            raise NotImplementedError("img=None (first block of a synthesis network) is not on the SR path")
        x, x_fmt, presplit = as_input(x, self)
        _folded = _folded or presplit
        img = _f32c(img)
        N = img.shape[0]
        Hin, Win = img.shape[-2], img.shape[-1]
        Cin, Cout = self.in_channels, self.out_channels
        dev = img.device
        prec = self._prec()
        pre, styles = _prepared if _prepared is not None else self.prepare(ws, dev)
        if prec >= 1 and not _folded:
            bx, self._depth_in = bound_of(x, self._meter, layers=2 if prec == 1 else MAX_DEPTH + 1)
            chain_fold([self.chain_op(-1)], N, [bx])
        need = _lib.call("r3d_sr_block_workspace_bytes", N, Cin, Cout, Hin, Win)
        work = self._buf("_workspace", need, dev)
        OH, OW = (2 * Hin, 2 * Win) if self._UP else (Hin, Win)
        img_out = torch.empty(N, 3, OH, OW, device=dev, dtype=torch.float32) if (_need_img or _u8_out is None) else None
        want_x = self.return_x if _return_x is None else _return_x
        out_fmt, next_scale, next_stride = out_target((self.out_format if _out_format is None else _out_format) if want_x else "none", prec == 2, _next)
        x_out = None if out_fmt == "none" else empty(out_fmt, N, Cout, OH, OW, dev)
        _lib.call("r3d_sr_block_forward", pre, styles, N, Cin, Cout, Hin, Win, self._UP, x, FMT[x_fmt], img, self._clamp(), x_out, FMT[out_fmt],
                  next_scale, next_stride, img_out, _u8_out, _x_absmax, prec, work, need)
        if out_fmt in SPLIT_FORMATS:
            tag_split(x_out, out_fmt, _next)
        elif x_out is not None and prec >= 1:
            tag_bound(x_out, self.bound_out(N), self._depth_in + 2)
        return x_out, img_out

    def num_layers(self):
        return 2

    def fold_for_input(self, N, dev, bounds, ws=None, depth=0):
        assert ws is not None, "folding a SynthesisBlock needs its ws"
        return _fold_single(self, N, dev, bounds, ws=ws, depth=depth)


class SynthesisBlockNoUp(SynthesisBlock):
    _UP = 0


class Conv2d(_DeviceBuffers, nn.Module):

    def __init__(self, in_channels, out_channels, kernel_size, stride=1, padding=0, bias=True):
        super().__init__()
        k = kernel_size[0] if isinstance(kernel_size, (tuple, list)) else kernel_size
        s = stride[0] if isinstance(stride, (tuple, list)) else stride
        pd = padding[0] if isinstance(padding, (tuple, list)) else padding
        if k not in (1, 3) or s != 1 or pd != k // 2:
            raise NotImplementedError("HIP Conv2d covers k in {1,3}, stride 1, padding k//2 (got k=%r s=%r p=%r)" % (k, s, pd))
        if out_channels % 4:
            raise NotImplementedError("HIP Conv2d needs out_channels %% 4 == 0 (got %d)" % out_channels)
        self.in_channels, self.out_channels, self.kernel_size, self.stride, self.padding = in_channels, out_channels, (k, k), (1, 1), (pd, pd)
        ref = nn.Conv2d(in_channels, out_channels, k, 1, pd, bias=bias)
        self.weight = nn.Parameter(ref.weight.detach().clone())
        self.bias = nn.Parameter(ref.bias.detach().clone()) if bias else None
        self._prepacked = None
        self._prepack_state = Derived()
        self._workspace = None
        self._scales = None
        self._bias32 = None
        self._meter = _BoundMeter()
        self._depth_in = 0
        self.precision = os.environ.get("R3D_SR_PRECISION", DEFAULT_SR_PRECISION)

    def wants_mx(self):
        return self.precision == "f16mx" and self.kernel_size[0] == 3 and self.in_channels % 16 == 0

    def prepare(self, N, dev):
        Cin, Cout, k = self.in_channels, self.out_channels, self.kernel_size[0]

        def prepack():
            pre = self._buf("_prepacked", _lib.call("r3d_conv_prepacked_bytes", Cin, Cout, k), dev)
            _lib.call("r3d_conv_prepack", _f32c(self.weight), Cin, Cout, k, pre)

        self._prepack_state.get([self.weight], prepack, dev)
        self._bias32 = _f32c(self.bias) if self.bias is not None else None
        self._buf("_scales", _lib.call("r3d_conv_scales_bytes", N, Cin, Cout), dev)

    def in_scale(self):
        N1 = _lib.call("r3d_conv_scales_bytes", 1, self.in_channels, self.out_channels) // 4
        return self._scales.view(torch.float32), N1

    def chain_op(self, src_a=-1, src_b=_lib.CHAIN_SRC_NONE, negative_slope=None):
        return _lib.ChainOp(kind=_lib.CHAIN_CONV, Cin=self.in_channels, Cout=self.out_channels, ksize=self.kernel_size[0],
                            act=0 if negative_slope is None else 1, gain=1.0, clamp=-1.0, src_a=src_a, src_b=src_b,
                            scales=self._scales.data_ptr(), prepacked=self._prepacked.data_ptr(),
                            bias=None if self._bias32 is None else self._bias32.data_ptr())

    def bound_out(self, N):
        off = _lib.call("r3d_conv_scales_bound_offset", self.in_channels, self.out_channels)
        return self._scales.view(torch.float32).as_strided((N,), (self.in_scale()[1],), off).contiguous()

    def can_blend(self, a, b):
        return (self.kernel_size[0] == 1 and fmt_of(a) == "cb8" and fmt_of(b) == "cb8"
                and logical_shape(a)[1] + logical_shape(b)[1] == self.in_channels and self.in_channels % 64 == 0)

    def forward(self, x, negative_slope=None, out_format="nchw", _next=None, _folded=False, _y_absmax=None, _blend=None):
        if _blend is not None:
            a, b, mask = _blend
            assert _folded and self.can_blend(a, b), "fused blend: a folded 1x1 conv over two 'cb8' sources"
            (N, Ca, H, W), (Nb, Cb, Hb, Wb) = logical_shape(a), logical_shape(b)
            a, b, mask = a.contiguous(), b.contiguous(), _f32c(mask)
            assert (Nb, Hb, Wb) == (N, H, W) and tuple(mask.shape) == (N, 1, H, W), (a.shape, b.shape, mask.shape)
            out_format, next_scale, next_stride = out_target(out_format, True, _next)
            y = empty(out_format, N, self.out_channels, H, W, a.device)
            _lib.call("r3d_conv_forward_blend", self._prepacked, self._scales, self._bias32, N, Ca, Cb, self.out_channels, H, W, a, b, mask,
                      0 if negative_slope is None else 1, float(negative_slope or 0.0), 1.0, -1.0, y, FMT[out_format], next_scale, next_stride,
                      _y_absmax)
            return self._tagged(y, out_format, _next, N)
        N, C, H, W = logical_shape(x)
        x, x_fmt, presplit = as_input(x, self)
        _folded = _folded or presplit
        Cin, Cout, k = self.in_channels, self.out_channels, self.kernel_size[0]
        if C != Cin:
            raise RuntimeError("Conv2d: expected input with %d channels, got %d" % (Cin, C))
        dev = x.device
        if not _folded:
            self.prepare(N, dev)
            bx, self._depth_in = bound_of(x, self._meter, layers=1)
            chain_fold([self.chain_op(-1, negative_slope=negative_slope)], N, [bx])
        need = _lib.call("r3d_conv_workspace_bytes", N, Cin, H, W)
        work = self._buf("_workspace", need, dev) if not presplit else None
        out_format, next_scale, next_stride = out_target(out_format, True, _next)
        y = empty(out_format, N, Cout, H, W, dev)
        act = 0 if negative_slope is None else 1
        _lib.call("r3d_conv_forward", self._prepacked, self._scales, self._bias32, N, Cin, Cout, H, W, k, x, FMT[x_fmt], act,
                  float(negative_slope or 0.0), 1.0, -1.0, y, FMT[out_format], next_scale, next_stride, _y_absmax,
                  work, need if work is not None else 0)
        return self._tagged(y, out_format, _next, N)

    def _tagged(self, y, out_format, _next, N):
        if out_format in SPLIT_FORMATS:
            return tag_split(y, out_format, _next)
        return tag_bound(y, self.bound_out(N), self._depth_in + 1)

    def num_layers(self):
        return 1

    def fold_for_input(self, N, dev, bounds, ws=None, depth=0):
        return _fold_single(self, N, dev, bounds, depth=depth)

    def forward_cat(self, x, dst, chan_off, mask, mask_invert, _next, negative_slope=None):
        x_fmt = fmt_of(x)
        assert x_fmt in ("nchw", "cb8") and self.kernel_size[0] == 1, "forward_cat: a 1x1 conv over an fp32 input"
        N, C, H, W = logical_shape(x)
        x = _f32c(x)
        Nd, C_total, Hd, Wd = logical_shape(dst)
        assert C == self.in_channels and fmt_of(dst) in SPLIT_FORMATS and (Nd, Hd, Wd) == (N, H, W) and tuple(mask.shape) == (N, 1, H, W)
        need = _lib.call("r3d_conv_workspace_bytes", N, C, H, W)
        work = self._buf("_workspace", need, x.device)
        ns, stride = _next.in_scale()
        _lib.call("r3d_conv_forward_cat", self._prepacked, self._scales, self._bias32, N, C, self.out_channels, H, W, 1, x, FMT[x_fmt],
                  0 if negative_slope is None else 1, float(negative_slope or 0.0), 1.0, -1.0, dst, FMT[fmt_of(dst)], C_total, chan_off,
                  _f32c(mask), int(bool(mask_invert)), ns, stride, work, need)
        return dst


def upsample2x_bilinear(x, out_format="split", _next=None):
    assert fmt_of(x) == "cb8", "upsample2x_bilinear takes the 'cb8' output of a Conv2d"
    bx, dx = getattr(x, "_r3d_bound", None), int(getattr(x, "_r3d_depth", 0))
    N, C, H, W = logical_shape(x)
    x = x.contiguous()
    out_format, next_scale, next_stride = out_target(out_format, True, _next)
    y = empty(out_format, N, C, 2 * H, 2 * W, x.device)
    _lib.call("r3d_upsample2x_bilinear", x, N, C, H, W, y, FMT[out_format], next_scale, next_stride)
    if out_format in SPLIT_FORMATS:
        tag_split(y, out_format, _next)
    elif bx is not None:
        tag_bound(y, bx, dx)
    return y


def resize_bilinear(x, size, antialias=True):
    x = _f32c(x)
    N, C, H, W = x.shape
# ... 213 lines not shown
```

Baseline: 1685.

## Fuse SR image tail (rgb+upsample+u8) into last block's conv1 epilogue

```diff
diff --git a/include/r3d_hip_sr_tail.h b/include/r3d_hip_sr_tail.h
--- /dev/null
+++ b/include/r3d_hip_sr_tail.h
@@ -0,0 +1,22 @@
+#ifndef R3D_HIP_SR_TAIL_H
+#define R3D_HIP_SR_TAIL_H
+
+#include "r3d_hip.h"
+
+#ifdef __cplusplus
+extern "C" {
+#endif
+
+int r3d_sr_block_forward_fused(const void* prepacked, const void* styles, int N, int Cin, int Cout, int Hin, int Win, int up,
+                               const void* x, int x_format, const float* img, float clamp,
+                               void* x_out, int x_out_format, const float* next_scale, size_t next_scale_stride,
+                               float* img_out, uint8_t* img_u8, float* x_absmax, int precision,
+                               void* workspace, size_t workspace_bytes, r3d_stream_t stream);
+
+int r3d_debug_sr_block_image_tail(int N, int Cin, int Cout, int Hin, int Win, int up, int x_format, int precision, float clamp, int* out);
+
+#ifdef __cplusplus
+}
+#endif
+
+#endif
diff --git a/real3dportrait_amd/_lib.py b/real3dportrait_amd/_lib.py
--- a/real3dportrait_amd/_lib.py
+++ b/real3dportrait_amd/_lib.py
@@ -133,6 +133,11 @@
     "r3d_a2m_wn_layer": (c_int, [F, F, c_int, c_int, c_int, c_int, c_int, F, F, F, F, F, c_int, c_int, F, F, S]),
     "r3d_a2m_pitch_embed": (c_int, [F, c_int, c_int, F, c_int, c_int, I32, F, S]),
 }
+SR_TAIL_SIGNATURES = {
+    "r3d_sr_block_forward_fused": (c_int, [V, V, c_int, c_int, c_int, c_int, c_int, c_int, V, c_int, F, c_float, V, c_int, F, c_size_t, F, U8, F, c_int, V,
+                                           c_size_t, S]),
+    "r3d_debug_sr_block_image_tail": (c_int, [c_int, c_int, c_int, c_int, c_int, c_int, c_int, c_int, c_float, ctypes.POINTER(c_int)]),
+}
 _FIT_COMMON = [F, F, F, c_int, c_int, c_int, F, F, c_int, c_int, c_float, c_float, c_float, ctypes.POINTER(c_float)]
 FIT_SIGNATURES = {
     "r3d_fit_workspace_bytes": (c_size_t, [c_int, c_int, c_int, c_int]),
@@ -197,7 +202,7 @@
         lib = ctypes.CDLL(LIB_PATH)
     except OSError as e:
         raise RuntimeError("real3dportrait_amd: cannot load %s: %s" % (LIB_PATH, e))
-    for name, (res, params) in list(SIGNATURES.items()) + list(AUDIO_SIGNATURES.items()) + list(FIT_SIGNATURES.items()):
+    for name, (res, params) in list(SIGNATURES.items()) + list(AUDIO_SIGNATURES.items()) + list(FIT_SIGNATURES.items()) + list(SR_TAIL_SIGNATURES.items()):
         try:
             fn = getattr(lib, name)
         except AttributeError:
diff --git a/real3dportrait_amd/csrc/r3d_sr.hip b/real3dportrait_amd/csrc/r3d_sr.hip
--- a/real3dportrait_amd/csrc/r3d_sr.hip
+++ b/real3dportrait_amd/csrc/r3d_sr.hip
@@ -1,4 +1,5 @@
 #include "r3d_sr_launch.h"
+#include "../../include/r3d_hip_sr_tail.h"
 
 namespace r3d {
 
@@ -574,21 +575,22 @@
     return check_launch("sr_block_styles");
 }
 
-extern "C" int r3d_sr_block_forward(const void* prepacked, const void* styles, int N, int Cin, int Cout, int Hin, int Win, int up,
-                                    const void* x, int x_format, const float* img, float clamp,
-                                    void* x_out, int x_out_format, const float* next_scale, size_t next_scale_stride,
-                                    float* img_out, uint8_t* img_u8, float* x_absmax, int precision,
-                                    void* workspace, size_t workspace_bytes, r3d_stream_t stream)
-{
-    if (precision < R3D_SR_F32 || precision > R3D_SR_F16MX) { set_error("sr_block_forward: unknown precision %d", precision); return R3D_ERR_INVALID_ARG; }
-    if ((img_u8 || x_absmax) && precision == R3D_SR_F32) { set_error("sr_block_forward: the fused uint8 output / x_absmax need R3D_SR_F16X3"); return R3D_ERR_INVALID_ARG; }
+static int sr_block_forward_entry(const char* what, bool fuse_tail, const void* prepacked, const void* styles, int N, int Cin, int Cout, int Hin, int Win, int up,
+                                  const void* x, int x_format, const float* img, float clamp,
+                                  void* x_out, int x_out_format, const float* next_scale, size_t next_scale_stride,
+                                  float* img_out, uint8_t* img_u8, float* x_absmax, int precision,
+                                  void* workspace, size_t workspace_bytes, r3d_stream_t stream)
+{
+    if (precision < R3D_SR_F32 || precision > R3D_SR_F16MX) { set_error("%s: unknown precision %d", what, precision); return R3D_ERR_INVALID_ARG; }
+    if ((img_u8 || x_absmax) && precision == R3D_SR_F32) { set_error("%s: the fused uint8 output / x_absmax need R3D_SR_F16X3", what); return R3D_ERR_INVALID_ARG; }
     if (!prepacked || !styles || !x || !img || (!img_out && !img_u8) || N <= 0 || Hin <= 0 || Win <= 0 || (Cin & 15) || (Cout % BLOCK_M) || (up != 0 && up != 1)) {
-        set_error("sr_block_forward: bad argument"); return R3D_ERR_INVALID_ARG;
-    }
-    if (!up && precision == R3D_SR_F32) { set_error("sr_block_forward: up=0 (SynthesisBlockNoUp) needs R3D_SR_F16X3"); return R3D_ERR_INVALID_ARG; }
-    if (int rc = r3d::check_index32("sr_block_forward", (size_t)(Cin > Cout ? Cin : Cout), (size_t)(up ? 2 : 1) * Hin, (size_t)(up ? 2 : 1) * Win)) return rc;
+        set_error("%s: bad argument", what); return R3D_ERR_INVALID_ARG;
+    }
+    if (fuse_tail && precision == R3D_SR_F32) { set_error("%s: the image tail is fused into the f16x3 / f16mx conv kernels (precision %d)", what, precision); return R3D_ERR_INVALID_ARG; }
+    if (!up && precision == R3D_SR_F32) { set_error("%s: up=0 (SynthesisBlockNoUp) needs R3D_SR_F16X3", what); return R3D_ERR_INVALID_ARG; }
+    if (int rc = r3d::check_index32(what, (size_t)(Cin > Cout ? Cin : Cout), (size_t)(up ? 2 : 1) * Hin, (size_t)(up ? 2 : 1) * Win)) return rc;
     if (!workspace || workspace_bytes < r3d_sr_block_workspace_bytes(N, Cin, Cout, Hin, Win)) {
-        set_error("sr_block_forward: workspace too small"); return R3D_ERR_WORKSPACE;
+        set_error("%s: workspace too small", what); return R3D_ERR_WORKSPACE;
     }
     if (!x_out) x_out_format = R3D_FMT_NONE;
     const bool f16 = precision != R3D_SR_F32;
@@ -597,13 +599,13 @@
         (!f16 && (x_format >= R3D_FMT_SPLIT || x_out_format >= R3D_FMT_SPLIT)) ||
         ((x_format == R3D_FMT_SPLIT_MX || x_out_format == R3D_FMT_SPLIT_MX) && !mxp) ||
         (x_out_format >= R3D_FMT_SPLIT && !next_scale)) {
-        set_error("sr_block_forward: unsupported activation format (x %d, x_out %d, precision %d)", x_format, x_out_format, precision);
+        set_error("%s: unsupported activation format (x %d, x_out %d, precision %d)", what, x_format, x_out_format, precision);
         return R3D_ERR_INVALID_ARG;
     }
     hipStream_t st = (hipStream_t)stream;
     if (f16)
         return sr_block_forward_f16x3(prepacked, styles, N, Cin, Cout, Hin, Win, up, x, x_format, img, clamp, x_out, x_out_format,
-                                      next_scale, next_scale_stride, img_out, img_u8, x_absmax, workspace, st, precision == R3D_SR_F16MX);
+                                      next_scale, next_scale_stride, img_out, img_u8, x_absmax, workspace, st, precision == R3D_SR_F16MX, fuse_tail);
 
     const SrStyleLayout L = sr_style_layout(Cin, Cout);
     const float* pk = reinterpret_cast<const float*>(styles);
@@ -672,6 +674,26 @@
     return check_launch("sr_block_forward");
 }
 
+extern "C" int r3d_sr_block_forward(const void* prepacked, const void* styles, int N, int Cin, int Cout, int Hin, int Win, int up,
+                                    const void* x, int x_format, const float* img, float clamp,
+                                    void* x_out, int x_out_format, const float* next_scale, size_t next_scale_stride,
+                                    float* img_out, uint8_t* img_u8, float* x_absmax, int precision,
+                                    void* workspace, size_t workspace_bytes, r3d_stream_t stream)
+{
+    return sr_block_forward_entry("sr_block_forward", false, prepacked, styles, N, Cin, Cout, Hin, Win, up, x, x_format, img, clamp, x_out, x_out_format,
+                                  next_scale, next_scale_stride, img_out, img_u8, x_absmax, precision, workspace, workspace_bytes, stream);
+}
+
+extern "C" int r3d_sr_block_forward_fused(const void* prepacked, const void* styles, int N, int Cin, int Cout, int Hin, int Win, int up,
+                                          const void* x, int x_format, const float* img, float clamp,
+                                          void* x_out, int x_out_format, const float* next_scale, size_t next_scale_stride,
+                                          float* img_out, uint8_t* img_u8, float* x_absmax, int precision,
+                                          void* workspace, size_t workspace_bytes, r3d_stream_t stream)
+{
+    return sr_block_forward_entry("sr_block_forward_fused", true, prepacked, styles, N, Cin, Cout, Hin, Win, up, x, x_format, img, clamp, x_out, x_out_format,
+                                  next_scale, next_scale_stride, img_out, img_u8, x_absmax, precision, workspace, workspace_bytes, stream);
+}
+
 extern "C" size_t r3d_conv_prepacked_bytes(int Cin, int Cout, int ksize) { return r3d::conv_prepacked_bytes_f16x3(Cin, Cout, ksize); }
 extern "C" size_t r3d_conv_workspace_bytes(int N, int Cin, int H, int W) { return r3d::conv_workspace_bytes_f16x3(N, Cin, H, W); }
 extern "C" size_t r3d_conv_scales_bytes(int N, int Cin, int Cout)
@@ -824,6 +846,17 @@
     return R3D_OK;
 }
 
+extern "C" int r3d_debug_sr_block_image_tail(int N, int Cin, int Cout, int Hin, int Win, int up, int x_format, int precision, float clamp, int* out)
+{
+    using namespace r3d;
+    int v12[12];
+    if (int rc = r3d_debug_sr_block_variants(N, Cin, Cout, Hin, Win, up, x_format, precision, clamp, out ? v12 : nullptr)) return rc;
+    SrVariantChoice v[2];
+    sr_block_variants(N, Cin, Cout, Hin, Win, up, x_format, precision == R3D_SR_F16MX, clamp, sr_wino_mode(), v);
+    out[0] = sr_image_tail_fuses(v[1], Cout) ? 1 : 0; out[1] = v[1].variant;
+    return R3D_OK;
+}
+
 extern "C" int r3d_upsample2x_bilinear(const float* x_cb8, int N, int C, int H, int W, void* y, int y_format,
                                        const float* next_scale, size_t next_scale_stride, r3d_stream_t stream)
 {
diff --git a/real3dportrait_amd/csrc/r3d_sr_common.h b/real3dportrait_amd/csrc/r3d_sr_common.h
--- a/real3dportrait_amd/csrc/r3d_sr_common.h
+++ b/real3dportrait_amd/csrc/r3d_sr_common.h
@@ -128,7 +128,8 @@
 int sr_block_forward_f16x3(const void* prepacked, const void* styles, int N, int Cin, int Cout, int Hin, int Win, int up,
                            const void* x, int x_format, const float* img, float clamp,
                            void* x_out, int x_out_format, const float* next_scale, size_t next_scale_stride,
-                           float* img_out, uint8_t* img_u8, float* x_absmax, void* workspace, hipStream_t st, bool mx);
+                           float* img_out, uint8_t* img_u8, float* x_absmax, void* workspace, hipStream_t st, bool mx,
+                           bool fuse_tail = false);
 
 size_t conv_prepacked_bytes_f16x3(int Cin, int Cout, int ksize);
 int conv_prepack_f16x3(const float* w, int Cin, int Cout, int ksize, void* prepacked, hipStream_t st);
diff --git a/real3dportrait_amd/csrc/r3d_sr_f16x3.hip b/real3dportrait_amd/csrc/r3d_sr_f16x3.hip
--- a/real3dportrait_amd/csrc/r3d_sr_f16x3.hip
+++ b/real3dportrait_amd/csrc/r3d_sr_f16x3.hip
@@ -196,8 +196,53 @@
     ConvPhase ph[4];
 };
 
+struct RgbTaps { int r0, r1, c0, c1; float wy0, wy1, wx0, wx1; bool vr0, vr1, vc0, vc1; };
+__device__ __forceinline__ RgbTaps rgb_taps(int y, int xx, int Hh, int Wh)
+{
+    RgbTaps k;
+    const int ky = y >> 1, kx = xx >> 1;
+    if (y & 1) { k.r0 = ky; k.r1 = ky + 1; k.wy0 = 0.75f; k.wy1 = 0.25f; } else { k.r0 = ky - 1; k.r1 = ky; k.wy0 = 0.25f; k.wy1 = 0.75f; }
+    if (xx & 1) { k.c0 = kx; k.c1 = kx + 1; k.wx0 = 0.75f; k.wx1 = 0.25f; } else { k.c0 = kx - 1; k.c1 = kx; k.wx0 = 0.25f; k.wx1 = 0.75f; }
+    k.vr0 = k.r0 >= 0 && k.r0 < Hh; k.vr1 = k.r1 >= 0 && k.r1 < Hh; k.vc0 = k.c0 >= 0 && k.c0 < Wh; k.vc1 = k.c1 >= 0 && k.c1 < Wh;
+    return k;
+}
+template <class Prev>
+__device__ __forceinline__ float rgb_pixel(float t, float clamp, int up, int y, int xx, const RgbTaps& k, Prev prev)
+{
+#pragma clang fp contract(off)
+    if (clamp >= 0.f) t = fminf(fmaxf(t, -clamp), clamp);
+    float upv;
+    if (up) {
+        upv = 0.f;
+        if (k.vr0 && k.vc0) upv = __builtin_fmaf(prev(k.r0, k.c0), k.wy0 * k.wx0, upv);
+        if (k.vr0 && k.vc1) upv = __builtin_fmaf(prev(k.r0, k.c1), k.wy0 * k.wx1, upv);
+        if (k.vr1 && k.vc0) upv = __builtin_fmaf(prev(k.r1, k.c0), k.wy1 * k.wx0, upv);
+        if (k.vr1 && k.vc1) upv = __builtin_fmaf(prev(k.r1, k.c1), k.wy1 * k.wx1, upv);
+    } else {
+        upv = prev(y, xx);
+    }
+    return upv + t;
+}
+
+struct ImgTailArgs {
+    const float* brgb; size_t brgb_stride_n;
+    const float* img_prev;
+    float* img_out; uint8_t* img_u8;
+    int up;
+};
+static constexpr int IT_COLS_UP = F_TILE_W / 2 + 2;
+static_assert(alignof(Conv2Args) == 8 && alignof(ImgTailArgs) == 8, "kernarg layout of (Conv2Args, ImgTailArgs)");
+__device__ __forceinline__ const __attribute__((address_space(4))) ImgTailArgs* kernarg_img_tail()
+{
+    typedef const __attribute__((address_space(4))) char* KA;
+    KA ap = (KA)__builtin_amdgcn_kernarg_segment_ptr();
+    asm volatile("" : "+s"(ap));
+    return (const __attribute__((address_space(4))) ImgTailArgs*)(ap + sizeof(Conv2Args));
+}
+static constexpr int EV_VECS = 6;
+
 static constexpr int EV_STRIDE = BLOCK_M;
-template <int WN, int NT, bool WINO = false, bool CAT = false>
+template <int WN, int NT, bool WINO = false, bool CAT = false, bool FIN = false>
 __device__ __forceinline__ void conv_epilogue(const Conv2Args& a, const ConvPhase& ph, int n, f32x16 (&acc)[2][NT],
                                               int i0, int j0, int m0, float* ev)
 {
@@ -208,9 +253,26 @@
     const int prow = li >> 4, pcol = ((li & 15) - 2 * prow) & 15;
     const int row0 = wn * 2 * NT;
     const bool do_rgb = a.rgb_partial != nullptr;
+    float* const ex = ev + EV_VECS * BLOCK_M;
+    float* const it = ex + WN * NT * 3 * 32;
+    constexpr int TH = 2 * NT * WN;
+    if constexpr (FIN) {
+        const auto tl = kernarg_img_tail();
+        const int up = tl->up;
+        const int it_rows = up ? TH / 2 + 2 : TH, it_cols = up ? IT_COLS_UP : F_TILE_W;
+        const int it_r0 = up ? (i0 >> 1) - 1 : i0, it_c0 = up ? (j0 >> 1) - 1 : j0;
+        const int Hp = up ? a.OH >> 1 : a.OH, Wp = up ? a.OW >> 1 : a.OW;
+        const float* I = tl->img_prev + (size_t)n * 3 * Hp * Wp;
+        const int per = it_rows * it_cols;
+        for (int e = threadIdx.x; e < 3 * per; e += 128 * WN) {
+            const int c = e / per, q = e - c * per, rr = q / it_cols, cc = q - rr * it_cols;
+            const int r = it_r0 + rr, cl = it_c0 + cc;
+            it[e] = (r >= 0 && r < Hp && cl >= 0 && cl < Wp) ? I[((size_t)c * Hp + r) * Wp + cl] : 0.f;
+        }
+    }
     {
         constexpr int NTHR = 128 * WN;
-        for (int e = threadIdx.x; e < 6 * BLOCK_M; e += NTHR) {
+        for (int e = threadIdx.x; e < EV_VECS * BLOCK_M; e += NTHR) {
             const int v = e / BLOCK_M, c = e - v * BLOCK_M, co = m0 + c;
             float val = (v == 0 || v == 2) ? 1.f : 0.f;
             if (co < a.CoutReal) {
@@ -381,6 +443,54 @@
         for (int nt = 0; nt < NT; ++nt)
 #pragma unroll
             for (int o = 0; o < 3; ++o) rgbp[nt][o] += __shfl_xor(rgbp[nt][o], 32);
+        if constexpr (FIN) {
+            int tid = threadIdx.x;
+            asm volatile("" : "+v"(tid));
+            const int wave = tid >> 6, wm = wave / WN, wn = wave - wm * WN, li = tid & 31, h = (tid >> 5) & 1;
+            const int prow = li >> 4, pcol = ((li & 15) - 2 * prow) & 15, row0 = wn * 2 * NT;
+            if (wm == 1 && h == 0) {
+#pragma unroll
+                for (int nt = 0; nt < NT; ++nt)
+#pragma unroll
+                    for (int o = 0; o < 3; ++o) ex[((wn * NT + nt) * 3 + o) * 32 + li] = rgbp[nt][o];
+            }
+            __syncthreads();
+            if (wm == 0 && h == 0) {
+                const auto tl = kernarg_img_tail();
+                const int up = tl->up;
+                const int it_rows = up ? TH / 2 + 2 : TH, it_cols = up ? IT_COLS_UP : F_TILE_W;
+                const int it_r0 = up ? (i0 >> 1) - 1 : i0, it_c0 = up ? (j0 >> 1) - 1 : j0;
+                const int Hp = up ? a.OH >> 1 : a.OH, Wp = up ? a.OW >> 1 : a.OW;
+                const size_t cs_img = (size_t)a.OH * a.OW;
+                float b3[3];
+#pragma unroll
+                for (int o = 0; o < 3; ++o) b3[o] = tl->brgb[(size_t)n * tl->brgb_stride_n + o];
+#pragma unroll
+                for (int nt = 0; nt < NT; ++nt) {
+                    const int i = i0 + row0 + nt * 2 + prow, j = j0 + pcol;
+                    if (i < ph.outH && j < ph.outW) {
+                        const int oy = i * ph.oy_mul + ph.oy_add, ox = j * ph.ox_mul + ph.ox_add;
+                        const RgbTaps k = rgb_taps(oy, ox, Hp, Wp);
+                        const size_t p = (size_t)oy * a.OW + ox;
+                        float rgb[3];
+#pragma unroll
+                        for (int o = 0; o < 3; ++o) {
+                            float t = b3[o];
+                            t += rgbp[nt][o];
+                            t += ex[((wn * NT + nt) * 3 + o) * 32 + li];
+                            const float* T = it + o * it_rows * it_cols;
+                            rgb[o] = rgb_pixel(t, a.clamp, up, oy, ox, k, [&](int r, int c) { return T[(r - it_r0) * it_cols + (c - it_c0)]; });
+                            if (tl->img_out) tl->img_out[((size_t)n * 3 + o) * cs_img + p] = rgb[o];
+                        }
+                        if (tl->img_u8) {
+                            uint8_t* d = tl->img_u8 + ((size_t)n * cs_img + p) * 3;
+#pragma unroll
+                            for (int o = 0; o < 3; ++o) d[o] = frame_u8(rgb[o]);
+                        }
+                    }
+                }
+            }
+        } else
         if (h == 0) {
             float* P = a.rgb_partial + (size_t)n * a.rgbp_stride_n + (size_t)(m0 / 64 + wm) * 3 * a.OH * a.OW;
 #pragma unroll
@@ -534,7 +644,7 @@
 
 typedef int i8v __attribute__((ext_vector_type(8)));
 
-template <bool MX = false, int TH = F_TILE_H>
+template <bool MX = false, int TH = F_TILE_H, bool FIN = false>
 __device__ __forceinline__ void conv3x3_dma_block(const Conv2Args& a, const ConvPhase& ph, int n, uint4* lds)
 {
     static_assert(TH == 16 || TH == 8, "tile rows");
@@ -734,7 +844,7 @@
     }
     __syncthreads();
     R3D_STAMP(5);
-    conv_epilogue<WN, NT>(a, ph, n, acc, i0, j0, m0, reinterpret_cast<float*>(lds));
+    conv_epilogue<WN, NT, false, false, FIN>(a, ph, n, acc, i0, j0, m0, reinterpret_cast<float*>(lds));
     if (blockIdx.x == (gridDim.x >> 1) && blockIdx.y == 0 && blockIdx.z == 0 && threadIdx.x == 0) clk_end(kernarg_clk<Conv2Args>());
     R3D_STAMP(6);
 #ifdef R3D_STAMPS
@@ -757,12 +867,27 @@
     conv3x3_dma_block<MX>(a, a.ph[0], blockIdx.z, lds);
 }
 
+template <int WN, int NT, int OCC, int FIN, bool MX>
+__global__ __launch_bounds__(128 * WN, OCC) void conv_mfma_f16x3_kernel(Conv2Args a, ImgTailArgs tl)
+{
+    static_assert(WN == 4 && NT == 2 && FIN == 1, "conv3x3_dma_block: 8 waves x (64 couts x 64 px), image tail");
+    __shared__ uint4 lds[F3_LDS_UINT4];
+    conv3x3_dma_block<MX, F_TILE_H, true>(a, a.ph[0], blockIdx.z, lds);
+}
+
 static constexpr int F3S_LDS_UINT4 = 2 * 768 + 2 * W2_BUF;
 template <bool MX = false>
 __global__ __launch_bounds__(512, 4) void conv_mfma_f16x3_rows8_kernel(Conv2Args a)
 {
     __shared__ uint4 lds[F3S_LDS_UINT4];
     conv3x3_dma_block<MX, 8>(a, a.ph[0], blockIdx.z, lds);
+}
+template <int FIN, bool MX>
+__global__ __launch_bounds__(512, 4) void conv_mfma_f16x3_rows8_kernel(Conv2Args a, ImgTailArgs tl)
+{
+    static_assert(FIN == 1, "image tail");
+    __shared__ uint4 lds[F3S_LDS_UINT4];
+    conv3x3_dma_block<MX, 8, true>(a, a.ph[0], blockIdx.z, lds);
 }
 
 template <int WN, int NT, int OCC>
@@ -1287,30 +1412,15 @@
     const int p = blockIdx.x * blockDim.x + threadIdx.x;
     if (p >= H * W) return;
     const int y = p / W, xx = p - y * W;
-    const int Hh = H >> 1, Wh = W >> 1;
-    const int ky = y >> 1, kx = xx >> 1;
-    int r0, r1, c0, c1; float wy0, wy1, wx0, wx1;
-    if (y & 1) { r0 = ky; r1 = ky + 1; wy0 = 0.75f; wy1 = 0.25f; } else { r0 = ky - 1; r1 = ky; wy0 = 0.25f; wy1 = 0.75f; }
-    if (xx & 1) { c0 = kx; c1 = kx + 1; wx0 = 0.75f; wx1 = 0.25f; } else { c0 = kx - 1; c1 = kx; wx0 = 0.25f; wx1 = 0.75f; }
-    const bool vr0 = r0 >= 0 && r0 < Hh, vr1 = r1 >= 0 && r1 < Hh, vc0 = c0 >= 0 && c0 < Wh, vc1 = c1 >= 0 && c1 < Wh;
+    const int Hp = up ? H >> 1 : H, Wp = up ? W >> 1 : W;
+    const RgbTaps k = rgb_taps(y, xx, Hp, Wp);
     float rgb[3];
 #pragma unroll
     for (int c = 0; c < 3; ++c) {
         float t = brgb[(size_t)n * vec_stride_n + c];
         for (int m = 0; m < nparts; ++m) t += partial[(size_t)n * part_stride_n + ((size_t)m * 3 + c) * H * W + p];
-        if (clamp >= 0.f) t = fminf(fmaxf(t, -clamp), clamp);
-        float upv;
-        if (up) {
-            const float* I = img_prev + ((size_t)n * 3 + c) * Hh * Wh;
-            upv = 0.f;
-            if (vr0 && vc0) upv += I[(size_t)r0 * Wh + c0] * (wy0 * wx0);
-            if (vr0 && vc1) upv += I[(size_t)r0 * Wh + c1] * (wy0 * wx1);
-            if (vr1 && vc0) upv += I[(size_t)r1 * Wh + c0] * (wy1 * wx0);
-            if (vr1 && vc1) upv += I[(size_t)r1 * Wh + c1] * (wy1 * wx1);
-        } else {
-            upv = img_prev[((size_t)n * 3 + c) * H * W + p];
-        }
-        rgb[c] = upv + t;
+        const float* I = img_prev + ((size_t)n * 3 + c) * Hp * Wp;
+        rgb[c] = rgb_pixel(t, clamp, up, y, xx, k, [&](int r, int cc) { return I[(size_t)r * Wp + cc]; });
         if (img_out) img_out[((size_t)n * 3 + c) * H * W + p] = rgb[c];
     }
     if (img_u8) {
@@ -1493,11 +1603,20 @@
 
 static_assert(SR_TILE == F_TILE_H && SR_TILE == F_TILE_W && SR_UP_TILE == U_TILE, "sr_conv_variant / sr_block_variants (r3d_sr_launch.h) size the grids by these tiles");
 
-static void launch_conv2(Conv2Args& a, const SrVariantChoice& v, hipStream_t st)
+static void launch_conv2(Conv2Args& a, const SrVariantChoice& v, hipStream_t st, const ImgTailArgs* tl = nullptr)
 {
     a.clk = prof_clock_slot(R3D_PROF_CONV);
     a.order = v.order;
     const dim3 grid(v.gx, v.gy, v.gz);
+    if (tl) {
+        switch (v.variant) {
+        case SR_VAR_ROWS8: hipLaunchKernelGGL((conv_mfma_f16x3_rows8_kernel<1, false>), grid, dim3(512), 0, st, a, *tl); break;
+        case SR_VAR_ROWS8_MX: hipLaunchKernelGGL((conv_mfma_f16x3_rows8_kernel<1, true>), grid, dim3(512), 0, st, a, *tl); break;
+        case SR_VAR_DIRECT16_MX: hipLaunchKernelGGL((conv_mfma_f16x3_kernel<4, 2, 4, 1, true>), grid, dim3(512), 0, st, a, *tl); break;
+        default: hipLaunchKernelGGL((conv_mfma_f16x3_kernel<4, 2, 4, 1, false>), grid, dim3(512), 0, st, a, *tl); break;
+        }
+        return;
+    }
     switch (v.variant) {
     case SR_VAR_WINO: hipLaunchKernelGGL(conv_wino_f16x3_kernel<false>, grid, dim3(512), 0, st, a); break;
     case SR_VAR_WINO_MX: hipLaunchKernelGGL(conv_wino_f16x3_kernel<true>, grid, dim3(512), 0, st, a); break;
@@ -1525,7 +1644,7 @@
 int sr_block_forward_f16x3(const void* prepacked, const void* styles, int N, int Cin, int Cout, int Hin, int Win, int up,
                            const void* x, int x_format, const float* img, float clamp,
                            void* x_out, int x_out_format, const float* next_scale, size_t next_scale_stride,
-                           float* img_out, uint8_t* img_u8, float* x_absmax, void* workspace, hipStream_t st, bool mx)
+                           float* img_out, uint8_t* img_u8, float* x_absmax, void* workspace, hipStream_t st, bool mx, bool fuse_tail)
 {
     const SrStyleLayout L = sr_style_layout(Cin, Cout);
     const float* pk = reinterpret_cast<const float*>(styles);
@@ -1577,8 +1696,16 @@
         c1.fill(a, Cout, Cout, pk + L.d1f, L.total, L.total);
         a.x = y0; a.x_stride_n = (size_t)Cout / 8 * OH * OW * 2;
         a.wp = reinterpret_cast<const uint4*>(wpk + (wino1 ? P.c1_wino : P.c1));
-        a.wrgb = pk + L.wrgb; a.wrgb_stride_n = L.total; a.rgb_partial = rgbp; a.rgbp_stride_n = (size_t)(Cout / 64) * 3 * OH * OW;
+        a.wrgb = pk + L.wrgb; a.wrgb_stride_n = L.total;
         ProfScope ps(R3D_PROF_CONV, st);
+        if (fuse_tail && sr_image_tail_fuses(v[1], Cout)) {
+            ImgTailArgs tl = {};
+            tl.brgb = pk + L.brgb; tl.brgb_stride_n = L.total; tl.img_prev = img; tl.img_out = img_out; tl.img_u8 = img_u8; tl.up = up;
+            a.rgb_partial = rgbp;
+            launch_conv2(a, v[1], st, &tl);
+            return check_launch("sr_block_forward_fused(f16x3)");
+        }
+        a.rgb_partial = rgbp; a.rgbp_stride_n = (size_t)(Cout / 64) * 3 * OH * OW;
         launch_conv2(a, v[1], st);
     }
     {
diff --git a/real3dportrait_amd/csrc/r3d_sr_launch.h b/real3dportrait_amd/csrc/r3d_sr_launch.h
--- a/real3dportrait_amd/csrc/r3d_sr_launch.h
+++ b/real3dportrait_amd/csrc/r3d_sr_launch.h
@@ -162,6 +162,11 @@
     v[0] = c;
 }
 
+inline bool sr_image_tail_fuses(const SrVariantChoice& v1, int Cout)
+{
+    return Cout == BLOCK_M && (v1.variant == SR_VAR_DIRECT16 || v1.variant == SR_VAR_DIRECT16_MX || v1.variant == SR_VAR_ROWS8 || v1.variant == SR_VAR_ROWS8_MX);
+}
+
 int conv_forward_f16x3(const SrConvCall& c);
 int conv_forward_blend_f16x3(const SrConvCall& c);
 
diff --git a/real3dportrait_amd/superresolution.py b/real3dportrait_amd/superresolution.py
--- a/real3dportrait_amd/superresolution.py
+++ b/real3dportrait_amd/superresolution.py
@@ -227,8 +227,9 @@
         want_x = self.return_x if _return_x is None else _return_x
         out_fmt, next_scale, next_stride = out_target((self.out_format if _out_format is None else _out_format) if want_x else "none", prec == 2, _next)
         x_out = None if out_fmt == "none" else empty(out_fmt, N, Cout, OH, OW, dev)
-        _lib.call("r3d_sr_block_forward", pre, styles, N, Cin, Cout, Hin, Win, self._UP, x, FMT[x_fmt], img, self._clamp(), x_out, FMT[out_fmt],
-                  next_scale, next_stride, img_out, _u8_out, _x_absmax, prec, work, need)
+        entry = "r3d_sr_block_forward_fused" if prec >= 1 and self.is_last else "r3d_sr_block_forward"
+        _lib.call(entry, pre, styles, N, Cin, Cout, Hin, Win, self._UP, x, FMT[x_fmt], img, self._clamp(), x_out, FMT[out_fmt], next_scale, next_stride,
+                  img_out, _u8_out, _x_absmax, prec, work, need)
         if out_fmt in SPLIT_FORMATS:
             tag_split(x_out, out_fmt, _next)
         elif x_out is not None and prec >= 1:
```

Measured after the change: 1683. No clear change (-0.1%).
